# Glaciohound/Chimera-ST

Measured on AMD Instinct MI355X. Metric: train utterances/sec, MuST-C EN-DE s2t_transformer_m, 1/2/4/8 MI355X, higher is better.
Workload: dtype bf16

## Files before the change

chimera-st_amd/csrc/elementwise.hip:

```cpp
#include "cst_common.h"

namespace {

inline int ew_blocks(int64_t items) {
  int64_t b = cst_ceil_div(items, 256);
  return (int)(b < 1 ? 1 : (b > 4096 ? 4096 : b));
}

template <typename T>
__global__ void glu_fwd_kernel(const T* z, T* y, int64_t rows, int64_t C) {
  const int64_t cv = C / 8, total = rows * cv;
  for (int64_t i = (int64_t)blockIdx.x * blockDim.x + threadIdx.x; i < total; i += (int64_t)gridDim.x * blockDim.x) {
    const int64_t r = i / cv, c = (i % cv) * 8;
    float a[8], g[8], o[8];
    load8(z + r * 2 * C + c, a);
    load8(z + r * 2 * C + C + c, g);
#pragma unroll
    for (int e = 0; e < 8; ++e) o[e] = a[e] / (1.0f + __expf(-g[e]));
    store8(y + r * C + c, o);
  }
}

template <typename T>
__global__ void glu_bwd_kernel(const T* dy, const T* z, T* dz, int64_t rows, int64_t C) {
  const int64_t cv = C / 8, total = rows * cv;
  for (int64_t i = (int64_t)blockIdx.x * blockDim.x + threadIdx.x; i < total; i += (int64_t)gridDim.x * blockDim.x) {
    const int64_t r = i / cv, c = (i % cv) * 8;
    float a[8], g[8], d[8], da[8], dg[8];
    load8(z + r * 2 * C + c, a);
    load8(z + r * 2 * C + C + c, g);
    load8(dy + r * C + c, d);
#pragma unroll
    for (int e = 0; e < 8; ++e) {
      const float sg = 1.0f / (1.0f + __expf(-g[e]));
      da[e] = d[e] * sg;
      dg[e] = d[e] * a[e] * sg * (1.0f - sg);
    }
    store8(dz + r * 2 * C + c, da);
    store8(dz + r * 2 * C + C + c, dg);
  }
}

template <typename T>
__global__ void act_bwd_kernel(const T* dy, const T* z, T* dx, int64_t n8, int act) {
  for (int64_t i = (int64_t)blockIdx.x * blockDim.x + threadIdx.x; i < n8; i += (int64_t)gridDim.x * blockDim.x) {
    float d[8], zz[8];
    load8(dy + i * 8, d);
    load8(z + i * 8, zz);
#pragma unroll
    for (int e = 0; e < 8; ++e) d[e] *= dact_t<T>(zz[e], act);
    store8(dx + i * 8, d);
  }
}

template <typename T>
__global__ void act_fwd_kernel(const T* x, T* y, int64_t n8, int act) {
  for (int64_t i = (int64_t)blockIdx.x * blockDim.x + threadIdx.x; i < n8; i += (int64_t)gridDim.x * blockDim.x) {
    float v[8];
    load8(x + i * 8, v);
#pragma unroll
    for (int e = 0; e < 8; ++e) v[e] = act_t<T>(v[e], act);
    store8(y + i * 8, v);
  }
}

template <typename T, bool PART = false, bool DROP = false>
__global__ __launch_bounds__(256) void colsum_kernel(const T* x, int64_t ldx, float* out, int64_t rows, int64_t cols, int64_t rows_per,
                                                     const uint32_t* row_live = nullptr, uint32_t epoch = 0, T* xd = nullptr,
                                                     uint32_t dkey = 0, uint32_t dthr = 0, float dscale = 1.0f) {
  __shared__ float red[16][16 * 8 + 1];
  auto masked = [&](float (&v)[8], int64_t r, int64_t c0) {
    cst_drop8(v, dkey, (uint64_t)(r * cols + c0), dthr, dscale);
    store8(xd + r * ldx + c0, v);
    if (sizeof(T) == 2) {
#pragma unroll
      for (int e = 0; e < 8; ++e) v[e] = bf16_bits_to_f32(f32_to_bf16_bits(v[e]));
    } else {
#pragma unroll
      for (int e = 0; e < 8; ++e) asm volatile("" : "+v"(v[e]));
    }
  };
  const int cl = threadIdx.x & 15, g = threadIdx.x >> 4;
  const int64_t cv = (int64_t)blockIdx.x * 16 + cl;
  const bool ok = cv * 8 < cols;
  const int64_t r0 = (int64_t)blockIdx.y * rows_per;
  const int64_t r1 = r0 + rows_per < rows ? r0 + rows_per : rows;
  float acc[8] = {0, 0, 0, 0, 0, 0, 0, 0};
  if (ok) {
    int64_t r = r0 + g;
    for (; r + 48 < r1; r += 64) {
      if (row_live && row_live[(r - g) >> 6] != epoch) {
        if (DROP) {
          float z[8] = {0, 0, 0, 0, 0, 0, 0, 0};
          store8(xd + r * ldx + cv * 8, z); store8(xd + (r + 16) * ldx + cv * 8, z);
          store8(xd + (r + 32) * ldx + cv * 8, z); store8(xd + (r + 48) * ldx + cv * 8, z);
        }
        continue;
      }
      float v0[8], v1[8], v2[8], v3[8];
      load8(x + r * ldx + cv * 8, v0);
      load8(x + (r + 16) * ldx + cv * 8, v1);
      load8(x + (r + 32) * ldx + cv * 8, v2);
      load8(x + (r + 48) * ldx + cv * 8, v3);
      if (DROP) { masked(v0, r, cv * 8); masked(v1, r + 16, cv * 8); masked(v2, r + 32, cv * 8); masked(v3, r + 48, cv * 8); }
#pragma unroll
      for (int e = 0; e < 8; ++e) acc[e] += (v0[e] + v1[e]) + (v2[e] + v3[e]);
    }
    for (; r < r1; r += 16) {
      float v[8];
      load8(x + r * ldx + cv * 8, v);
      if (DROP) masked(v, r, cv * 8);
#pragma unroll
      for (int e = 0; e < 8; ++e) acc[e] += v[e];
    }
  }
#pragma unroll
  for (int e = 0; e < 8; ++e) red[g][cl * 8 + e] = acc[e];
  __syncthreads();
  if (threadIdx.x < 128) {
    const int c = threadIdx.x;
    float a = 0.0f;
#pragma unroll
    for (int k = 0; k < 16; ++k) a += red[k][c];
    const int64_t col = (int64_t)blockIdx.x * 128 + c;
    if (col < cols) {
      if (PART) out[(int64_t)blockIdx.y * cols + col] = a;
      else atomicAdd(out + col, a);
    }
  }
}

template <typename TO>
__global__ __launch_bounds__(1024) void colsum_reduce_kernel(const float* part, TO* out, int chunks, int64_t cols) {
  __shared__ float red[64][17];
  const int cl = threadIdx.x & 15, g = threadIdx.x >> 4;
  const int64_t c = (int64_t)blockIdx.x * 16 + cl;
  float a = 0.0f;
  if (c < cols)
    for (int i = g; i < chunks; i += 64) a += part[(int64_t)i * cols + c];
  red[g][cl] = a;
  __syncthreads();
  if (g == 0 && c < cols) {
#pragma unroll 8
    for (int k = 1; k < 64; ++k) a += red[k][cl];
    DT<TO>::st(out + c, a);
  }
}

template <typename T>
__global__ void col2im1d_kernel(const T* dcol, const T* z, T* dx, int64_t B, int64_t Lin, int64_t Lout, int64_t C, int k,
                                int stride, int pad, int dact) {
  const int64_t cv = C / 8, total = B * Lin * cv;
  for (int64_t i = (int64_t)blockIdx.x * blockDim.x + threadIdx.x; i < total; i += (int64_t)gridDim.x * blockDim.x) {
    const int64_t c = (i % cv) * 8, l = (i / cv) % Lin, b = i / (cv * Lin);
    float acc[8] = {0, 0, 0, 0, 0, 0, 0, 0};
    for (int j = 0; j < k; ++j) {
      const int64_t num = l + pad - j;
      if (num < 0 || num % stride) continue;
      const int64_t t = num / stride;
      if (t >= Lout) continue;
      float v[8];
      load8(dcol + ((b * Lout + t) * k + j) * C + c, v);
#pragma unroll
      for (int e = 0; e < 8; ++e) acc[e] += v[e];
    }
    if (dact) {
      float zz[8];
      load8(z + (b * Lin + l) * C + c, zz);
#pragma unroll
      for (int e = 0; e < 8; ++e) acc[e] *= dact_t<T>(zz[e], dact);
    }
    store8(dx + (b * Lin + l) * C + c, acc);
  }
// ... 133 lines not shown
  CST_REQUIRE(dtype == CST_F32 || dtype == CST_BF16, "cst_act_fwd: bad dtype");
  hipStream_t s = (hipStream_t)stream;
  CstProfScope prof(CST_K_ELEMENTWISE, s, 0.0, 2.0 * n * cst_dtype_size(dtype));
  if (dtype == CST_BF16) hipLaunchKernelGGL(act_fwd_kernel<bf16_t>, dim3(ew_blocks(n / 8)), dim3(256), 0, s, (const bf16_t*)x, (bf16_t*)y, n / 8, act);
  else hipLaunchKernelGGL(act_fwd_kernel<float>, dim3(ew_blocks(n / 8)), dim3(256), 0, s, (const float*)x, (float*)y, n / 8, act);
  return cst_check_launch("cst_act_fwd");
}

extern "C" int cst_colsum(const void* x, int64_t ldx, float* out, int64_t rows, int64_t cols, int dtype, cst_stream stream) {
  CST_REQUIRE(x && out && rows > 0 && cols > 0 && cols % 8 == 0 && ldx % 8 == 0, "cst_colsum: cols/ldx must be multiples of 8");
  CST_REQUIRE(dtype == CST_F32 || dtype == CST_BF16, "cst_colsum: bad dtype");
  hipStream_t s = (hipStream_t)stream;
  CstProfScope prof(CST_K_ELEMENTWISE, s, 0.0, (double)rows * cols * cst_dtype_size(dtype));
  if (hipMemsetAsync(out, 0, sizeof(float) * cols, s) != hipSuccess) { cst_set_error("cst_colsum: memset failed"); return CST_ERR_LAUNCH; }
  const int64_t cblocks = cst_ceil_div(cols / 8, 16);
  int64_t chunks = cst_ceil_div(1536, cblocks);
  if (chunks > cst_ceil_div(rows, 64)) chunks = cst_ceil_div(rows, 64);
  if (chunks < 1) chunks = 1;
  const int64_t rows_per = cst_ceil_div(rows, chunks);
  dim3 grid((unsigned)cblocks, (unsigned)cst_ceil_div(rows, rows_per));
  if (dtype == CST_BF16) hipLaunchKernelGGL(colsum_kernel<bf16_t>, grid, dim3(256), 0, s, (const bf16_t*)x, ldx, out, rows, cols, rows_per);
  else hipLaunchKernelGGL(colsum_kernel<float>, grid, dim3(256), 0, s, (const float*)x, ldx, out, rows, cols, rows_per);
  return cst_check_launch("cst_colsum");
}

static void colsum_grid(int64_t rows, int64_t cols, int64_t& cblocks, int64_t& nchunks, int64_t& rows_per) {
  cblocks = cst_ceil_div(cols / 8, 16);
  int64_t chunks = cst_ceil_div(1536, cblocks);
  if (chunks > cst_ceil_div(rows, 64)) chunks = cst_ceil_div(rows, 64);
  if (chunks < 1) chunks = 1;
  rows_per = cst_ceil_div(cst_ceil_div(rows, chunks), 64) * 64;
  nchunks = cst_ceil_div(rows, rows_per);
}

extern "C" int64_t cst_colsum_workspace(int64_t rows, int64_t cols) {
  if (rows <= 0 || cols <= 0) return 0;
  int64_t cb, nc, rp;
  colsum_grid(rows, cols, cb, nc, rp);
  return nc * cols * (int64_t)sizeof(float);
}

static int colsum_typed_impl(const void* x, int64_t ldx, void* out, void* workspace, int64_t rows, int64_t cols, int dtype,
                             int out_dtype, const uint32_t* row_live, uint32_t epoch, cst_stream stream) {
  CST_REQUIRE(x && workspace && rows > 0 && cols > 0 && cols % 8 == 0 && ldx % 8 == 0, "cst_colsum_typed: cols/ldx must be multiples of 8");
  CST_REQUIRE((dtype == CST_F32 || dtype == CST_BF16) && (out_dtype == CST_F32 || out_dtype == CST_BF16), "cst_colsum_typed: bad dtype");
  hipStream_t s = (hipStream_t)stream;
  CstProfScope prof(CST_K_ELEMENTWISE, s, 0.0, (double)rows * cols * cst_dtype_size(dtype));
  int64_t cblocks, nchunks, rows_per;
  colsum_grid(rows, cols, cblocks, nchunks, rows_per);
  dim3 grid((unsigned)cblocks, (unsigned)nchunks);
  float* part = (float*)workspace;
  if (dtype == CST_BF16) hipLaunchKernelGGL((colsum_kernel<bf16_t, true>), grid, dim3(256), 0, s, (const bf16_t*)x, ldx, part, rows, cols, rows_per, row_live, epoch);
  else hipLaunchKernelGGL((colsum_kernel<float, true>), grid, dim3(256), 0, s, (const float*)x, ldx, part, rows, cols, rows_per, row_live, epoch);
  if (!out) return cst_check_launch("cst_colsum_typed");
  const dim3 rgrid((unsigned)cst_ceil_div(cols, 16));
  if (out_dtype == CST_BF16) hipLaunchKernelGGL(colsum_reduce_kernel<bf16_t>, rgrid, dim3(1024), 0, s, (const float*)part, (bf16_t*)out, (int)nchunks, cols);
  else hipLaunchKernelGGL(colsum_reduce_kernel<float>, rgrid, dim3(1024), 0, s, (const float*)part, (float*)out, (int)nchunks, cols);
  return cst_check_launch("cst_colsum_typed");
}

extern "C" int cst_dropout_colsum(const void* x, void* xd, void* out, void* workspace, int64_t rows, int64_t cols, int dtype, int out_dtype,
                                  float p, uint32_t key, const uint32_t* row_live, uint32_t epoch, cst_stream stream) {
  CST_REQUIRE(x && xd && workspace && rows > 0 && cols > 0 && cols % 8 == 0, "cst_dropout_colsum: cols must be a multiple of 8");
  CST_REQUIRE((dtype == CST_F32 || dtype == CST_BF16) && (out_dtype == CST_F32 || out_dtype == CST_BF16), "cst_dropout_colsum: bad dtype");
  CST_REQUIRE(p > 0.0f && p < 1.0f, "cst_dropout_colsum: p must be in (0, 1)");
  CST_REQUIRE(!row_live || epoch != 0, "cst_dropout_colsum: stamps need a non-zero epoch");
  hipStream_t s = (hipStream_t)stream;
  CstProfScope prof(CST_K_ELEMENTWISE, s, 0.0, 2.0 * (double)rows * cols * cst_dtype_size(dtype));
  int64_t cblocks, nchunks, rows_per;
  colsum_grid(rows, cols, cblocks, nchunks, rows_per);
  dim3 grid((unsigned)cblocks, (unsigned)nchunks);
  float* part = (float*)workspace;
  const uint32_t thr = cst_drop_thr16(p);
  const float scale = 1.0f / (1.0f - p);
  if (dtype == CST_BF16) hipLaunchKernelGGL((colsum_kernel<bf16_t, true, true>), grid, dim3(256), 0, s, (const bf16_t*)x, cols, part, rows, cols, rows_per, row_live, epoch, (bf16_t*)xd, key, thr, scale);
  else hipLaunchKernelGGL((colsum_kernel<float, true, true>), grid, dim3(256), 0, s, (const float*)x, cols, part, rows, cols, rows_per, row_live, epoch, (float*)xd, key, thr, scale);
  if (!out) return cst_check_launch("cst_dropout_colsum");
  const dim3 rgrid((unsigned)cst_ceil_div(cols, 16));
  if (out_dtype == CST_BF16) hipLaunchKernelGGL(colsum_reduce_kernel<bf16_t>, rgrid, dim3(1024), 0, s, (const float*)part, (bf16_t*)out, (int)nchunks, cols);
  else hipLaunchKernelGGL(colsum_reduce_kernel<float>, rgrid, dim3(1024), 0, s, (const float*)part, (float*)out, (int)nchunks, cols);
  return cst_check_launch("cst_dropout_colsum");
}

extern "C" int cst_colsum_typed(const void* x, int64_t ldx, void* out, void* workspace, int64_t rows, int64_t cols, int dtype,
                                int out_dtype, cst_stream stream) {
  return colsum_typed_impl(x, ldx, out, workspace, rows, cols, dtype, out_dtype, nullptr, 0, stream);
}

extern "C" int cst_colsum_typed_live(const void* x, int64_t ldx, void* out, void* workspace, int64_t rows, int64_t cols, int dtype,
                                     int out_dtype, const uint32_t* row_live, uint32_t epoch, cst_stream stream) {
  CST_REQUIRE(row_live && epoch != 0, "cst_colsum_typed_live: stamps / non-zero epoch required");
  return colsum_typed_impl(x, ldx, out, workspace, rows, cols, dtype, out_dtype, row_live, epoch, stream);
}

extern "C" int cst_col2im1d(const void* dcol, const void* z, void* dx, int64_t B, int64_t Lin, int64_t Lout, int64_t C, int k,
                            int stride, int pad, int dact, int dtype, cst_stream stream) {
  CST_REQUIRE(dcol && dx && B > 0 && Lin > 0 && Lout > 0 && C > 0 && C % 8 == 0 && k >= 1 && stride >= 1 && pad >= 0, "cst_col2im1d: bad args");
  CST_REQUIRE(!dact || z, "cst_col2im1d: dact needs z");
  CST_REQUIRE(dtype == CST_F32 || dtype == CST_BF16, "cst_col2im1d: bad dtype");
  hipStream_t s = (hipStream_t)stream;
  CstProfScope prof(CST_K_ELEMENTWISE, s, 0.0, ((double)B * Lout * k * C + (double)B * Lin * C * (dact ? 2.0 : 1.0)) * cst_dtype_size(dtype));
  const int blocks = ew_blocks(B * Lin * C / 8);
  if (dtype == CST_BF16) hipLaunchKernelGGL(col2im1d_kernel<bf16_t>, dim3(blocks), dim3(256), 0, s, (const bf16_t*)dcol, (const bf16_t*)z, (bf16_t*)dx, B, Lin, Lout, C, k, stride, pad, dact);
  else hipLaunchKernelGGL(col2im1d_kernel<float>, dim3(blocks), dim3(256), 0, s, (const float*)dcol, (const float*)z, (float*)dx, B, Lin, Lout, C, k, stride, pad, dact);
  return cst_check_launch("cst_col2im1d");
}

extern "C" int cst_mask_rows(const void* x, const uint8_t* mask, void* y, int64_t rows, int64_t cols, int dtype, cst_stream stream) {
  CST_REQUIRE(x && mask && y && rows > 0 && cols > 0 && cols % 8 == 0, "cst_mask_rows: bad args");
  CST_REQUIRE(dtype == CST_F32 || dtype == CST_BF16, "cst_mask_rows: bad dtype");
  hipStream_t s = (hipStream_t)stream;
  CstProfScope prof(CST_K_ELEMENTWISE, s, 0.0, 2.0 * rows * cols * cst_dtype_size(dtype));
  const int blocks = ew_blocks(rows * cols / 8);
  if (dtype == CST_BF16) hipLaunchKernelGGL(mask_rows_kernel<bf16_t>, dim3(blocks), dim3(256), 0, s, (const bf16_t*)x, mask, (bf16_t*)y, rows, cols);
  else hipLaunchKernelGGL(mask_rows_kernel<float>, dim3(blocks), dim3(256), 0, s, (const float*)x, mask, (float*)y, rows, cols);
  return cst_check_launch("cst_mask_rows");
}

extern "C" int cst_dropout(const void* x, void* y, int64_t n, float p, uint32_t key, int dtype, cst_stream stream) {
  CST_REQUIRE(x && y && n > 0 && p >= 0.0f && p < 1.0f, "cst_dropout: bad args");
  CST_REQUIRE(dtype == CST_F32 || dtype == CST_BF16, "cst_dropout: bad dtype");
  CST_REQUIRE(((uintptr_t)x % 16 == 0) && ((uintptr_t)y % 16 == 0), "cst_dropout: x/y must be 16-byte aligned");
  hipStream_t s = (hipStream_t)stream;
  CstProfScope prof(CST_K_ELEMENTWISE, s, 0.0, 2.0 * n * cst_dtype_size(dtype));
  const int blocks = ew_blocks(cst_ceil_div(n, 8));
  const uint32_t thr = cst_drop_thr16(p);
  const float scale = 1.0f / (1.0f - p);
  if (dtype == CST_BF16) hipLaunchKernelGGL(dropout_kernel<bf16_t>, dim3(blocks), dim3(256), 0, s, (const bf16_t*)x, (bf16_t*)y, n, key, thr, scale);
  else hipLaunchKernelGGL(dropout_kernel<float>, dim3(blocks), dim3(256), 0, s, (const float*)x, (float*)y, n, key, thr, scale);
  return cst_check_launch("cst_dropout");
}


extern "C" int cst_rows_pack(const void* src, const int32_t* seq_off, void* dst, int64_t B, int64_t T, int64_t C, int tail_sum, int dtype,
                             cst_stream stream) {
  CST_REQUIRE(src && seq_off && dst && B > 0 && T > 0 && C > 0, "cst_rows_pack: bad args");
  CST_REQUIRE(dtype == CST_F32 || dtype == CST_BF16, "cst_rows_pack: bad dtype %d", dtype);
  CST_REQUIRE(C % 8 == 0 && B < 65536, "cst_rows_pack: C=%lld must be a multiple of 8", (long long)C);
  hipStream_t s = (hipStream_t)stream;
  CstProfScope prof(CST_K_ELEMENTWISE, s, 0.0, 2.0 * B * T * C * cst_dtype_size(dtype));
  const dim3 grid((unsigned)cst_ceil_div(T, 4), (unsigned)B);
  if (dtype == CST_BF16) hipLaunchKernelGGL(rows_pack_kernel<bf16_t>, grid, dim3(256), 0, s, (const bf16_t*)src, seq_off, (bf16_t*)dst, (int)T, (int)C, tail_sum);
  else hipLaunchKernelGGL(rows_pack_kernel<float>, grid, dim3(256), 0, s, (const float*)src, seq_off, (float*)dst, (int)T, (int)C, tail_sum);
  return cst_check_launch("cst_rows_pack");
}

extern "C" int cst_rows_unpack(const void* src, const int32_t* seq_off, void* dst, int64_t B, int64_t T, int64_t C, int tail_broadcast, int dtype,
                               cst_stream stream) {
  CST_REQUIRE(src && seq_off && dst && B > 0 && T > 0 && C > 0, "cst_rows_unpack: bad args");
  CST_REQUIRE(dtype == CST_F32 || dtype == CST_BF16, "cst_rows_unpack: bad dtype %d", dtype);
  CST_REQUIRE(C % 8 == 0 && B < 65536, "cst_rows_unpack: C=%lld must be a multiple of 8", (long long)C);
  hipStream_t s = (hipStream_t)stream;
  CstProfScope prof(CST_K_ELEMENTWISE, s, 0.0, 2.0 * B * T * C * cst_dtype_size(dtype));
  const dim3 grid((unsigned)cst_ceil_div(T, 4), (unsigned)B);
  if (dtype == CST_BF16) hipLaunchKernelGGL(rows_unpack_kernel<bf16_t>, grid, dim3(256), 0, s, (const bf16_t*)src, seq_off, (bf16_t*)dst, (int)T, (int)C, tail_broadcast);
  else hipLaunchKernelGGL(rows_unpack_kernel<float>, grid, dim3(256), 0, s, (const float*)src, seq_off, (float*)dst, (int)T, (int)C, tail_broadcast);
  return cst_check_launch("cst_rows_unpack");
}

namespace {
constexpr int WN_ROWS = 256;

template <typename T, bool DOT>
__global__ __launch_bounds__(256) void wn_partial_kernel(const T* v, const T* dw, float* part, int64_t R, int C) {
  const int gpr = C / 8, rl = threadIdx.x / gpr, cg = threadIdx.x % gpr, rpp = 256 / gpr;
  __shared__ float red[256 * 8];
// ... 274 lines not shown
```

chimera-st_amd/csrc/gemm.hip:

```cpp
#include "gemm_common.h"
#include <vector>
#include <stdlib.h>
#include <string.h>
#include <type_traits>

namespace {
using namespace cstg;

template <int BM_, int BN_, int WM_, int WN_, int KV_ = 8>
struct Cfg {
  static constexpr int BM = BM_, BN = BN_, WM = WM_, WN = WN_, NT = 64 * WM_ * WN_, TM = BM_ / WM_ / 32, TN = BN_ / WN_ / 32;
  static constexpr int KV = KV_;
  static_assert(BM_ <= GEMM_MAX_BM && GEMM_MAX_BM % BM_ == 0, "conv0.hip (cst_conv_row_limits) sizes live frames from GEMM_MAX_BM");
};
using CfgSmall = Cfg<128, 128, 2, 2>;
using CfgSkinny = Cfg<64, 64, 2, 2>;
using CfgNarrowN = Cfg<128, 64, 2, 2>;
using CfgNarrowM = Cfg<64, 128, 2, 2>;
using CfgLarge = Cfg<256, 256, 4, 4>;

template <typename T, bool A_KMAJOR, bool B_KMAJOR, bool SEG, typename C, bool CS = false>
__global__ __launch_bounds__(C::NT) void gemm_kernel(GemmParams p) {
  constexpr int BM = C::BM, BN = C::BN, NTHREADS = C::NT, TM = C::TM, TN = C::TN;
  constexpr int VEC = DT<T>::VEC;
  constexpr int KV = C::KV, BK = KV * VEC;
  constexpr int LDK = BK + VEC;
  constexpr int LDMA = sizeof(T) == 2 ? BM + 32 : BM + VEC;
  constexpr int LDMB = sizeof(T) == 2 ? BN + 32 : BN + VEC;
  constexpr int A_ELEMS = A_KMAJOR ? BM * LDK : BK * LDMA;
  constexpr int B_ELEMS = B_KMAJOR ? BN * LDK : BK * LDMB;
  constexpr int MVA = BM / VEC, MVB = BN / VEC;
  constexpr int NVA = BM * KV / NTHREADS, NVB = BN * KV / NTHREADS;
  extern __shared__ __attribute__((aligned(16))) char smem_raw[];
  T* smem = reinterpret_cast<T*>(smem_raw);
  constexpr int STAGE = A_ELEMS + B_ELEMS;

  const int tid = threadIdx.x, lane = tid & 63, wave = tid >> 6;
  const int wm = wave / C::WN, wn = wave % C::WN;

  const int ntiles = p.tiles_m * p.tiles_n;
  int tm, tn, z;
  if (p.split_order) {
    const int total = ntiles * p.splits, L = (int)blockIdx.x + (int)gridDim.x * (int)blockIdx.z;
    const int q = total / 8, r = total % 8, xcd = L % 8, loc = L / 8;
    const int item = (xcd < r ? xcd * (q + 1) : r * (q + 1) + (xcd - r) * q) + loc;
    z = item / ntiles;
    const int t = item % ntiles;
    tm = t / p.tiles_n;
    tn = t % p.tiles_n;
  } else {
    int id = blockIdx.x;
    {
      const int q = ntiles / 8, r = ntiles % 8, xcd = id % 8, loc = id / 8;
      id = (xcd < r ? xcd * (q + 1) : r * (q + 1) + (xcd - r) * q) + loc;
    }
    constexpr int GROUP_M = 8;
    const int per_group = GROUP_M * p.tiles_n;
    const int grp = id / per_group, rem = id % per_group;
    const int gm0 = grp * GROUP_M;
    const int gsz = (p.tiles_m - gm0 < GROUP_M) ? (p.tiles_m - gm0) : GROUP_M;
    tm = gm0 + rem % gsz;
    tn = rem / gsz;
    z = blockIdx.z;
  }
  const int64_t m0 = (int64_t)tm * BM, n0 = (int64_t)tn * BN;

  const int split = z % p.splits;
  const int64_t bidx = z / p.splits;
  const int64_t b0 = bidx / p.batch1, b1 = bidx % p.batch1;
  const T* A = (const T*)p.A + b0 * p.sa0 + b1 * p.sa1;
  const T* B = (const T*)p.B + b0 * p.sb0 + b1 * p.sb1;
  const int64_t cofs = b0 * p.sc0 + b1 * p.sc1;
  const int64_t bofs = b0 * p.sbias0 + b1 * p.sbias1;

  int ktiles = (int)((p.K + BK - 1) / BK);
  const int kfull = (int)(p.K / BK);
  if (p.k_len) {
    typedef const __attribute__((address_space(4))) int32_t* cptr_t;
    const int kl = ((cptr_t)p.k_len)[b0];
    const int live = kl <= 0 ? 0 : (kl + BK - 1) / BK;
    ktiles = live < ktiles ? live : ktiles;
  }
  const int per = (ktiles + p.splits - 1) / p.splits;
// ... 671 lines not shown
  p.tiles_m = (int)cst_ceil_div(M, C::BM);
  p.tiles_n = (int)cst_ceil_div(N, C::BN);
  p.split_order = (p.splits > 1 && nbatch == 1) ? 1 : 0;
  dim3 grid(p.tiles_m * p.tiles_n, 1, (unsigned)(nbatch * p.splits));
  if constexpr (!AK && !BK_ && !SEG && C::NT <= 256) {
    if (p.colsum) {
      static bool attr_cs = false;
      if (!attr_cs) {
        (void)hipFuncSetAttribute(reinterpret_cast<const void*>(&gemm_kernel<T, AK, BK_, SEG, C, true>), hipFuncAttributeMaxDynamicSharedMemorySize, 160 * 1024 - 4096);
        attr_cs = true;
      }
      hipLaunchKernelGGL((gemm_kernel<T, AK, BK_, SEG, C, true>), grid, dim3(C::NT), lds, s, p);
      return cst_check_launch("cst_gemm");
    }
  }
  if (p.colsum) { cst_set_error("cst_gemm: internal: column sums requested from a configuration that does not build them"); return CST_ERR_UNSUPPORTED; }
  hipLaunchKernelGGL((gemm_kernel<T, AK, BK_, SEG, C>), grid, dim3(C::NT), lds, s, p);
  return cst_check_launch("cst_gemm");
}

template <typename T, bool AK, bool BK_, typename C, int NS>
int launch_glds(GemmParams p, int64_t M, int64_t N, int64_t nbatch, hipStream_t s) {
  constexpr int ES = sizeof(T), BKc = 128 / ES;
  constexpr int A_BYTES = AK ? C::BM * 128 : BKc * C::BM * ES, B_BYTES = BK_ ? C::BN * 128 : BKc * C::BN * ES;
  size_t lds = (size_t)NS * (A_BYTES + B_BYTES);
  const size_t stage_bytes = (size_t)64 * (C::BN + 4) * sizeof(float);
  if (lds < stage_bytes) lds = stage_bytes;
  static bool attr_set = false;
  if (!attr_set) {
    (void)hipFuncSetAttribute(reinterpret_cast<const void*>(&gemm_glds_kernel<T, AK, BK_, C, NS>), hipFuncAttributeMaxDynamicSharedMemorySize, 160 * 1024);
    attr_set = true;
  }
  p.tiles_m = (int)cst_ceil_div(M, C::BM);
  p.tiles_n = (int)cst_ceil_div(N, C::BN);
  dim3 grid(p.tiles_m * p.tiles_n, 1, (unsigned)(nbatch * p.splits));
  hipLaunchKernelGGL((gemm_glds_kernel<T, AK, BK_, C, NS>), grid, dim3(C::NT), lds, s, p);
  return cst_check_launch("cst_gemm");
}


struct GemmSwitches {
  bool no_klive;
  int group_m;
  bool no_narrow;
  bool no_4w;
  bool experiment;
  const char* force_cfg;
};

GemmSwitches gemm_switches() {
  static const GemmSwitches once = [] {
    GemmSwitches w;
    w.no_klive = getenv("CST_GEMM_NO_KLIVE") != nullptr;
    const char* gm = getenv("CST_GEMM8P_GROUP_M");
    w.group_m = gm && atoi(gm) > 0 ? atoi(gm) : 4;
    w.no_narrow = getenv("CST_GEMM_NO_NARROW") != nullptr;
    w.no_4w = getenv("CST_GEMM_NO_4W") != nullptr;
    w.experiment = getenv("CST_GEMM_EXPERIMENT") != nullptr;
    w.force_cfg = nullptr;
    return w;
  }();
  GemmSwitches w = once;
  if (w.experiment) {
    const char* f = getenv("CST_GEMM_FORCE_CFG");
    w.force_cfg = f && *f ? f : nullptr;
  }
  return w;
}

enum class Family { Reg, Dma, Persistent8, FourWave };
enum class Tile { Small, Large, Skinny, NarrowN, NarrowM, Big4, Big4N, Unknown };
enum class Colsum { None, Fused, Separate };
using CfgBig4 = Cfg<256, 256, 2, 2>;
using CfgBig4N = Cfg<256, 192, 2, 2>;

struct GemmRoute {
  Family family;
  Tile tile;
  bool bf16, ak, bk;
  bool seg;
  int stages;
  int splits;
  Colsum colsum;
};

struct TileDims { int bm, bn, nt; };
template <typename C> constexpr TileDims dims_of() { return {C::BM, C::BN, C::NT}; }
constexpr TileDims kTileDims[] = {dims_of<CfgSmall>(),   dims_of<CfgLarge>(), dims_of<CfgSkinny>(), dims_of<CfgNarrowN>(),
                                  dims_of<CfgNarrowM>(), dims_of<CfgBig4>(),  dims_of<CfgBig4N>(),  {0, 0, 0}};

bool use_large(const cst_gemm_desc* d, bool seg, int splits) {
  if (seg) return false;
  const int64_t tiles = cst_ceil_div(d->M, 256) * cst_ceil_div(d->N, 256) * d->batch0 * d->batch1 * splits;
  return d->M >= 256 && d->N >= 256 && tiles >= 200;
}

int choose_splits(const cst_gemm_desc* d) {
  if (d->split_k > 1) return d->split_k;
  if (d->split_k == 0 || d->split_k == 1) return 1;
  const int bk = d->dtype == CST_BF16 ? 64 : 32;
  const int64_t ktiles = cst_ceil_div(d->K, bk);
  const int64_t nb = d->batch0 * d->batch1;
  if (d->M >= 256 && d->N >= 256) {
    const int64_t tl = cst_ceil_div(d->M, 256) * cst_ceil_div(d->N, 256) * nb;
    if (tl >= 200) return 1;
    int64_t s = 256 / tl;
    if (s > ktiles / 16) s = ktiles / 16;
    if (s > 32) s = 32;
    if (s >= 1 && tl * s >= 200) return (int)s;
  }
  const int64_t tiles = cst_ceil_div(d->M, 128) * cst_ceil_div(d->N, 128) * nb;
  if (tiles >= 256 || ktiles < 16) return 1;
  const int64_t cap = ktiles / 8 < 32 ? ktiles / 8 : 32;
  int64_t s1 = 256 / tiles, s2 = 512 / tiles;
  if (s1 > cap) s1 = cap;
  if (s2 > cap) s2 = cap;
  if (s1 < 1) s1 = 1;
  if (s2 < 1) s2 = 1;
  const int64_t s = (2.0 / (double)s2 < 0.9 / (double)s1) ? s2 : s1;
  return (int)s;
}

struct Forced { const char* name; bool kk; Family family; Tile tile; int stages; };
const Forced kForced[] = {
    {"small", false, Family::Reg, Tile::Small, 0},     {"narrowm", false, Family::Reg, Tile::NarrowM, 0},
    {"narrown", false, Family::Reg, Tile::NarrowN, 0}, {"skinny", false, Family::Reg, Tile::Skinny, 0},
    {"large", false, Family::Reg, Tile::Large, 0},     {"big4r", false, Family::Reg, Tile::Big4, 0},
    {"skinny4", true, Family::Dma, Tile::Skinny, 4},   {"skinny2", true, Family::Dma, Tile::Skinny, 2},
    {"small2", true, Family::Dma, Tile::Small, 2},     {"small3", true, Family::Dma, Tile::Small, 3},
    {"big4", true, Family::Dma, Tile::Big4, 2},        {"big4n", true, Family::Dma, Tile::Big4N, 2},
    {"big4r", true, Family::Reg, Tile::Big4, 0},       {"large", true, Family::Reg, Tile::Large, 0},
    {"8p", true, Family::Persistent8, Tile::Large, 0}, {"4w", true, Family::FourWave, Tile::Big4N, 0},
};

GemmRoute gemm_route(const cst_gemm_desc* d, const GemmParams& p, const GemmSwitches& sw) {
  GemmRoute r;
  r.bf16 = d->dtype == CST_BF16;
  r.ak = d->a_kmajor != 0;
  r.bk = d->b_kmajor != 0;
  r.seg = (r.ak && d->a_seg) || (r.bk && d->b_seg);
  r.stages = 2;
  r.splits = choose_splits(d);
  const bool kk = r.ak && r.bk, mm = !r.ak && !r.bk;
  const bool large = use_large(d, r.seg, r.splits);
  const int64_t nbatch = d->batch0 * d->batch1;
  r.colsum = !d->colsum ? Colsum::None : (mm && !d->a_seg && !d->b_seg && !large) ? Colsum::Fused : Colsum::Separate;
  auto take = [&r](Family f, Tile t, int stages = 2) { r.family = f; r.tile = t; r.stages = stages; return r; };

  if (!sw.no_narrow && !r.seg && !large && kk && d->N <= 64 && d->M > 256) return take(Family::Dma, Tile::NarrowN);
  if (!sw.no_narrow && !r.seg && !large && mm && d->M <= 64 && d->N > 256) return take(Family::Reg, Tile::NarrowM);

  GemmParams q = p;
  q.splits = r.splits;
  const bool unsplit1 = !r.seg && nbatch == 1 && r.splits == 1;
  if (sw.force_cfg && r.bf16 && !r.seg && nbatch == 1 && (mm || (kk && r.splits == 1))) {
    for (const Forced& f : kForced) {
      if (f.kk != kk || strcmp(f.name, sw.force_cfg) != 0) continue;
      if (f.family == Family::Persistent8 && !cst_gemm8p_supported(q, r.ak, r.bk, nbatch)) break;
      if (f.family == Family::FourWave && !cst_gemm4w_supported(q, r.ak, r.bk, nbatch)) break;
      return take(f.family, f.tile, f.stages);
    }
    return take(Family::Reg, Tile::Unknown);
  }

  const bool mid8p = kk && unsplit1 && d->M >= 256 && d->N >= 256 && cst_ceil_div(d->M, 256) * cst_ceil_div(d->N, 256) >= 150;
  if (kk && unsplit1 && (d->M <= 256 || (!large && !mid8p && cst_ceil_div(d->M, 128) * cst_ceil_div(d->N, 128) < 256))) {
    const bool two_stage = d->M > 256 && cst_ceil_div(d->M, 64) * cst_ceil_div(d->N, 64) > 512;
    return take(Family::Dma, Tile::Skinny, two_stage ? 2 : 4);
  }
  if (r.bf16 && !r.seg && !d->colsum) {
    if (!sw.no_4w && cst_gemm4w_supported(q, r.ak, r.bk, nbatch)) return take(Family::FourWave, Tile::Big4N);
    if (r.ak && (!d->dact || (!d->resid && !d->aux_out)) && (large || mid8p) && cst_gemm8p_supported(q, r.ak, r.bk, nbatch))
      return take(Family::Persistent8, Tile::Large);
  }
  const Tile t = large ? Tile::Large : Tile::Small;
  if (r.seg) return take(Family::Reg, Tile::Small);
  return take(kk && !d->colsum ? Family::Dma : Family::Reg, t);
}

void route_text(const GemmRoute& r, char* out, int64_t n) {
  const TileDims t = kTileDims[(int)r.tile];
  const char* dt = r.bf16 ? "bf16" : "f32";
  const char a = r.ak ? 'k' : 'm', b = r.bk ? 'k' : 'm';
  switch (r.family) {
    case Family::Reg:
      snprintf(out, (size_t)n, "reg %s %c%c%s %dx%d nt%d%s split%d", dt, a, b, r.seg ? " seg" : "", t.bm, t.bn, t.nt,
               r.colsum == Colsum::Fused ? " colsum" : "", r.splits);
      break;
    case Family::Dma: snprintf(out, (size_t)n, "glds %s %c%c %dx%d nt%d ns%d split%d", dt, a, b, t.bm, t.bn, t.nt, r.stages, r.splits); break;
    case Family::Persistent8: snprintf(out, (size_t)n, "8p %c%c", a, b); break;
    case Family::FourWave: snprintf(out, (size_t)n, "4w"); break;
  }
}

}

extern "C" int64_t cst_colsum_workspace(int64_t rows, int64_t cols);
extern "C" int cst_colsum_typed(const void* x, int64_t ldx, void* out, void* workspace, int64_t rows, int64_t cols, int dtype, int out_dtype, cst_stream stream);
extern "C" int cst_colsum_typed_live(const void* x, int64_t ldx, void* out, void* workspace, int64_t rows, int64_t cols, int dtype, int out_dtype,
                                     const uint32_t* row_live, uint32_t epoch, cst_stream stream);

namespace {

int validate(const cst_gemm_desc* d) {
  CST_REQUIRE(d && d->A && d->B && d->C, "cst_gemm: null operand");
  CST_REQUIRE(d->dtype == CST_F32 || d->dtype == CST_BF16, "cst_gemm: bad dtype %d", d->dtype);
  CST_REQUIRE(d->c_dtype == d->dtype || d->c_dtype == CST_F32, "cst_gemm: c_dtype must be dtype or f32");
  CST_REQUIRE(d->M > 0 && d->N > 0 && d->K > 0, "cst_gemm: empty problem M=%lld N=%lld K=%lld", (long long)d->M,
              (long long)d->N, (long long)d->K);
  const int vec = d->dtype == CST_BF16 ? 8 : 4;
  if (d->a_kmajor) CST_REQUIRE(d->K % vec == 0 && d->lda % vec == 0, "cst_gemm: k-major A needs K,lda %% %d == 0 (K=%lld lda=%lld)", vec, (long long)d->K, (long long)d->lda);
  else CST_REQUIRE(d->M % vec == 0 && d->lda % vec == 0, "cst_gemm: mn-major A needs M,lda %% %d == 0 (M=%lld lda=%lld)", vec, (long long)d->M, (long long)d->lda);
  if (d->b_kmajor) CST_REQUIRE(d->K % vec == 0 && d->ldb % vec == 0, "cst_gemm: k-major B needs K,ldb %% %d == 0 (K=%lld ldb=%lld)", vec, (long long)d->K, (long long)d->ldb);
  else CST_REQUIRE(d->N % vec == 0 && d->ldb % vec == 0, "cst_gemm: mn-major B needs N,ldb %% %d == 0 (N=%lld ldb=%lld)", vec, (long long)d->N, (long long)d->ldb);
  CST_REQUIRE(d->a_seg % vec == 0 && d->b_seg % vec == 0 && d->a_seg_stride % vec == 0 && d->b_seg_stride % vec == 0,
              "cst_gemm: segment sizes must be multiples of %d", vec);
  CST_REQUIRE(((uintptr_t)d->A % 16 == 0) && ((uintptr_t)d->B % 16 == 0), "cst_gemm: A/B must be 16-byte aligned");
  CST_REQUIRE(d->sa0 % vec == 0 && d->sa1 % vec == 0 && d->sb0 % vec == 0 && d->sb1 % vec == 0, "cst_gemm: batch strides of A/B must be multiples of %d", vec);
  CST_REQUIRE(d->batch0 >= 1 && d->batch1 >= 1, "cst_gemm: batch counts must be >= 1");
  CST_REQUIRE(!d->dact || d->aux_in, "cst_gemm: dact needs aux_in");
  CST_REQUIRE(d->drop_p >= 0.0f && d->drop_p < 1.0f, "cst_gemm: drop_p must be in [0, 1)");
  CST_REQUIRE(d->drop_p == 0.0f || d->batch0 * d->batch1 == 1, "cst_gemm: fused dropout needs an unbatched problem");
  CST_REQUIRE(!d->colsum || (!d->a_kmajor && !d->a_seg), "cst_gemm: colsum needs an mn-major, unsegmented A");
  return CST_OK;
}

GemmParams fill_params(const cst_gemm_desc* d, const GemmSwitches& sw) {
  GemmParams p;
  p.M = d->M; p.N = d->N; p.K = d->K;
  p.A = d->A; p.lda = d->lda; p.a_seg = d->a_seg; p.a_seg_stride = d->a_seg_stride;
  p.B = d->B; p.ldb = d->ldb; p.b_seg = d->b_seg; p.b_seg_stride = d->b_seg_stride;
  p.C = d->C; p.ldc = d->ldc;
  p.bias = d->bias; p.bias_mode = d->bias ? d->bias_mode : CST_BIAS_NONE; p.sbias0 = d->sbias0; p.sbias1 = d->sbias1;
  p.act = d->act;
  p.aux_out = d->aux_out; p.ld_aux_out = d->ld_aux_out;
  p.dact = d->dact; p.aux_in = d->aux_in; p.ld_aux_in = d->ld_aux_in;
  p.resid = d->resid; p.ld_resid = d->ld_resid;
  p.alpha = d->alpha;
  p.drop_thr = d->drop_p > 0.0f ? cst_drop_thr16(d->drop_p) : 0u;
  p.drop_key = d->drop_key;
  p.drop_scale = d->drop_p > 0.0f ? 1.0f / (1.0f - d->drop_p) : 1.0f;
  p.drop_row0 = 0;
  p.batch1 = d->batch1;
  p.sa0 = d->sa0; p.sa1 = d->sa1; p.sb0 = d->sb0; p.sb1 = d->sb1; p.sc0 = d->sc0; p.sc1 = d->sc1;
  p.c_f32 = (d->c_dtype == CST_F32 && d->dtype != CST_F32) ? 1 : 0;
  {
    auto al16 = [](const void* q) { return q == nullptr || ((uintptr_t)q % 16) == 0; };
    bool ok = d->ldc % 8 == 0 && d->sc0 % 8 == 0 && d->sc1 % 8 == 0 && al16(d->C) && al16(d->bias) && al16(d->aux_out) && al16(d->aux_in) && al16(d->resid);
    if (d->bias && d->bias_mode == CST_BIAS_COL) ok = ok && d->sbias0 % 8 == 0 && d->sbias1 % 8 == 0;
    if (d->aux_out) ok = ok && d->ld_aux_out % 8 == 0;
    if (d->aux_in) ok = ok && d->ld_aux_in % 8 == 0;
    if (d->resid) ok = ok && d->ld_resid % 8 == 0;
    if (d->drop_p > 0.0f) ok = ok && (d->N % 2 == 0);
    p.vec_epi = ok ? 1 : 0;
  }
  p.tiles_m = p.tiles_n = 0;
  p.split_order = 0;
  p.sched = nullptr;
  p.gperm_full = 0;
  p.mrot = 0;
  p.k_live = sw.no_klive ? nullptr : d->k_live;
  p.k_epoch = d->k_epoch;
  p.m_live = sw.no_klive ? nullptr : d->m_live;
  p.m_epoch = d->m_epoch;
  p.k_len = sw.no_klive ? nullptr : d->k_len;
  p.m_len = sw.no_klive ? nullptr : d->m_len;
  p.group_m = sw.group_m;
  p.splits = 1;
  p.ws = nullptr;
  p.colsum = nullptr;
  p.colsum_ws = nullptr;
  return p;
}

int64_t route_workspace(const cst_gemm_desc* d, const GemmRoute& r) {
  const int64_t s = r.splits, nb = d->batch0 * d->batch1;
  int64_t bytes = s > 1 ? s * d->M * d->N * nb * (int64_t)sizeof(float) : 0;
  if (r.colsum == Colsum::Fused) bytes += s > 1 ? s * d->M * nb * (int64_t)sizeof(float) : 0;
  else if (r.colsum == Colsum::Separate) bytes += cst_colsum_workspace(d->K, d->M);
  return bytes;
}

int take_route(const cst_gemm_desc* d, const GemmSwitches& sw, GemmParams& p, GemmRoute& r) {
  r = gemm_route(d, p, sw);
  const int64_t nbatch = d->batch0 * d->batch1;
  CST_REQUIRE(r.colsum != Colsum::Separate || (nbatch == 1 && d->M % 8 == 0 && d->lda % 8 == 0),
              "cst_gemm: colsum of this configuration runs as a separate column sum: unbatched, M and lda multiples of 8");
  CST_REQUIRE(cst_ceil_div(d->M, 128) * cst_ceil_div(d->N, 128) < (1ll << 31) && nbatch * r.splits < 65536, "cst_gemm: grid too large");
  p.splits = r.splits;
  p.colsum = r.colsum == Colsum::Fused ? d->colsum : nullptr;
#ifdef CST_TRACE
  if (p.splits == 1 && d->workspace) p.ws = (float*)d->workspace;
#endif
  const int64_t need = route_workspace(d, r);
  if (need > 0 && (!d->workspace || d->workspace_bytes < need)) {
    if (r.splits > 1) cst_set_error("cst_gemm: split_k=%d needs %lld workspace bytes, got %lld", r.splits, (long long)need, (long long)d->workspace_bytes);
    else cst_set_error("cst_gemm: colsum needs %lld workspace bytes, got %lld", (long long)need, (long long)d->workspace_bytes);
    return CST_ERR_WORKSPACE;
  }
  if (r.splits > 1) {
    p.ws = (float*)d->workspace;
    p.colsum_ws = p.ws + (int64_t)r.splits * d->M * d->N * nbatch;
  }
  return CST_OK;
}

template <typename W>
bool read_back(hipStream_t s, const W* dev, int64_t n, std::vector<W>& host) {
  host.resize((size_t)n);
  return hipStreamSynchronize(s) == hipSuccess && hipMemcpy(host.data(), dev, sizeof(W) * n, hipMemcpyDeviceToHost) == hipSuccess;
}

struct Work { double flops, bytes; };
Work credited_work(const cst_gemm_desc* d, const GemmParams& p, hipStream_t s) {
  double frac = 1.0;
  if (cst_prof_is_on()) {
    std::vector<uint32_t> st;
    std::vector<int32_t> len;
    const int64_t mtiles = cst_ceil_div(d->M, 256);
    if (p.k_live && read_back(s, p.k_live, cst_ceil_div(d->K, 64), st)) {
      int64_t live = 0;
      for (uint32_t v : st) live += v == p.k_epoch;
      frac *= (double)live / (double)st.size();
    }
    if (p.k_len && read_back(s, p.k_len, d->batch0, len)) {
      double sum = 0.0;
      for (int32_t v : len) sum += (double)(v < 0 ? 0 : (v < d->K ? v : d->K));
      frac *= sum / ((double)d->batch0 * (double)d->K);
    }
    if (p.m_len && read_back(s, p.m_len, d->batch0, len)) {
      double live = 0.0;
      for (int32_t v : len) {
        const int64_t t = v <= 0 ? 0 : cst_ceil_div((int64_t)v, 256);
        live += (double)(t < mtiles ? t : mtiles);
      }
      frac *= live / ((double)d->batch0 * (double)mtiles);
    }
    if (p.m_live && read_back(s, p.m_live, cst_ceil_div(d->M, 64), st)) {
      const int64_t nt = (int64_t)st.size();
      int64_t live = 0;
      for (int64_t t = 0; t < mtiles; ++t) {
        bool l = false;
        for (int64_t i = 4 * t; i < 4 * t + 4 && i < nt; ++i) l |= st[i] == p.m_epoch;
        live += l;
      }
      frac *= (double)live / (double)mtiles;
    }
  }
  const double nbatch = (double)(d->batch0 * d->batch1), esz = (double)cst_dtype_size(d->dtype);
  return {2.0 * (double)d->M * (double)d->N * (double)d->K * nbatch * frac,
          ((double)d->M * d->K + (double)d->N * d->K) * esz * nbatch * frac + (double)d->M * d->N * cst_dtype_size(d->c_dtype) * nbatch};
}

int unlaunchable(const GemmRoute& r, const GemmSwitches& sw) {
  if (r.tile == Tile::Unknown) {
    cst_set_error("cst_gemm: unknown CST_GEMM_FORCE_CFG %s", sw.force_cfg ? sw.force_cfg : "");
    return CST_ERR_BAD_ARG;
  }
  if (r.family == Family::Reg && r.colsum == Colsum::Fused && kTileDims[(int)r.tile].nt > 256) {
    cst_set_error("cst_gemm: internal: column sums requested from a configuration that does not build them");
    return CST_ERR_UNSUPPORTED;
  }
  return CST_OK;
}

template <typename T, bool SEG, typename C>
int launch_reg(const GemmRoute& r, const GemmParams& p, int64_t nbatch, hipStream_t s) {
  return r.ak ? (r.bk ? launch<T, true, true, SEG, C>(p, p.M, p.N, nbatch, s) : launch<T, true, false, SEG, C>(p, p.M, p.N, nbatch, s))
              : (r.bk ? launch<T, false, true, SEG, C>(p, p.M, p.N, nbatch, s) : launch<T, false, false, SEG, C>(p, p.M, p.N, nbatch, s));
}

constexpr int arm(Family f, Tile t, int stages = 0) { return ((int)f << 8) | ((int)t << 4) | stages; }

// ... 5 lines not shown
    case arm(Family::Persistent8, Tile::Large): return cst_gemm8p_launch(p, r.ak, r.bk, nbatch, s);
    case arm(Family::FourWave, Tile::Big4N): return cst_gemm4w_launch(p, s);
    case arm(Family::Reg, Tile::Small): return r.seg ? launch_reg<T, true, CfgSmall>(r, p, nbatch, s) : launch_reg<T, false, CfgSmall>(r, p, nbatch, s);
    case arm(Family::Reg, Tile::Large): return launch_reg<T, false, CfgLarge>(r, p, nbatch, s);
    case arm(Family::Reg, Tile::NarrowM): return launch<T, false, false, false, CfgNarrowM>(p, M, N, nbatch, s);
    case arm(Family::Dma, Tile::Small, 2): return launch_glds<T, true, true, CfgSmall, 2>(p, M, N, nbatch, s);
    case arm(Family::Dma, Tile::Large, 2): return launch_glds<T, true, true, CfgLarge, 2>(p, M, N, nbatch, s);
    case arm(Family::Dma, Tile::NarrowN, 2): return launch_glds<T, true, true, CfgNarrowN, 2>(p, M, N, nbatch, s);
    case arm(Family::Dma, Tile::Skinny, 2): return launch_glds<T, true, true, CfgSkinny, 2>(p, M, N, nbatch, s);
    case arm(Family::Dma, Tile::Skinny, 4): return launch_glds<T, true, true, CfgSkinny, 4>(p, M, N, nbatch, s);
    case arm(Family::Reg, Tile::NarrowN): if constexpr (HOOK) return launch<T, false, false, false, CfgNarrowN>(p, M, N, nbatch, s); break;
    case arm(Family::Reg, Tile::Skinny): if constexpr (HOOK) return launch<T, false, false, false, CfgSkinny>(p, M, N, nbatch, s); break;
    case arm(Family::Reg, Tile::Big4):
      if constexpr (HOOK) return r.ak ? launch<T, true, true, false, CfgBig4>(p, M, N, nbatch, s) : launch<T, false, false, false, CfgBig4>(p, M, N, nbatch, s);
      break;
    case arm(Family::Dma, Tile::Small, 3): if constexpr (HOOK) return launch_glds<T, true, true, CfgSmall, 3>(p, M, N, nbatch, s); break;
    case arm(Family::Dma, Tile::Big4, 2): if constexpr (HOOK) return launch_glds<T, true, true, CfgBig4, 2>(p, M, N, nbatch, s); break;
    case arm(Family::Dma, Tile::Big4N, 2): if constexpr (HOOK) return launch_glds<T, true, true, CfgBig4N, 2>(p, M, N, nbatch, s); break;
    default: break;
  }
  const int rc = unlaunchable(r, sw);
  if (rc == CST_OK) cst_set_error("cst_gemm: internal: a route without a launch arm");
  return rc == CST_OK ? CST_ERR_UNSUPPORTED : rc;
}

int finish(const cst_gemm_desc* d, const GemmRoute& r, const GemmParams& p, cst_stream stream) {
  const int64_t nbatch = d->batch0 * d->batch1;
  if (p.splits > 1 && d->defer_reduce) {
    CST_REQUIRE((nbatch == 1 || !d->colsum) && d->alpha == 1.0f && !d->bias && !d->act && !d->dact && !d->aux_out && !d->resid && d->drop_p == 0.0f && d->ldc == d->N &&
                    d->N % 8 == 0 && r.colsum != Colsum::Separate,
                "cst_gemm: defer_reduce needs a plain epilogue and a dense C (batched: no colsum; the slabs are [batch][split][M][N])");
    return CST_OK;
  }
  int rc = CST_OK;
  if (p.splits > 1) {
    const int64_t total = d->M * d->N;
    const int64_t work = (p.vec_epi && d->N % 8 == 0) ? total / 8 : total;
    int blocks = (int)(cst_ceil_div(work, 256) < 2048 ? cst_ceil_div(work, 256) : 2048);
    dim3 grid(blocks, (unsigned)nbatch);
    if (d->dtype == CST_BF16) hipLaunchKernelGGL(splitk_reduce_kernel<bf16_t>, grid, dim3(256), 0, (hipStream_t)stream, p);
    else hipLaunchKernelGGL(splitk_reduce_kernel<float>, grid, dim3(256), 0, (hipStream_t)stream, p);
    rc = cst_check_launch("cst_gemm split-k reduce");
  }
  if (rc == CST_OK && r.colsum == Colsum::Separate) {
    void* cws = (char*)d->workspace + (p.splits > 1 ? (int64_t)p.splits * d->M * d->N * (int64_t)sizeof(float) : 0);
    rc = p.k_live ? cst_colsum_typed_live(d->A, d->lda, d->colsum, cws, d->K, d->M, d->dtype, d->dtype, p.k_live, p.k_epoch, stream)
                  : cst_colsum_typed(d->A, d->lda, d->colsum, cws, d->K, d->M, d->dtype, d->dtype, stream);
  }
  return rc;
}

int gemm_one(const cst_gemm_desc* d, cst_stream stream) {
  int rc = validate(d);
  if (rc != CST_OK) return rc;
  const GemmSwitches sw = gemm_switches();
  GemmParams p = fill_params(d, sw);
  GemmRoute r;
  if ((rc = take_route(d, sw, p, r)) != CST_OK) return rc;
  hipStream_t s = (hipStream_t)stream;
  const int64_t nbatch = d->batch0 * d->batch1;
  const Work w = credited_work(d, p, s);
  CstProfScope prof(CST_K_GEMM, s, w.flops, w.bytes);
  rc = r.bf16 ? launch_route<bf16_t>(r, p, nbatch, s, sw) : launch_route<float>(r, p, nbatch, s, sw);
  if (cst_prof_is_on())
    prof.tag("M=%lld N=%lld K=%lld b=%lld a%c b%c split=%d%s%s%s%s%s%s%s", (long long)d->M, (long long)d->N, (long long)d->K, (long long)nbatch, r.ak ? 'k' : 'm',
             r.bk ? 'k' : 'm', p.splits, d->bias ? " bias" : "", d->act ? " act" : "", d->aux_out ? " aux_out" : "", d->dact ? " dact" : "",
             d->resid ? " resid" : "", d->drop_p > 0 ? " drop" : "", (d->k_live || d->m_live || d->k_len || d->m_len) ? " live" : "");
  return rc != CST_OK ? rc : finish(d, r, p, stream);
}

GemmRoute query_route(const cst_gemm_desc* d) {
  const GemmSwitches sw = gemm_switches();
  return gemm_route(d, fill_params(d, sw), sw);
}

}

extern "C" int cst_gemm_splits(const cst_gemm_desc* d) { return d ? query_route(d).splits : 0; }

extern "C" int cst_gemm_colsum_is_fused(const cst_gemm_desc* d) { return d && query_route(d).colsum == Colsum::Fused ? 1 : 0; }

extern "C" int64_t cst_gemm_workspace(const cst_gemm_desc* d) { return route_workspace(d, query_route(d)); }

extern "C" int cst_gemm_route(const cst_gemm_desc* d, char* out, int64_t out_bytes) {
  if (out && out_bytes > 0) out[0] = 0;
  int rc = validate(d);
  if (rc != CST_OK) return rc;
  CST_REQUIRE(out && out_bytes > 0, "cst_gemm_route: no room for the text");
  const GemmSwitches sw = gemm_switches();
  GemmParams p = fill_params(d, sw);
  GemmRoute r;
  if ((rc = take_route(d, sw, p, r)) != CST_OK) return rc;
  if ((rc = unlaunchable(r, sw)) != CST_OK) return rc;
  route_text(r, out, out_bytes);
  return CST_OK;
}

extern "C" int cst_gemm(const cst_gemm_desc* d, cst_stream stream) { return gemm_one(d, stream); }
```

chimera-st_amd/csrc/gemm8p.hip:

```cpp
#include "gemm_common.h"
#include <atomic>
#include <cstdlib>
#include <mutex>
#include <type_traits>

namespace {
using namespace cstg;
using T = bf16_t;

constexpr int BM = 256, BN = 256, BK = 64, NTHREADS = 512;
static_assert(BM <= cstg::GEMM_MAX_BM && cstg::GEMM_MAX_BM % BM == 0, "conv0.hip (cst_conv_row_limits) sizes live frames from GEMM_MAX_BM");
constexpr int QB = 17408;
constexpr int GSTRIDE = 1088;
constexpr int KSTRIDE = 1024;
constexpr int BUFB = 4 * QB;
constexpr int LDS_BYTES = 2 * BUFB;
constexpr unsigned OOB = 0x80000000u;

template <int N>
__device__ __forceinline__ void wait_vm() { asm volatile("s_waitcnt vmcnt(%0)" ::"n"(N) : "memory"); }
template <int N>
__device__ __forceinline__ void wait_lgkm() { asm volatile("s_waitcnt lgkmcnt(%0)" ::"n"(N) : "memory"); }

__device__ __forceinline__ unsigned lds_off(const void* p) {
  return (unsigned)(uintptr_t)(const __attribute__((address_space(3))) char*)p;
}
__device__ __forceinline__ void lds_write_b64(unsigned addr, uint2 v) {
  asm volatile("ds_write_b64 %0, %1" ::"v"(addr), "v"(v) : "memory");
}
__device__ __forceinline__ void lds_write_b128(unsigned addr, f32x4 v) {
  asm volatile("ds_write_b128 %0, %1" ::"v"(addr), "v"(v) : "memory");
}
__device__ __forceinline__ u32x4 lds_read_b128(unsigned addr) {
  u32x4 v;
  asm volatile("ds_read_b128 %0, %1" : "=v"(v) : "v"(addr) : "memory");
  return v;
}

template <int OFF>
__device__ __forceinline__ u32x4 lds_read_b128_off(unsigned addr) {
  u32x4 v;
  asm volatile("ds_read_b128 %0, %1 offset:%2" : "=v"(v) : "v"(addr), "n"(OFF) : "memory");
  return v;
}

__device__ __forceinline__ void dma16(__amdgpu_buffer_rsrc_t rsrc, char* lds_wave_base, unsigned voff) {
  __builtin_amdgcn_raw_ptr_buffer_load_lds(rsrc, (__attribute__((address_space(3))) void*)lds_wave_base, 16, (int)voff, 0, 0, 0);
}

template <bool AK, bool BKM, int MODE>
__global__ __launch_bounds__(NTHREADS) void gemm8p_kernel(GemmParams p) {
  extern __shared__ __attribute__((aligned(16))) char smem[];
  const int tid = threadIdx.x, lane = tid & 63;
  const int wave = __builtin_amdgcn_readfirstlane(tid >> 6);
  const int wm = wave >> 2, wn = wave & 3;
  const int lrow = lane & 31, hi = lane >> 5;
  const int ntiles = p.tiles_m * p.tiles_n;
  const int total = p.nitems;
  const int ktiles = (int)((p.K + BK - 1) / BK);
  const int per = (ktiles + p.splits - 1) / p.splits;
  typedef const __attribute__((address_space(4))) GemmParams* kparg_t;
  kparg_t kp = (kparg_t)__builtin_amdgcn_kernarg_segment_ptr();

  const int ck = (lane & 7) ^ (((4 * wave) + (lane >> 4)) & 7);
  const int klm = 16 * (wave >> 2) + 4 * (lane >> 4) + (wave & 3);
  const int kla = AK ? ck * 8 : klm, klb = BKM ? ck * 8 : klm;
  const int pa = AK ? 8 * wave + (lane >> 3) : (lane & 15) * 8;
  const int pb = BKM ? 8 * wave + (lane >> 3) : (lane & 15) * 8;
  const unsigned step_a = AK ? (unsigned)(BK * 2) : (unsigned)(BK * p.lda * 2);
  const unsigned step_b = BKM ? (unsigned)(BK * 2) : (unsigned)(BK * p.ldb * 2);
  constexpr bool EXF = MODE == 2;
  const bool fast_epi = MODE != 0 || (!p.c_f32 && p.splits == 1 && p.vec_epi && (p.N % 8) == 0 && p.bias_mode != CST_BIAS_ROW &&
                                (p.bias_mode == CST_BIAS_NONE || p.alpha == 1.0f));
  const bool bias_in_acc = fast_epi && p.bias_mode == CST_BIAS_COL;
  char* const bias_lds = smem + 2 * BUFB;

  __amdgpu_buffer_rsrc_t ra, rb;
  unsigned va0 = 0, vb0 = 0;
  int nt = 0, krem0 = 0, mrem = 0, nrem = 0;
  int hf = 0;
  unsigned lda2 = 0, ldb2 = 0;
  int64_t m0 = 0, n0 = 0, cofs = 0, bofs = 0;
  int zcur = 0;

  auto setup = [&](int v) {
    asm volatile("" : "+s"(kp));
    struct { int64_t M, N, K, lda, ldb, batch1, sa0, sa1, sb0, sb1, sc0, sc1, sbias0, sbias1; const void *A, *B, *bias; int splits, tiles_m, tiles_n; } p;
    p.M = kp->M; p.N = kp->N; p.K = kp->K; p.lda = kp->lda; p.ldb = kp->ldb; p.batch1 = kp->batch1;
    p.sa0 = kp->sa0; p.sa1 = kp->sa1; p.sb0 = kp->sb0; p.sb1 = kp->sb1; p.sc0 = kp->sc0; p.sc1 = kp->sc1;
    p.sbias0 = kp->sbias0; p.sbias1 = kp->sbias1; p.A = kp->A; p.B = kp->B; p.bias = kp->bias;
    p.splits = kp->splits; p.tiles_m = kp->tiles_m; p.tiles_n = kp->tiles_n;
    auto fdiv = [](int n, unsigned long long magic) { return (int)(((unsigned long long)(unsigned)n * magic) >> 40); };
    int half = -1, vt = v;
    if (v >= kp->half_from) {
      const int o = v - kp->half_from;
      half = o & 1;
      vt = kp->half_from + (o >> 1);
    }
    hf = half >= 0 ? 1 : 0;
    const int z = kp->nz > 1 ? fdiv(vt, kp->magic_ntiles) : 0;
    int id = vt - z * ntiles;
    {
      const int q = ntiles >> 3, r = ntiles & 7, xcd = id & 7, loc = id >> 3;
      id = (xcd < r ? xcd * (q + 1) : r * (q + 1) + (xcd - r) * q) + loc;
    }
    if (kp->mrot > 0) {
      int zr = z * kp->mrot;
      zr -= fdiv(zr, kp->magic_ntiles) * ntiles;
      id += zr;
      if (id >= ntiles) id -= ntiles;
    }
    const int GROUP_M = kp->group_m, per_group = kp->per_group, gshift = kp->group_shift;
    int grp = fdiv(id, kp->magic_per_group);
    const int rem = id - grp * per_group;
    if (kp->gperm_full > 0 && grp < kp->gperm_full) {
      const int q = kp->gperm_q, r = kp->gperm_r, big = (q + 1) * r;
      int col, row;
      if (grp < big) { col = fdiv(grp, kp->magic_gq1); row = grp - col * (q + 1); }
      else { const int t = grp - big, c = fdiv(t, kp->magic_gq); col = r + c; row = t - c * q; }
      grp = row * 8 + col;
    }
    const int gm0 = grp * GROUP_M;
    const int gsz = (p.tiles_m - gm0 < GROUP_M) ? (p.tiles_m - gm0) : GROUP_M;
    int tm, tn;
    if (gsz == GROUP_M && gshift >= 0) { tm = gm0 + (rem & (GROUP_M - 1)); tn = rem >> gshift; }
    else { tm = gm0 + rem % gsz; tn = rem / gsz; }
    m0 = (int64_t)tm * BM + (half == 1 ? 128 : 0);
    n0 = (int64_t)tn * BN;
    zcur = z;
    const int split = p.splits > 1 ? z % p.splits : 0;
    const int64_t bidx = p.splits > 1 ? z / p.splits : z;
    const int64_t b0 = p.batch1 > 1 ? bidx / p.batch1 : bidx, b1 = p.batch1 > 1 ? bidx % p.batch1 : 0;
    const T* A = (const T*)p.A + b0 * p.sa0 + b1 * p.sa1;
// ... 69 lines not shown
    const v4s_t x = __builtin_amdgcn_ds_read_tr16_b64_v4i16((v4s_t __attribute__((address_space(3)))*)(q));
    const v4s_t y = __builtin_amdgcn_ds_read_tr16_b64_v4i16((v4s_t __attribute__((address_space(3)))*)(q + 256));
    u16x8 t;
    t[0] = (unsigned short)x[0]; t[1] = (unsigned short)x[1]; t[2] = (unsigned short)x[2]; t[3] = (unsigned short)x[3];
    t[4] = (unsigned short)y[0]; t[5] = (unsigned short)y[1]; t[6] = (unsigned short)y[2]; t[7] = (unsigned short)y[3];
    f.v = __builtin_bit_cast(bf16x8, t);
  };
  auto read_a = [&](Frag<T>& f, const char* img, int i, int kk) {
    if (AK) f.v = *reinterpret_cast<const bf16x8*>(img + arow + i * 4096 + (((2 * kk + hi) ^ swr) << 4));
    else read_tr(f, img + trl + wm * 128 + i * 64 + kk * 4 * GSTRIDE);
  };
  auto read_b = [&](Frag<T>& f, const char* img, int kk) {
    if (BKM) f.v = *reinterpret_cast<const bf16x8*>(img + brow + (((2 * kk + hi) ^ swr) << 4));
    else read_tr(f, img + trl + wn * 64 + kk * 4 * GSTRIDE);
  };

  f32x16 acc[4][2];
  Frag<T> fa[2][4], fb0[4], fb1[4];

  auto mfma_quadrant = [&](auto hmc, auto hnc) {
    constexpr int HM = decltype(hmc)::value, HN = decltype(hnc)::value;
    __builtin_amdgcn_s_setprio(1);
#pragma unroll
    for (int kk = 0; kk < 4; ++kk)
#pragma unroll
      for (int i = 0; i < 2; ++i) mma16(acc[HM * 2 + i][HN], HN ? fb1[kk] : fb0[kk], fa[i][kk]);
    __builtin_amdgcn_s_setprio(0);
  };

  auto tile_body = [&](auto bufc, int t, int S, const bool half) {
    constexpr int BUF = decltype(bufc)::value;
    using BC = std::integral_constant<int, BUF>;
    using BN_ = std::integral_constant<int, BUF ^ 1>;
    const char* img = smem + BUF * BUFB;
    const int s0 = 7 + 4 * t;
#pragma unroll
    for (int kk = 0; kk < 4; ++kk) read_b(fb0[kk], img + 0 * QB, kk);
    __builtin_amdgcn_sched_barrier(0);
#pragma unroll
    for (int kk = 0; kk < 4; ++kk)
#pragma unroll
      for (int i = 0; i < 2; ++i) read_a(fa[i][kk], img + 1 * QB, i, kk);
    __builtin_amdgcn_sched_barrier(0);
    if (s0 < S) stage(I3{}, BN_{}, t + 1);
    wait_lgkm<AK ? 8 : 15>();
    __builtin_amdgcn_s_barrier();
    wait_lgkm<0>();
    __builtin_amdgcn_sched_barrier(0);
    mfma_quadrant(I0{}, I0{});
    __builtin_amdgcn_s_barrier();
#pragma unroll
    for (int kk = 0; kk < 4; ++kk) read_b(fb1[kk], img + 2 * QB, kk);
    __builtin_amdgcn_sched_barrier(0);
    if (s0 + 1 < S) stage(I0{}, BC{}, t + 2);
    __builtin_amdgcn_s_barrier();
    wait_lgkm<0>();
    __builtin_amdgcn_sched_barrier(0);
    mfma_quadrant(I0{}, I1{});
    __builtin_amdgcn_s_barrier();
    if (!half) {
#pragma unroll
      for (int kk = 0; kk < 4; ++kk)
#pragma unroll
        for (int i = 0; i < 2; ++i) read_a(fa[i][kk], img + 3 * QB, i, kk);
    }
    __builtin_amdgcn_sched_barrier(0);
    if (s0 + 2 < S) stage(I1{}, BC{}, t + 2);
    __builtin_amdgcn_s_barrier();
    wait_lgkm<0>();
    __builtin_amdgcn_sched_barrier(0);
    if (!half) mfma_quadrant(I1{}, I1{});
    __builtin_amdgcn_s_barrier();
    if (s0 + 3 < S) stage(I2{}, BC{}, t + 2);
    if (s0 + 4 <= S) wait_vm<6>();
    else wait_vm<0>();
    __builtin_amdgcn_s_barrier();
    __builtin_amdgcn_sched_barrier(0);
    if (!half) mfma_quadrant(I1{}, I0{});
    __builtin_amdgcn_s_barrier();
  };

  char* const ebase = smem + BUFB;
  const unsigned ebase_off = lds_off(ebase);

  int v = blockIdx.x;
  if (v >= total) return;
  const unsigned slot_off = lds_off(smem + 2 * BUFB + 1024);
  int par = 0;
  int claim = 0;
  auto claim_issue = [&]() {
    int* const sched = p.sched;
    if (sched && tid == 0) claim = __hip_atomic_fetch_add(sched + (blockIdx.x & 7), 1, __ATOMIC_RELAXED, __HIP_MEMORY_SCOPE_AGENT);
  };
  auto claim_land = [&]() {
    if (p.sched && tid == 0) {
      const int item = (int)gridDim.x + (int)(blockIdx.x & 7) + 8 * claim;
      asm volatile("ds_write_b32 %0, %1" ::"v"(slot_off + 4u * (unsigned)(par ^ 1)), "v"(item) : "memory");
    }
    par ^= 1;
  };
  setup(v);
  {
    const int S = 4 * nt;
    if (0 < S) stage(I0{}, I0{}, 0);
    if (1 < S) stage(I1{}, I0{}, 0);
    if (2 < S) stage(I2{}, I0{}, 0);
    if (3 < S) stage(I3{}, I0{}, 0);
  }
  claim_issue();
  claim_land();
#ifdef CST_TRACE
  long long* trace = (p.splits == 1 && p.ws) ? reinterpret_cast<long long*>(p.ws) + (int64_t)blockIdx.x * 64 : nullptr;
  int titem = 0;
#define CST_STAMP(k) do { if (trace && tid == 0 && titem < 8) trace[titem * 8 + (k)] = (long long)__builtin_readcyclecounter(); } while (0)
#else
#define CST_STAMP(k) do { } while (0)
#endif
  while (true) {
    CST_STAMP(0);
    const int64_t e_m0 = m0, e_n0 = n0, e_cofs = cofs, e_bofs = bofs;
    const int e_z = zcur, e_nt = nt;
    const bool e_hf = hf != 0;
    const int S = 4 * e_nt;
    if (4 < S) stage(I0{}, I1{}, 1);
    if (5 < S) stage(I1{}, I1{}, 1);
    if (6 < S) stage(I2{}, I1{}, 1);
    if (7 <= S) wait_vm<6>();
    else wait_vm<0>();
    __builtin_amdgcn_s_barrier();
    if (bias_in_acc) {
#pragma unroll
      for (int hn = 0; hn < 2; ++hn)
#pragma unroll
        for (int g = 0; g < 4; ++g) {
          const uint2 raw = *reinterpret_cast<const uint2*>(bias_lds + (hn * 128 + wn * 32 + 8 * g + 4 * hi) * 2);
          const float b0 = __uint_as_float(raw.x << 16), b1 = __uint_as_float(raw.x & 0xffff0000u);
          const float b2 = __uint_as_float(raw.y << 16), b3 = __uint_as_float(raw.y & 0xffff0000u);
#pragma unroll
          for (int i = 0; i < 4; ++i) {
            acc[i][hn][4 * g] = b0; acc[i][hn][4 * g + 1] = b1; acc[i][hn][4 * g + 2] = b2; acc[i][hn][4 * g + 3] = b3;
          }
        }
      wait_lgkm<0>();
    } else {
#pragma unroll
      for (int i = 0; i < 4; ++i)
#pragma unroll
        for (int j = 0; j < 2; ++j)
#pragma unroll
          for (int r = 0; r < 16; ++r) acc[i][j][r] = 0.0f;
    }
    if (wm == 1) __builtin_amdgcn_s_barrier();
    CST_STAMP(1);
    for (int t = 0; t < e_nt; t += 2) {
      tile_body(I0{}, t, S, e_hf);
      if (t + 1 < e_nt) tile_body(I1{}, t + 1, S, e_hf);
    }
    if (wm == 0) __builtin_amdgcn_s_barrier();
    CST_STAMP(2);

    {
      int item;
      asm volatile("ds_read_b32 %0, %1\n\ts_waitcnt lgkmcnt(0)" : "=v"(item) : "v"(slot_off + 4u * (unsigned)par) : "memory");
      v = __builtin_amdgcn_readfirstlane(p.sched ? item : v + (int)gridDim.x);
    }
    const bool has_next = v < total;
    if (has_next) {
      claim_issue();
      setup(v);
      CST_STAMP(5);
      const int Sn = 4 * nt;
      if (0 < Sn) stage(I0{}, I0{}, 0);
      if (1 < Sn) stage(I1{}, I0{}, 0);
      if (2 < Sn) stage(I2{}, I0{}, 0);
      if (3 < Sn) stage(I3{}, I0{}, 0);
      CST_STAMP(6);
    }

    CST_STAMP(3);
    asm volatile("" : "+s"(kp));
    GemmParams q;
    q.M = kp->M; q.N = kp->N; q.C = kp->C; q.ldc = kp->ldc; q.bias = kp->bias; q.bias_mode = kp->bias_mode; q.act = kp->act;
    q.aux_out = kp->aux_out; q.ld_aux_out = kp->ld_aux_out; q.dact = kp->dact; q.aux_in = kp->aux_in; q.ld_aux_in = kp->ld_aux_in;
    q.resid = kp->resid; q.ld_resid = kp->ld_resid; q.alpha = kp->alpha; q.splits = kp->splits; q.ws = kp->ws;
    q.c_f32 = kp->c_f32; q.vec_epi = kp->vec_epi; q.drop_thr = kp->drop_thr; q.drop_key = kp->drop_key; q.drop_scale = kp->drop_scale; q.drop_row0 = kp->drop_row0;
    if (fast_epi && e_nt == 0 && q.bias_mode == CST_BIAS_NONE && !q.resid) {
      if (has_next) claim_land();
      const u32x4 z4 = {0u, 0u, 0u, 0u};
      const int64_t col = e_n0 + (tid & 31) * 8;
      if (col < q.N) {
        T* const cb = (T*)q.C + e_cofs + col;
        T* const xb = q.aux_out ? (T*)q.aux_out + e_cofs + col : nullptr;
#pragma unroll 4
        for (int it = 0; it < (e_hf ? 8 : 16); ++it) {
          const int64_t row = e_m0 + (tid >> 5) + 16 * it;
          if (row < q.M) {
            __builtin_nontemporal_store(z4, reinterpret_cast<u32x4*>(cb + row * q.ldc));
            if (xb) __builtin_nontemporal_store(z4, reinterpret_cast<u32x4*>(xb + row * q.ld_aux_out));
          }
        }
      }
    } else if (fast_epi) {
      constexpr int ERS = 528;
      const T* exsrc = MODE == 1 ? nullptr : (q.dact ? (const T*)q.aux_in : (const T*)q.resid);
      const int64_t exld = q.dact ? q.ld_aux_in : q.ld_resid;
      const bool both = q.dact && q.resid;
      constexpr bool ex_fast = EXF;
      u32x4 exq[8];
      const T* ex_b = nullptr;
      if (ex_fast) {
        int64_t colc = e_n0 + (tid & 31) * 8;
        colc = colc < q.N ? colc : q.N - 8;
        ex_b = exsrc + e_cofs + colc;
#pragma unroll
        for (int it = 0; it < 8; ++it) {
          int64_t row = e_m0 + (tid >> 5) + 16 * it;
          row = row < q.M ? row : q.M - 1;
          exq[it] = __builtin_nontemporal_load(reinterpret_cast<const u32x4*>(ex_b + row * exld));
        }
      }
#pragma unroll
      for (int hm = 0; hm < 2; ++hm) {
        if (hm && e_hf) break;
        if (hm) __builtin_amdgcn_s_barrier();
#pragma unroll
        for (int i = 0; i < 2; ++i)
#pragma unroll
          for (int hn = 0; hn < 2; ++hn)
#pragma unroll
            for (int g = 0; g < 4; ++g) {
              typedef __bf16 bf16x4_t __attribute__((ext_vector_type(4)));
              bf16x4_t pk;
#pragma unroll
              for (int e = 0; e < 4; ++e) pk[e] = static_cast<__bf16>(acc[hm * 2 + i][hn][4 * g + e] * q.alpha);
              lds_write_b64(ebase_off + (wm * 64 + i * 32 + lrow) * ERS + (hn * 128 + wn * 32 + 8 * g + 4 * hi) * 2, __builtin_bit_cast(uint2, pk));
            }
        wait_lgkm<0>();
        __builtin_amdgcn_s_barrier();
        if (hm == 0 && has_next) claim_land();
        if (exsrc && !ex_fast) {
#pragma unroll 2
          for (int it = 0; it < 8; ++it) {
            const int vi = tid + NTHREADS * it;
            const int rl = vi >> 5, cl = (vi & 31) * 8;
            const int64_t row = e_m0 + hm * 128 + rl, col = e_n0 + cl;
            if (row >= q.M || col >= q.N) continue;
            const u32x4 exv = *reinterpret_cast<const u32x4*>(exsrc + e_cofs + row * exld + col);
            const u32x4 zraw = lds_read_b128(ebase_off + rl * ERS + cl * 2);
            wait_lgkm<0>();
            __builtin_amdgcn_sched_barrier(0);
            if (q.aux_out) *reinterpret_cast<u32x4*>((T*)q.aux_out + e_cofs + row * q.ld_aux_out + col) = zraw;
            float x[8];
#pragma unroll
            for (int e = 0; e < 4; ++e) {
              x[2 * e] = __uint_as_float(zraw[e] << 16);
              x[2 * e + 1] = __uint_as_float(zraw[e] & 0xffff0000u);
            }
            if (q.act == CST_ACT_RELU) {
#pragma unroll
              for (int e = 0; e < 8; ++e) x[e] = fmaxf(x[e], 0.0f);
            } else if (q.act == CST_ACT_GELU) {
#pragma unroll
              for (int e = 0; e < 8; ++e) x[e] = gelu_t<T>(x[e]);
            }
            if (q.drop_thr) cst_drop8(x, q.drop_key, (uint64_t)((row + q.drop_row0) * q.N + col), q.drop_thr, q.drop_scale);
            if (q.dact) {
#pragma unroll
              for (int e = 0; e < 4; ++e) {
                x[2 * e] *= dact_t<T>(__uint_as_float(exv[e] << 16), q.dact);
                x[2 * e + 1] *= dact_t<T>(__uint_as_float(exv[e] & 0xffff0000u), q.dact);
              }
              if (both) {
                float rr[8];
                load8((const T*)q.resid + e_cofs + row * q.ld_resid + col, rr);
#pragma unroll
                for (int e = 0; e < 8; ++e) x[e] += rr[e];
              }
            } else {
#pragma unroll
              for (int e = 0; e < 4; ++e) {
                x[2 * e] += __uint_as_float(exv[e] << 16);
                x[2 * e + 1] += __uint_as_float(exv[e] & 0xffff0000u);
              }
            }
            bf16x8 ob;
#pragma unroll
            for (int e = 0; e < 8; ++e) ob[e] = static_cast<__bf16>(x[e]);
            lds_write_b128(ebase_off + rl * ERS + cl * 2, __builtin_bit_cast(f32x4, ob));
          }
          wait_lgkm<0>();
        }
        const bool post = !exsrc && (q.act != CST_ACT_NONE || q.drop_thr);
        {
          constexpr int RSTEP = 16 * ERS;
          const int rl0 = tid >> 5, cl = (tid & 31) * 8;
          const unsigned a0 = ebase_off + rl0 * ERS + cl * 2;
          const int64_t col = e_n0 + cl, row0 = e_m0 + hm * 128 + rl0;
          const bool col_ok = col < q.N;
          u32x4 zr[8];
          zr[0] = lds_read_b128_off<0 * RSTEP>(a0); zr[1] = lds_read_b128_off<1 * RSTEP>(a0);
          zr[2] = lds_read_b128_off<2 * RSTEP>(a0); zr[3] = lds_read_b128_off<3 * RSTEP>(a0);
          zr[4] = lds_read_b128_off<4 * RSTEP>(a0); zr[5] = lds_read_b128_off<5 * RSTEP>(a0);
          zr[6] = lds_read_b128_off<6 * RSTEP>(a0); zr[7] = lds_read_b128_off<7 * RSTEP>(a0);
          T* const cbase = (T*)q.C + e_cofs + row0 * q.ldc + col;
          T* const xbase = (T*)q.aux_out + e_cofs + row0 * q.ld_aux_out + col;
          const bool want_aux = !exsrc && q.aux_out;
          if (ex_fast) {
            wait_lgkm<0>();
            __builtin_amdgcn_sched_barrier(0);
#pragma unroll
            for (int it = 0; it < 8; ++it) {
              const u32x4 zraw = zr[it], exv = exq[it];
              float x[8];
#pragma unroll
              for (int e = 0; e < 4; ++e) {
                x[2 * e] = __uint_as_float(zraw[e] << 16);
                x[2 * e + 1] = __uint_as_float(zraw[e] & 0xffff0000u);
              }
              if (q.act == CST_ACT_RELU) {
#pragma unroll
                for (int e = 0; e < 8; ++e) x[e] = fmaxf(x[e], 0.0f);
              } else if (q.act == CST_ACT_GELU) {
#pragma unroll
                for (int e = 0; e < 8; ++e) x[e] = gelu_t<T>(x[e]);
              }
              if (q.drop_thr) cst_drop8(x, q.drop_key, (uint64_t)((row0 + 16 * it + q.drop_row0) * q.N + col), q.drop_thr, q.drop_scale);
              if (q.dact) {
#pragma unroll
                for (int e = 0; e < 4; ++e) {
                  x[2 * e] *= dact_t<T>(__uint_as_float(exv[e] << 16), q.dact);
                  x[2 * e + 1] *= dact_t<T>(__uint_as_float(exv[e] & 0xffff0000u), q.dact);
                }
              } else {
#pragma unroll
                for (int e = 0; e < 4; ++e) {
                  x[2 * e] += __uint_as_float(exv[e] << 16);
                  x[2 * e + 1] += __uint_as_float(exv[e] & 0xffff0000u);
                }
              }
              bf16x8 ob;
#pragma unroll
              for (int e = 0; e < 8; ++e) ob[e] = static_cast<__bf16>(x[e]);
              zr[it] = __builtin_bit_cast(u32x4, ob);
            }
            if (hm == 0 && !e_hf) {
#pragma unroll
              for (int it = 0; it < 8; ++it) {
                int64_t row = e_m0 + 128 + (tid >> 5) + 16 * it;
                row = row < q.M ? row : q.M - 1;
                exq[it] = __builtin_nontemporal_load(reinterpret_cast<const u32x4*>(ex_b + row * exld));
              }
            }
#pragma unroll
            for (int it = 0; it < 8; ++it)
              if (col_ok && row0 + 16 * it < q.M)
                __builtin_nontemporal_store(zr[it], reinterpret_cast<u32x4*>(cbase + (int64_t)(16 * it) * q.ldc));
            continue;
          }
#pragma unroll
          for (int it = 0; it < 8; ++it) {
            if (it == 0) wait_lgkm<7>(); else if (it == 1) wait_lgkm<6>(); else if (it == 2) wait_lgkm<5>(); else if (it == 3) wait_lgkm<4>();
            else if (it == 4) wait_lgkm<3>(); else if (it == 5) wait_lgkm<2>(); else if (it == 6) wait_lgkm<1>(); else wait_lgkm<0>();
            __builtin_amdgcn_sched_barrier(0);
            const u32x4 zraw = zr[it];
            if (!(col_ok && row0 + 16 * it < q.M)) continue;
            T* cdst = cbase + (int64_t)(16 * it) * q.ldc;
            if (want_aux) __builtin_nontemporal_store(zraw, reinterpret_cast<u32x4*>(xbase + (int64_t)(16 * it) * q.ld_aux_out));
            if (!post) {
              __builtin_nontemporal_store(zraw, reinterpret_cast<u32x4*>(cdst));
              continue;
            }
            float x[8];
#pragma unroll
            for (int e = 0; e < 4; ++e) {
              x[2 * e] = __uint_as_float(zraw[e] << 16);
              x[2 * e + 1] = __uint_as_float(zraw[e] & 0xffff0000u);
            }
            if (q.act == CST_ACT_RELU) {
#pragma unroll
              for (int e = 0; e < 8; ++e) x[e] = fmaxf(x[e], 0.0f);
            } else if (q.act == CST_ACT_GELU) {
#pragma unroll
              for (int e = 0; e < 8; ++e) x[e] = gelu_t<T>(x[e]);
            }
            if (q.drop_thr) cst_drop8(x, q.drop_key, (uint64_t)((row0 + 16 * it + q.drop_row0) * q.N + col), q.drop_thr, q.drop_scale);
            {
              bf16x8 ob;
#pragma unroll
              for (int e = 0; e < 8; ++e) ob[e] = static_cast<__bf16>(x[e]);
              __builtin_nontemporal_store(__builtin_bit_cast(u32x4, ob), reinterpret_cast<u32x4*>(cdst));
            }
          }
        }
      }
    } else {
      constexpr int LDC = BN + 4;
      constexpr int VPR = BN / 8;
      constexpr int ITERS = 64 * VPR / NTHREADS;
      float* wsp = q.splits > 1 ? q.ws + ((int64_t)e_z) * q.M * q.N : nullptr;
      const bool ws_vec = (q.N % 4) == 0;
#pragma unroll
      for (int ps = 0; ps < 4; ++ps) {
        if (ps == 2 && e_hf) break;
        if (ps) __builtin_amdgcn_s_barrier();
        if (wm == (ps & 1)) {
#pragma unroll
          for (int i = 0; i < 2; ++i)
#pragma unroll
            for (int hn = 0; hn < 2; ++hn)
#pragma unroll
              for (int g = 0; g < 4; ++g) {
                f32x4 q;
#pragma unroll
                for (int e = 0; e < 4; ++e) q[e] = acc[(ps >> 1) * 2 + i][hn][4 * g + e];
                lds_write_b128(ebase_off + ((i * 32 + lrow) * LDC + hn * 128 + wn * 32 + 8 * g + 4 * hi) * 4, q);
              }
        }
        wait_lgkm<0>();
        __builtin_amdgcn_s_barrier();
        if (ps == 0 && has_next) claim_land();
#pragma unroll 2
        for (int itv = 0; itv < ITERS; ++itv) {
          const int vi = tid + NTHREADS * itv;
          const int rl = vi / VPR, cl = (vi % VPR) * 8;
          const int64_t row = e_m0 + 64 * ps + rl, col = e_n0 + cl;
          if (row >= q.M || col >= q.N) continue;
          float x[8];
          {
            const u32x4 ua = lds_read_b128(ebase_off + (rl * LDC + cl) * 4), ub = lds_read_b128(ebase_off + (rl * LDC + cl + 4) * 4);
            wait_lgkm<0>();
            __builtin_amdgcn_sched_barrier(0);
            const f32x4 a = __builtin_bit_cast(f32x4, ua), b = __builtin_bit_cast(f32x4, ub);
            x[0] = a[0]; x[1] = a[1]; x[2] = a[2]; x[3] = a[3]; x[4] = b[0]; x[5] = b[1]; x[6] = b[2]; x[7] = b[3];
          }
          const bool full = col + 8 <= q.N;
          if (wsp) {
            if (full && ws_vec) store8(wsp + row * q.N + col, x);
            else
              for (int e = 0; e < 8 && col + e < q.N; ++e) wsp[row * q.N + col + e] = x[e];
          } else if (full && q.vec_epi) {
            epilogue_store8<T>(q, e_cofs, e_bofs, row, col, x);
          } else {
            for (int e = 0; e < 8 && col + e < q.N; ++e) epilogue_store<T>(q, e_cofs, e_bofs, row, col + e, x[e]);
          }
        }
      }
    }
    CST_STAMP(4);
#ifdef CST_TRACE
    ++titem;
#endif
    if (!has_next) break;
    __builtin_amdgcn_s_barrier();
  }
  int* const sched_exit = p.sched;
  if (int* const sched = sched_exit; sched && tid == 0) {
    if (atomicAdd(sched + 8, 1) == (int)gridDim.x - 1) {
#pragma unroll
      for (int i = 0; i < 9; ++i) __hip_atomic_store(sched + i, 0, __ATOMIC_RELAXED, __HIP_MEMORY_SCOPE_AGENT);
    }
  }
}

int* sched_slot() {
  constexpr int SLOTS = 1024, MAXDEV = 64;
  static int* ring[MAXDEV] = {};
  static std::atomic<unsigned> next[MAXDEV];
  static std::mutex mu;
  int dev = 0;
  if (hipGetDevice(&dev) != hipSuccess || dev < 0 || dev >= MAXDEV) return nullptr;
  int* r = __atomic_load_n(&ring[dev], __ATOMIC_ACQUIRE);
  if (!r) {
    std::lock_guard<std::mutex> g(mu);
    r = ring[dev];
    if (!r) {
      void* q = nullptr;
      if (hipMalloc(&q, SLOTS * 64) != hipSuccess) return nullptr;
      if (hipMemset(q, 0, SLOTS * 64) != hipSuccess || hipDeviceSynchronize() != hipSuccess) return nullptr;
      r = (int*)q;
      __atomic_store_n(&ring[dev], r, __ATOMIC_RELEASE);
    }
  }
  return r + 16 * (next[dev].fetch_add(1, std::memory_order_relaxed) % SLOTS);
}

std::atomic<int> g_reserved_cus{[] { const char* e = getenv("CST_GEMM_RESERVE_CUS"); return e ? atoi(e) : 0; }()};

template <bool AK, bool BKM, int MODE>
int launch8p(GemmParams p, int64_t nbatch, hipStream_t s) {
  static bool attr_set = false;
  if (!attr_set) {
    (void)hipFuncSetAttribute(reinterpret_cast<const void*>(&gemm8p_kernel<AK, BKM, MODE>), hipFuncAttributeMaxDynamicSharedMemorySize, 160 * 1024);
    attr_set = true;
  }
  p.tiles_m = (int)cst_ceil_div(p.M, BM);
  p.tiles_n = (int)cst_ceil_div(p.N, BN);
  p.nz = (int)(nbatch * p.splits);
  const int64_t total = (int64_t)p.tiles_m * p.tiles_n * p.nz;
  {
    const int64_t ntl = (int64_t)p.tiles_m * p.tiles_n;
    p.per_group = p.group_m * p.tiles_n;
    if (total * ntl >= (1ll << 40) || total * (int64_t)p.per_group >= (1ll << 40)) { cst_set_error("cst_gemm (8-phase): too many work items"); return CST_ERR_BAD_ARG; }
    p.magic_ntiles = ((1ull << 40) / (unsigned long long)ntl) + 1ull;
    p.magic_per_group = ((1ull << 40) / (unsigned long long)p.per_group) + 1ull;
    p.group_shift = -1;
    for (int sft = 0; sft < 16; ++sft)
      if ((1 << sft) == p.group_m) p.group_shift = sft;
    const int gfull = p.tiles_m / p.group_m;
    p.gperm_full = (p.m_len && gfull >= 16) ? gfull : 0;
    p.mrot = (p.m_len && p.gperm_full == 0 && ntl >= 2) ? (int)(ntl / 8 > 0 ? ntl / 8 : 1) : 0;
    p.gperm_q = gfull / 8;
    p.gperm_r = gfull % 8;
    p.magic_gq = p.gperm_q > 0 ? ((1ull << 40) / (unsigned long long)p.gperm_q) + 1ull : 0ull;
    p.magic_gq1 = ((1ull << 40) / (unsigned long long)(p.gperm_q + 1)) + 1ull;
  }
  static const int ncu = [] {
    int dev = 0, n = 256;
    (void)hipGetDevice(&dev);
    (void)hipDeviceGetAttribute(&n, hipDeviceAttributeMultiprocessorCount, dev);
    return n > 0 ? n : 256;
  }();
  const int avail = ncu - g_reserved_cus.load(std::memory_order_relaxed) > 8 ? ncu - g_reserved_cus.load(std::memory_order_relaxed) : 8;
  const bool no_halves = getenv("CST_GEMM8P_NO_HALVES") != nullptr;
  int64_t nitems = total;
  p.half_from = 0x7fffffff;
  if (!no_halves && p.nz == 1 && total > avail) {
    const int64_t r = total % avail;
    if (r > 0 && 2 * r <= avail) {
      p.half_from = (int)(total - r);
      nitems = total + r;
    }
  }
  p.nitems = (int)nitems;
  dim3 grid((unsigned)(nitems < avail ? nitems : avail), 1, 1);
  static const bool static_walk = getenv("CST_GEMM8P_STATIC") != nullptr;
  hipStreamCaptureStatus cap = hipStreamCaptureStatusNone;
  const bool capturing = hipStreamIsCapturing(s, &cap) != hipSuccess || cap != hipStreamCaptureStatusNone;
  p.sched = (!static_walk && !capturing && nitems > avail && grid.x % 8 == 0) ? sched_slot() : nullptr;
  hipLaunchKernelGGL((gemm8p_kernel<AK, BKM, MODE>), grid, dim3(NTHREADS), LDS_BYTES + 1024 + 64, s, p);
  return cst_check_launch("cst_gemm (8-phase)");
}

}

extern "C" int cst_gemm_reserve_cus(int n) {
  const int old = g_reserved_cus.load();
  if (n >= 0) g_reserved_cus.store(n > 248 ? 248 : n);
  return old;
}

bool cst_gemm8p_supported(const cstg::GemmParams& p, bool ak, bool bk, int64_t nbatch) {
  (void)nbatch;
  if (p.a_seg || p.b_seg) return false;
  const int64_t lim = (int64_t)1 << 31;
  const int64_t ea = ak ? (256 * p.lda + p.K) * 2 : (p.K + 64) * p.lda * 2;
  const int64_t eb = bk ? (256 * p.ldb + p.K) * 2 : (p.K + 64) * p.ldb * 2;
  return ea < lim && eb < lim && p.lda > 0 && p.ldb > 0;
}

int cst_gemm8p_launch(cstg::GemmParams p, bool ak, bool bk, int64_t nbatch, hipStream_t s) {
  const bool fast = !p.c_f32 && p.splits == 1 && p.vec_epi && (p.N % 8) == 0 && p.bias_mode != CST_BIAS_ROW &&
                    (p.bias_mode == CST_BIAS_NONE || p.alpha == 1.0f);
  const bool exf = fast && !p.aux_out && ((p.dact != 0) != (p.resid != nullptr)) && (!p.dact || p.aux_in);
  const bool plainf = fast && !p.dact && !p.resid;
#define CST_8P_MODE(MODE)                                                                                          \
  (ak ? (bk ? launch8p<true, true, MODE>(p, nbatch, s) : launch8p<true, false, MODE>(p, nbatch, s))              \
      : (bk ? launch8p<false, true, MODE>(p, nbatch, s) : launch8p<false, false, MODE>(p, nbatch, s)))
  if (exf) return CST_8P_MODE(2);
  if (plainf) return CST_8P_MODE(1);
  return CST_8P_MODE(0);
#undef CST_8P_MODE
}
```

chimera-st_amd/csrc/gemm_common.h:

```cpp
#pragma once
#include "cst_common.h"

namespace cstg {

constexpr int GEMM_MAX_BM = 256;

struct GemmParams {
  int64_t M, N, K;
  const void* A; int64_t lda, a_seg, a_seg_stride;
  const void* B; int64_t ldb, b_seg, b_seg_stride;
  void* C; int64_t ldc;
  const void* bias; int bias_mode; int64_t sbias0, sbias1;
  int act;
  void* aux_out; int64_t ld_aux_out;
  int dact;
  const void* aux_in; int64_t ld_aux_in;
  const void* resid; int64_t ld_resid;
  float alpha;
  uint32_t drop_thr, drop_key; float drop_scale;
  int64_t drop_row0;
  int64_t batch1;
  int64_t sa0, sa1, sb0, sb1, sc0, sc1;
  int splits;
  float* ws;
  int c_f32;
  int vec_epi;
  int tiles_m, tiles_n;
  int nz;
  int half_from, nitems;
  int group_m;
  unsigned long long magic_ntiles, magic_per_group;
  int per_group, group_shift;
  int gperm_full, gperm_q, gperm_r;
  int mrot;
  unsigned long long magic_gq, magic_gq1;
  int split_order;
  int* sched;
  const uint32_t* m_live; uint32_t m_epoch;
  const int32_t* k_len;
  const int32_t* m_len;
  const uint32_t* k_live; uint32_t k_epoch;
  void* colsum;
  float* colsum_ws;
};

__device__ __forceinline__ int64_t segaddr(int64_t c, int64_t seg, int64_t seg_stride) {
  return seg ? (c / seg) * seg_stride + (c % seg) : c;
}

template <typename T>
__device__ __forceinline__ void epilogue_store(const GemmParams& p, int64_t cofs, int64_t bofs, int64_t row, int64_t col, float v) {
  v *= p.alpha;
  if (p.bias_mode == CST_BIAS_COL) v += DT<T>::ld((const T*)p.bias + bofs + col);
  else if (p.bias_mode == CST_BIAS_ROW) v += DT<T>::ld((const T*)p.bias + bofs + row);
  if (p.aux_out) DT<T>::st((T*)p.aux_out + cofs + row * p.ld_aux_out + col, v);
  v = act_t<T>(v, p.act);
  if (p.drop_thr) v *= cst_drop1(p.drop_key, (uint64_t)((row + p.drop_row0) * p.N + col), p.drop_thr, p.drop_scale);
  if (p.dact) v *= dact_t<T>(DT<T>::ld((const T*)p.aux_in + cofs + row * p.ld_aux_in + col), p.dact);
  if (p.resid) v += DT<T>::ld((const T*)p.resid + cofs + row * p.ld_resid + col);
  if (p.c_f32) ((float*)p.C)[cofs + row * p.ldc + col] = v;
  else DT<T>::st((T*)p.C + cofs + row * p.ldc + col, v);
}

template <typename T>
__device__ __forceinline__ void epilogue_store8(const GemmParams& p, int64_t cofs, int64_t bofs, int64_t row, int64_t col, float (&v)[8]) {
#pragma unroll
  for (int e = 0; e < 8; ++e) v[e] *= p.alpha;
  if (p.bias_mode == CST_BIAS_COL) {
    float b[8];
    load8((const T*)p.bias + bofs + col, b);
#pragma unroll
    for (int e = 0; e < 8; ++e) v[e] += b[e];
  } else if (p.bias_mode == CST_BIAS_ROW) {
    const float b = DT<T>::ld((const T*)p.bias + bofs + row);
#pragma unroll
    for (int e = 0; e < 8; ++e) v[e] += b;
  }
  if (p.aux_out) store8((T*)p.aux_out + cofs + row * p.ld_aux_out + col, v);
  if (p.act == CST_ACT_RELU) {
#pragma unroll
    for (int e = 0; e < 8; ++e) v[e] = fmaxf(v[e], 0.0f);
  } else if (p.act == CST_ACT_GELU) {
#pragma unroll
    for (int e = 0; e < 8; ++e) v[e] = gelu_t<T>(v[e]);
  }
  if (p.drop_thr) cst_drop8(v, p.drop_key, (uint64_t)((row + p.drop_row0) * p.N + col), p.drop_thr, p.drop_scale);
  if (p.dact) {
    float z[8];
    load8((const T*)p.aux_in + cofs + row * p.ld_aux_in + col, z);
#pragma unroll
    for (int e = 0; e < 8; ++e) v[e] *= dact_t<T>(z[e], p.dact);
  }
  if (p.resid) {
    float r[8];
    load8((const T*)p.resid + cofs + row * p.ld_resid + col, r);
#pragma unroll
    for (int e = 0; e < 8; ++e) v[e] += r[e];
  }
  if (p.c_f32) store8((float*)p.C + cofs + row * p.ldc + col, v);
  else store8((T*)p.C + cofs + row * p.ldc + col, v);
}

}

int cst_gemm8p_launch(cstg::GemmParams p, bool a_kmajor, bool b_kmajor, int64_t nbatch, hipStream_t s);
bool cst_gemm8p_supported(const cstg::GemmParams& p, bool a_kmajor, bool b_kmajor, int64_t nbatch);
int cst_gemm4w_launch(cstg::GemmParams p, hipStream_t s);
bool cst_gemm4w_supported(const cstg::GemmParams& p, bool a_kmajor, bool b_kmajor, int64_t nbatch);
```

chimera-st_amd/functional.py:

```python
import os as _os
import weakref as _weakref

import torch

from . import kernels as K
from . import lib as L

_ACT = {None: L.ACT_NONE, "none": L.ACT_NONE, "relu": L.ACT_RELU, "gelu": L.ACT_GELU}


def _flat2d(x):
    return x.reshape(-1, x.shape[-1]).contiguous()


def _vec(dtype):
    return 8 if dtype == torch.bfloat16 else 4


def _with_tiles(t, tiles):
    if t.is_contiguous():
        t._cst_live_tiles = (tiles[0], tiles[1], t.data_ptr(), t.numel(), t.shape[-1], t._version)
        if t._base is not None:
            t._base._cst_live_tiles = t._cst_live_tiles
    return t
# ... 21 lines not shown
    parts = getattr(w, "_cst_parts", None)
    return w._version if parts is None else sum(p._version for p in parts)


class _WeightTransposes:

    def __init__(self):
        self.entries = {}
        self.tables = {}
        self.refreshes = 0
        self.persistent = {}

    def register_storage(self, owner, flat):
        sp = flat.untyped_storage().data_ptr()
        self.persistent[sp] = _weakref.ref(owner)
        _weakref.finalize(owner, self._drop_storage, sp)

    def _drop_storage(self, sp):
        self.persistent.pop(sp, None)
        for k in [k for k, e in self.entries.items() if e[4] == sp]:
            del self.entries[k]
        self.tables.clear()

    def invalidate(self):
        self.entries.clear()
        self.tables.clear()

    @staticmethod
    def _src(e):
        return e[0]() if isinstance(e[0], _weakref.ref) else e[0]

    def get(self, w):
        from .optim import PARAM_EPOCH
        epoch = PARAM_EPOCH[0]
        key = (w.data_ptr(), tuple(w.shape), w.dtype)
        e = self.entries.get(key)
        if e is not None and self._src(e) is None:
            del self.entries[key]
            self.tables.pop((w.device, w.dtype), None)
            e = None
        if e is None:
            sp = w.untyped_storage().data_ptr()
            owner = self.persistent.get(sp)
            if owner is not None and owner() is not None:
                src = w.detach()
                parts = getattr(w, "_cst_parts", None)
                if parts is not None:
                    src._cst_parts = parts
            elif isinstance(w, torch.nn.Parameter):
                src, sp = _weakref.ref(w), None
            else:
                return K.transpose2d(w)
            e = self.entries[key] = [src, K.transpose2d(w), _wversion(w), epoch, sp]
            self.tables.pop((w.device, w.dtype), None)
            return e[1]
        if e[2] != _wversion(w):
            K.transpose2d(w, e[1])
            e[2], e[3] = _wversion(w), epoch
            return e[1]
        if e[3] != epoch:
            kind = (w.device, w.dtype)
            stale = []
            for k, v in list(self.entries.items()):
                t = self._src(v)
                if t is None or t.data_ptr() != k[0]:
                    del self.entries[k]
                    self.tables.pop(kind, None)
                elif t.device == w.device and k[2] == w.dtype and v[3] != epoch:
                    stale.append(v)
            ids = [id(v) for v in stale]
            t = self.tables.get(kind)
            if t is None or t[5] != ids:
                t = self.tables[kind] = K.transpose_table([(self._src(v), v[1]) for v in stale]) + (ids,)
            K.transpose2d_multi(t)
            self.refreshes += 1
            for v in stale:
                v[2], v[3] = _wversion(self._src(v)), epoch
        return e[1]


WEIGHT_TRANSPOSES = _WeightTransposes()


def _may_defer(*params):
    if not K.DEFER.on:
        return False
    for w in params:
        if w is None:
            continue
        for p in (getattr(w, "_cst_parts_params", None) or (w,)):
            if not isinstance(p, torch.nn.Parameter) or p.grad is not None or getattr(p, "_cst_shared", False):
                return False
    return True


def _grad_out(w):
    if _os.environ.get("CST_NO_GRAD_SLOT"):
        return None
    from .optim import grad_slot
    return grad_slot(w)


class _LinearFn(torch.autograd.Function):
    @staticmethod
    def forward(ctx, x, weight, bias, resid, act, drop_p, drop_key):
        x2 = _flat2d(x)
        M, Kd = x2.shape
        N = weight.shape[0]
        w = weight.contiguous()
        ctx.bias_obj = bias
        Np = (N + _vec(x.dtype) - 1) // _vec(x.dtype) * _vec(x.dtype)
        if Np != N:
            wp = torch.zeros(Np, Kd, dtype=w.dtype, device=w.device)
            wp[:N] = w
            w = wp
            if bias is not None:
                bp = torch.zeros(Np, dtype=bias.dtype, device=bias.device)
                bp[:N] = bias
                bias = bp
            assert resid is None and drop_p == 0.0
        y = torch.empty(M, Np, dtype=x.dtype, device=x.device)
        z = torch.empty_like(y) if act != L.ACT_NONE else None
        r2 = _flat2d(resid) if resid is not None else None
        K.gemm(x2, w, y, M, Np, Kd, a_kmajor=1, b_kmajor=1, lda=Kd, ldb=Kd, ldc=Np, bias=bias, act=act, aux_out=z, ld_aux_out=Np,
               resid=r2, ld_resid=Np, split_k=1, drop_p=drop_p, drop_key=drop_key)
        ctx.save_for_backward(x2, w, z)
        ctx.act, ctx.has_bias, ctx.has_resid = act, bias is not None, resid is not None
        ctx.drop = (drop_p, drop_key)
        ctx.xshape, ctx.N = x.shape, N
        if Np != N:
            y = y[:, :N].contiguous()
        return y.view(*x.shape[:-1], N)

    @staticmethod
    def backward(ctx, dy):
        return _linear_backward(ctx, dy, None)


def _dx_gemm(dz, w, M, *, use_wt, like, resid=None, dact=L.ACT_NONE, aux_in=None, drop=(0.0, 0), m_live=None):
    n_out, n_in = w.shape
    dx = torch.empty(M, n_in, dtype=like.dtype, device=like.device)
    b, b_kmajor, ldb = (WEIGHT_TRANSPOSES.get(w), 1, n_out) if use_wt else (w, 0, n_in)
    K.gemm(dz, b, dx, M, n_in, n_out, a_kmajor=1, b_kmajor=b_kmajor, lda=n_out, ldb=ldb, ldc=n_in, dact=dact, aux_in=aux_in, ld_aux_in=n_in,
           resid=resid, ld_resid=n_in, split_k=1, drop_p=drop[0], drop_key=drop[1], m_live=m_live)
    return dx


def _dw_gemm(dz, x2, w, bias_obj, M, *, db_in_dw, live, dz_travels_on, allow_slot=True, allow_defer=True):
    n_out, n_in = w.shape
    dw = _grad_out(w) if allow_slot else None
    if dw is None:
        dw = torch.empty(n_out, n_in, dtype=w.dtype, device=w.device)
    db = torch.empty(n_out, dtype=w.dtype, device=w.device) if db_in_dw else None
    may = allow_defer and _may_defer(w, bias_obj if db_in_dw else None)
    big = not may or not K.dw_colsum_is_fused(n_out, n_in, M, w.dtype) or dz_travels_on
    K.side_gemm(big, (dz, x2, live[0] if live is not None else None), dz, x2, dw, n_out, n_in, M, a_kmajor=0, b_kmajor=0, lda=n_out, ldb=n_in,
                ldc=n_in, split_k=-1, k_live=live, colsum=db, defer=may)
    return dw, db


def _drop_grad(dy2, drop, out_dtype, live, *, with_colsum, defer):
    if with_colsum and not _os.environ.get("CST_NO_DROP_COLSUM"):
        return K.dropout_colsum(dy2.contiguous(), drop[0], drop[1], out_dtype, live, defer=defer)
    return K.dropout(dy2.contiguous(), *drop), None


def _linear_backward(ctx, dy, dxp):
    x2, w, z = ctx.saved_tensors
    M, Kd = x2.shape
    Np, N = w.shape[0], ctx.N
    if dy is None:
        return dxp, None, None, None, None, None, None
    dy2 = _flat2d(dy)
    live = _tiles_of(dy, M)
    if Np != N:
        dyp = torch.zeros(M, Np, dtype=dy2.dtype, device=dy2.device)
        dyp[:, :N] = dy2
        dy2 = dyp
    db_fused = None
    want_db = ctx.has_bias and ctx.needs_input_grad[2]
    db_in_dw = want_db and ctx.needs_input_grad[1] and Np % 8 == 0 and not _os.environ.get("CST_NO_GEMM_COLSUM") and K.dw_colsum_is_fused(Np, Kd, M, w.dtype)
    may_b = want_db and Np == N and _may_defer(w, ctx.bias_obj)
    if ctx.drop[0] > 0.0:
        dy2, db_fused = _drop_grad(dy2, ctx.drop, w.dtype, live, defer=may_b,
                                   with_colsum=not db_in_dw and ctx.act == L.ACT_NONE and want_db and Np == N and N % 8 == 0)
    dz = K.act_bwd(dy2, z, ctx.act) if ctx.act != L.ACT_NONE else dy2
    dx = dw = db = dres = None
    if ctx.needs_input_grad[0]:
        dx = _dx_gemm(dz, w, M, use_wt=_want_wt(M, w), like=x2, resid=_flat2d(dxp) if dxp is not None else None,
                      m_live=live).view(ctx.xshape)
        if live is not None and dxp is None:
            dx = _with_tiles(dx, live)
    if ctx.needs_input_grad[1]:
        dw, db = _dw_gemm(dz, x2, w, ctx.bias_obj, M, db_in_dw=db_in_dw, live=live, dz_travels_on=dz.data_ptr() == dy.data_ptr() and ctx.has_resid,
                          allow_slot=Np == N, allow_defer=Np == N)
        dw = dw[:N]
        if db is not None:
            db = db[:N]
    if want_db and db is None:
        db = db_fused if db_fused is not None else K.colsum(dz, w.dtype, live, defer=may_b)[:N]
    if ctx.has_resid and ctx.needs_input_grad[3]:
        dres = dy
    return dx, dw, db, dres, None, None, None


class _LinearPassFn(torch.autograd.Function):

    @staticmethod
    def forward(ctx, x, weight, bias, act, drop_p, drop_key):
        y = _LinearFn.forward(ctx, x, weight, bias, None, act, drop_p, drop_key)
        ctx.set_materialize_grads(False)
        return y, x.view_as(x)

    @staticmethod
    def backward(ctx, dy, dxp):
        g = _linear_backward(ctx, dy, dxp)
        return g[0], g[1], g[2], None, None, None


def linear_pass(x, weight, bias=None, act=None, dropout_p=0.0):
    return _LinearPassFn.apply(x, weight, bias, _ACT[act], *_drop_args(dropout_p))


def linear(x, weight, bias=None, act=None, resid=None, dropout_p=0.0):
    return _LinearFn.apply(x, weight, bias, resid, _ACT[act], *_drop_args(dropout_p))


class _FFNFn(torch.autograd.Function):

    @staticmethod
    def forward(ctx, x, w1, b1, w2, b2, resid, act, p_act, key_act, p_out, key_out):
        x2 = _flat2d(x)
        M, d = x2.shape
        F_ = w1.shape[0]
        dout = w2.shape[0]
        z1 = torch.empty(M, F_, dtype=x.dtype, device=x.device)
        h = torch.empty_like(z1)
        K.gemm(x2, w1, h, M, F_, d, a_kmajor=1, b_kmajor=1, lda=d, ldb=d, ldc=F_, bias=b1, act=act, aux_out=z1, ld_aux_out=F_, split_k=1,
               drop_p=p_act, drop_key=key_act)
        y = torch.empty(M, dout, dtype=x.dtype, device=x.device)
        r2 = _flat2d(resid) if resid is not None else None
        K.gemm(h, w2, y, M, dout, F_, a_kmajor=1, b_kmajor=1, lda=F_, ldb=F_, ldc=dout, bias=b2, resid=r2, ld_resid=dout, split_k=1,
               drop_p=p_out, drop_key=key_out)
        ctx.save_for_backward(x2, w1, w2, z1, h)
        ctx.cfg = (act, b1 is not None, b2 is not None, resid is not None, x.shape)
        ctx.res_is_x = (resid is not None and resid.data_ptr() == x.data_ptr() and resid.shape == x.shape
                        and resid.stride() == x.stride() and dout == d)
        ctx.drop = (p_act, key_act, p_out, key_out)
        ctx.bias_objs = (b1, b2)
        return y.view(*x.shape[:-1], dout)

    @staticmethod
    def backward(ctx, dy):
        x2, w1, w2, z1, h = ctx.saved_tensors
        act, has_b1, has_b2, has_res, xshape = ctx.cfg
        M, d = x2.shape
        F_, dout = w1.shape[0], w2.shape[0]
        dy2 = _flat2d(dy)
        live = _tiles_of(dy, M)
        p_act, key_act, p_out, key_out = ctx.drop
        b1, b2 = ctx.bias_objs
        db2_fused = None
        gcs = not _os.environ.get("CST_NO_GEMM_COLSUM")
        db2_in_dw = gcs and has_b2 and ctx.needs_input_grad[4] and ctx.needs_input_grad[3] and dout % 8 == 0 and K.dw_colsum_is_fused(dout, F_, M, w2.dtype)
        db1_in_dw = gcs and has_b1 and ctx.needs_input_grad[2] and ctx.needs_input_grad[1] and F_ % 8 == 0 and K.dw_colsum_is_fused(F_, d, M, w1.dtype)
        if p_out > 0.0:
            dy2, db2_fused = _drop_grad(dy2, (p_out, key_out), w2.dtype, live, defer=_may_defer(w2, b2),
                                        with_colsum=not db2_in_dw and has_b2 and ctx.needs_input_grad[4] and dout % 8 == 0)
        use_wt = _want_wt(M, w2) and _want_wt(M, w1)
        dz1 = _dx_gemm(dy2, w2, M, use_wt=use_wt, like=dy2, dact=act, aux_in=z1, drop=(p_act, key_act), m_live=live)
        dx = dw1 = db1 = dw2 = db2 = None
        if ctx.needs_input_grad[3]:
            dw2, db2 = _dw_gemm(dy2, h, w2, b2, M, db_in_dw=db2_in_dw, live=live, dz_travels_on=dy2.data_ptr() == dy.data_ptr() and has_res)
        if has_b2 and ctx.needs_input_grad[4] and db2 is None:
            db2 = db2_fused if db2_fused is not None else K.colsum(dy2, w2.dtype, live, defer=_may_defer(w2, b2))
        if ctx.needs_input_grad[0]:
            dx = _dx_gemm(dz1, w1, M, use_wt=use_wt, like=x2, resid=_flat2d(dy) if ctx.res_is_x else None, m_live=live).view(xshape)
        if ctx.needs_input_grad[1]:
            dw1, db1 = _dw_gemm(dz1, x2, w1, b1, M, db_in_dw=db1_in_dw, live=live, dz_travels_on=False)
        if has_b1 and ctx.needs_input_grad[2] and db1 is None:
            db1 = K.colsum(dz1, w1.dtype, live, defer=_may_defer(w1, b1))
        dres = dy if has_res and ctx.needs_input_grad[5] and not (ctx.res_is_x and ctx.needs_input_grad[0]) else None
        return dx, dw1, db1, dw2, db2, dres, None, None, None, None, None


def ffn(x, w1, b1, w2, b2, act, resid=None, activation_dropout_p=0.0, dropout_p=0.0):
    assert _ACT[act] != L.ACT_NONE
    return _FFNFn.apply(x, w1.contiguous(), b1, w2.contiguous(), b2, resid, _ACT[act], *_drop_args(activation_dropout_p), *_drop_args(dropout_p))


class _LayerNormFn(torch.autograd.Function):
    @staticmethod
    def forward(ctx, x, res, gamma, beta, eps):
        x2 = _flat2d(x)
        r2 = _flat2d(res) if res is not None else None
        y, s, mean, rstd = K.layernorm_fwd(x2, r2, gamma, beta, eps, want_sum=True)
        src = s if res is not None else x2
        ctx.save_for_backward(src, gamma, mean, rstd)
        ctx.has_res = res is not None
        ctx.shape = x.shape
        ctx.set_materialize_grads(False)
        if res is not None:
            return y.view(x.shape), s.view(x.shape)
        return y.view(x.shape), None

    @staticmethod
    def backward(ctx, dy, ds):
        src, gamma, mean, rstd = ctx.saved_tensors
        if dy is None:
            return ds, (ds if ctx.has_res else None), None, None, None
        dy2 = _flat2d(dy)
        dres = _flat2d(ds) if ds is not None else None
        dx, dg, db, tiles = K.layernorm_bwd(dy2, src, gamma, mean, rstd, dres, grad_dtype=gamma.dtype, want_tiles=True, defer=_may_defer(gamma))
        dx = _with_tiles(dx.view(ctx.shape), tiles)
        return dx, (dx if ctx.has_res else None), dg, db, None


def layer_norm(x, gamma, beta, eps=1e-5):
    return _LayerNormFn.apply(x, None, gamma, beta, eps)[0]


def add_layer_norm(x, res, gamma, beta, eps=1e-5):
    return _LayerNormFn.apply(x, res, gamma, beta, eps)


class _LayerNormPassFn(torch.autograd.Function):

    @staticmethod
    def forward(ctx, x, gamma, beta, eps):
        x2 = _flat2d(x)
        y, _, mean, rstd = K.layernorm_fwd(x2, None, gamma, beta, eps)
        ctx.save_for_backward(x2, gamma, mean, rstd)
        ctx.shape = x.shape
        ctx.set_materialize_grads(False)
        return y.view(x.shape), x.view_as(x)

    @staticmethod
    def backward(ctx, dy, dxp):
        x2, gamma, mean, rstd = ctx.saved_tensors
        dres = _flat2d(dxp) if dxp is not None else None
        if dy is None:
            return (dxp, None, None, None)
        dx, dg, db = K.layernorm_bwd(_flat2d(dy), x2, gamma, mean, rstd, dres, grad_dtype=gamma.dtype, defer=_may_defer(gamma))
        return dx.view(ctx.shape), dg, db, None


def layer_norm_residual(x, gamma, beta, eps=1e-5):
    return _LayerNormPassFn.apply(x, gamma, beta, eps)


_MASK_CACHE = []


_PAD_TILES = []


def _pad_tiles(u8):
    for src, pt in _PAD_TILES:
        if src is u8:
            return pt
    flat = u8.reshape(-1)
    pad = (-flat.numel()) % 64
    if pad:
        flat = torch.cat([flat, torch.ones(pad, dtype=flat.dtype, device=flat.device)])
# ... 826 lines not shown
```

chimera-st_amd/kernels.py:

```python
import ctypes
import os

import torch

from . import lib as L

_ws = {}
STATS = {}


def workspace(nbytes: int, device) -> torch.Tensor:
    key = (device.index, L.stream_ptr().value)
    t = _ws.get(key)
    if t is None or t.numel() < nbytes:
        t = torch.empty(max(nbytes, 1 << 20), dtype=torch.uint8, device=device)
        _ws[key] = t
    return t


class _Deferred:

    MAX_BYTES = 32 << 20

    def __init__(self):
# ... 15 lines not shown
        if self.side_used:
            torch.cuda.current_stream().wait_stream(self.side)
            self.side_used = False

    def flush(self):
        self.join()
        if self.items:
            reduce_multi(self.items)
            self.flushes += 1
            self.items, self.keep = [], []


DEFER = _Deferred()


def reduce_multi(items):
    lib = L.load()
    for at in range(0, len(items), 64):
        chunk = items[at:at + 64]
        arr = (L.ReduceItem * len(chunk))()
        for a, (src, dst, stride, Lr, P, dt, order) in zip(arr, chunk):
            a.src, a.dst, a.stride, a.L, a.P, a.dst_dtype, a.order = src, dst, stride, Lr, P, dt, order
        L.check(lib.cst_reduce_multi(arr, len(chunk), L.stream_ptr()), "cst_reduce_multi")


class deferred_reductions:

    def __init__(self, enabled=True):
        self.enabled = bool(enabled) and not os.environ.get("CST_NO_DEFER")

    def __enter__(self):
        if self.enabled:
            DEFER.on += 1
            DEFER.main = torch.cuda.current_stream()
            DEFER.poison = bool(os.environ.get("CST_DEFER_POISON"))
        return self

    def __exit__(self, *exc):
        if self.enabled:
            DEFER.on -= 1
            if DEFER.on == 0:
                DEFER.flush()
        return False


def side_gemm(big, reads, *args, **kw):
    if big or not DEFER.on or DEFER.main is None or not os.environ.get("CST_SIDE_STREAM") or torch.cuda.current_stream() != DEFER.main:
        return gemm(*args, **kw)
    if DEFER.side is None:
        DEFER.side = torch.cuda.Stream()
    side = DEFER.side
    side.wait_stream(DEFER.main)
    DEFER.side_used = True
    with torch.cuda.stream(side):
        out = gemm(*args, **kw)
    for t in reads:
        if t is not None:
            t.record_stream(side)
    STATS["side_gemm"] = STATS.get("side_gemm", 0) + 1
    return out


def _2d(t):
    assert t.dim() == 2 and t.stride(1) == 1, "expected a row-major 2-D tensor, got %s / %s" % (tuple(t.shape), t.stride())
    return t


def _stamps(live, extent, stat):
    if live is None:
        return None, 0
    assert live[0].numel() * 64 >= extent and live[0].dtype == torch.int32
    STATS[stat] = STATS.get(stat, 0) + 1
    return live[0].data_ptr(), live[1]


def _per_batch(v, batch0, stat):
    if v is None:
        return None
    assert v.dtype == torch.int32 and v.numel() == batch0 and v.is_contiguous()
    STATS[stat] = STATS.get(stat, 0) + 1
    return v.data_ptr()


def gemm(A, B, C, M, N, K, *, a_kmajor, b_kmajor, lda, ldb, ldc, bias=None, bias_mode=L.BIAS_COL, act=L.ACT_NONE,
         aux_out=None, ld_aux_out=0, dact=L.ACT_NONE, aux_in=None, ld_aux_in=0, resid=None, ld_resid=0, alpha=1.0,
         batch0=1, batch1=1, sa=(0, 0), sb=(0, 0), sc=(0, 0), sbias=(0, 0), a_seg=0, a_seg_stride=0, b_seg=0,
         b_seg_stride=0, split_k=-1, a_off=0, b_off=0, c_off=0, drop_p=0.0, drop_key=0, k_live=None, m_live=None, k_len=None, m_len=None,
         ws=None, colsum=None, defer=False, reduce_to=None):
    lib = L.load()
    d = L.GemmDesc()
    d.dtype = L.dtype_code(A.dtype)
    assert B.dtype == A.dtype, "A/B dtype mismatch"
    d.c_dtype = L.dtype_code(C.dtype)
    d.a_kmajor, d.b_kmajor = int(a_kmajor), int(b_kmajor)
    d.M, d.N, d.K = M, N, K
    es = A.element_size()
    d.A = A.data_ptr() + a_off * es
    d.lda, d.a_seg, d.a_seg_stride = lda, a_seg, a_seg_stride
    d.B = B.data_ptr() + b_off * es
    d.ldb, d.b_seg, d.b_seg_stride = ldb, b_seg, b_seg_stride
    d.C = C.data_ptr() + c_off * C.element_size()
    d.ldc = ldc
    if bias is not None:
        assert bias.dtype == A.dtype
        d.bias, d.bias_mode = bias.data_ptr(), bias_mode
    else:
        d.bias, d.bias_mode = None, L.BIAS_NONE
    d.sbias0, d.sbias1 = sbias
    d.act = act
    d.aux_out = None if aux_out is None else aux_out.data_ptr() + c_off * es
    d.ld_aux_out = ld_aux_out
    d.dact = dact
    d.aux_in = None if aux_in is None else aux_in.data_ptr() + c_off * es
    d.ld_aux_in = ld_aux_in
    d.resid = None if resid is None else resid.data_ptr() + c_off * es
    d.ld_resid = ld_resid
    d.alpha = alpha
    d.drop_p, d.drop_key = float(drop_p), int(drop_key) & 0xFFFFFFFF
    d.batch0, d.batch1 = batch0, batch1
    d.sa0, d.sa1 = sa
    d.sb0, d.sb1 = sb
    d.sc0, d.sc1 = sc
    d.split_k = split_k
    d.k_live, d.k_epoch = _stamps(k_live, K, "gemm_k_live")
    d.m_live, d.m_epoch = _stamps(m_live, M, "gemm_m_live")
    d.k_len = _per_batch(k_len, batch0, "gemm_k_len")
    d.m_len = _per_batch(m_len, batch0, "gemm_m_len")
    if colsum is not None:
        assert not a_kmajor and colsum.dtype == A.dtype and colsum.is_contiguous() and colsum.numel() == M * batch0 * batch1
        d.colsum = colsum.data_ptr()
    else:
        d.colsum = None
    d.defer_reduce = 0
    splits = 1
    need = lib.cst_gemm_workspace(ctypes.byref(d))
    nb = batch0 * batch1
    deferred = False
    if need > 0 and (reduce_to is not None or (defer and DEFER.on and nb == 1 and need <= DEFER.MAX_BYTES and ldc == N and N % 8 == 0)):
        splits = lib.cst_gemm_splits(ctypes.byref(d))
        if splits > 1:
            assert ws is None and bias is None and act == L.ACT_NONE and dact == L.ACT_NONE and resid is None and aux_out is None and alpha == 1.0
            ws = torch.empty(need, dtype=torch.uint8, device=A.device)
            d.defer_reduce = 1
            deferred = True
    if need > 0:
        if ws is None:
            ws = workspace(need, A.device)
        assert ws.dtype == torch.uint8 and ws.numel() >= need, "split-K scratch too small: %d < %d" % (ws.numel(), need)
        d.workspace, d.workspace_bytes = ws.data_ptr(), ws.numel()
    else:
        d.workspace, d.workspace_bytes = None, 0
    L.check(lib.cst_gemm(ctypes.byref(d), L.stream_ptr()), "cst_gemm")
    if reduce_to is not None:
        assert C.dtype == torch.float32 and sc == (M * N, 0) and ldc == N and reduce_to.numel() == M * N and reduce_to.is_contiguous() and colsum is None
        item = ((ws.data_ptr(), reduce_to, M * N, M * N, nb * splits, ws) if deferred else (C.data_ptr(), reduce_to, M * N, M * N, nb, C))
        if defer and DEFER.on:
            DEFER.push(*item)
        else:
            reduce_multi([(item[0], item[1].data_ptr(), item[2], item[3], item[4], L.dtype_code(reduce_to.dtype), 0)])
    elif deferred:
        DEFER.push(ws.data_ptr(), C, M * N, M * N, splits, ws)
        if colsum is not None:
            DEFER.push(ws.data_ptr() + 4 * splits * M * N, colsum, M, M, splits, ws)
    return C


_DW_FUSED = {}


def dw_colsum_is_fused(n_out, k_in, tokens, dtype):
    key = (n_out, k_in, tokens, dtype)
    r = _DW_FUSED.get(key)
    if r is None:
        d = L.GemmDesc()
        d.dtype = d.c_dtype = L.dtype_code(dtype)
        d.a_kmajor = d.b_kmajor = 0
        d.M, d.N, d.K = n_out, k_in, tokens
        d.batch0 = d.batch1 = 1
        d.split_k = -1
        d.colsum = 1
        r = _DW_FUSED[key] = bool(L.load().cst_gemm_colsum_is_fused(ctypes.byref(d)))
        if len(_DW_FUSED) > 4096:
            _DW_FUSED.clear()
    return r


def layernorm_fwd(x, res, gamma, beta, eps, want_sum=False):
    x = _2d(x)
    rows, cols = x.shape
    y = torch.empty_like(x)
    s = torch.empty_like(x) if (want_sum and res is not None) else None
    mean = torch.empty(rows, dtype=torch.float32, device=x.device)
    rstd = torch.empty(rows, dtype=torch.float32, device=x.device)
    L.check(L.load().cst_layernorm_fwd(L.ptr(x), L.ptr(res), L.ptr(gamma), L.ptr(beta), L.ptr(y), L.ptr(s), L.ptr(mean),
                                       L.ptr(rstd), rows, cols, eps, L.dtype_code(x.dtype), L.stream_ptr()), "cst_layernorm_fwd")
    return y, s, mean, rstd


_EPOCH = [0x3C6EF372]


def next_epoch():
    _EPOCH[0] = (_EPOCH[0] % 0xFFFFFFFE) + 1
    return _EPOCH[0]


def _two_stage(wbytes, outs, defer, launch):
    deferred = bool(defer) and DEFER.on > 0
    dev = outs[0].device
    ws = torch.empty(wbytes, dtype=torch.uint8, device=dev) if deferred else workspace(wbytes, dev)
    launch(ws, *[None if deferred else L.ptr(o) for o in outs])
    if deferred:
        n, cols = len(outs), outs[0].numel()
        for i, o in enumerate(outs):
            DEFER.push(ws.data_ptr() + 4 * cols * i, o, n * cols, cols, wbytes // (4 * n * cols), ws, order=1)


def layernorm_bwd(dy, s, gamma, mean, rstd, dres=None, grad_dtype=torch.float32, want_tiles=False, defer=False):
    dy, s = _2d(dy), _2d(s)
    rows, cols = s.shape
    lib = L.load()
    dx = torch.empty_like(s)
    dg = torch.empty(cols, dtype=grad_dtype, device=s.device)
    db = torch.empty(cols, dtype=grad_dtype, device=s.device)
    stamps, epoch = (torch.empty((rows + 63) // 64, dtype=torch.int32, device=s.device), next_epoch()) if want_tiles else (None, 0)

    def launch(ws, pg, pb):
        if want_tiles:
            L.check(lib.cst_layernorm_bwd_tiles(L.ptr(dy), L.ptr(s), L.ptr(gamma), L.ptr(mean), L.ptr(rstd), L.ptr(dres), L.ptr(dx), pg,
                                                pb, L.ptr(ws), rows, cols, L.dtype_code(s.dtype), L.dtype_code(grad_dtype),
                                                L.ptr(stamps), epoch, L.stream_ptr()), "cst_layernorm_bwd_tiles")
        else:
            L.check(lib.cst_layernorm_bwd(L.ptr(dy), L.ptr(s), L.ptr(gamma), L.ptr(mean), L.ptr(rstd), L.ptr(dres), L.ptr(dx), pg,
                                          pb, L.ptr(ws), rows, cols, L.dtype_code(s.dtype), L.dtype_code(grad_dtype), L.stream_ptr()),
                    "cst_layernorm_bwd")

    _two_stage(lib.cst_layernorm_bwd_workspace(rows, cols), (dg, db), defer, launch)
    return (dx, dg, db, (stamps, epoch)) if want_tiles else (dx, dg, db)


def _bhtd_strides(t, layout):
    assert t.stride(-1) == 1
    if layout == "bt":
        return t.stride(0), None, t.stride(1)
    return t.stride(1), None, t.stride(0)


def attn_desc(q, k, v, o, lse, H, D, kpm, causal, scale, layout_q="bt", layout_kv="bt", drop_p=0.0, drop_key=0, kv_len=None, seq=None):
    d = L.AttnDesc()
# ... 224 lines not shown

def glu_fwd(z):
    z = _2d(z)
    rows, C2 = z.shape
    y = torch.empty(rows, C2 // 2, dtype=z.dtype, device=z.device)
    L.check(L.load().cst_glu_fwd(L.ptr(z), L.ptr(y), rows, C2 // 2, L.dtype_code(z.dtype), L.stream_ptr()), "cst_glu_fwd")
    return y


def glu_bwd(dy, z):
    dy, z = _2d(dy), _2d(z)
    rows, C2 = z.shape
    dz = torch.empty_like(z)
    L.check(L.load().cst_glu_bwd(L.ptr(dy), L.ptr(z), L.ptr(dz), rows, C2 // 2, L.dtype_code(z.dtype), L.stream_ptr()), "cst_glu_bwd")
    return dz


def act_bwd(dy, z, act):
    assert dy.is_contiguous() and z.is_contiguous()
    dx = torch.empty_like(z)
    L.check(L.load().cst_act_bwd(L.ptr(dy), L.ptr(z), L.ptr(dx), z.numel(), act, L.dtype_code(z.dtype), L.stream_ptr()), "cst_act_bwd")
    return dx


def posconv_fwd(x, wg, bias, groups, m_len=None):
    B, T, C = x.shape
    k = wg.shape[2]
    assert x.is_contiguous() and wg.is_contiguous() and x.dtype == torch.bfloat16 and wg.dtype == x.dtype
    y = torch.empty_like(x)
    z = torch.empty_like(x)
    L.check(L.load().cst_posconv_fwd(L.ptr(x), L.ptr(wg), L.ptr(bias) if bias is not None else None, L.ptr(y), L.ptr(z),
                                     _per_batch(m_len, B, "gemm_m_len"), B, T, C, groups, k, L.stream_ptr()), "cst_posconv_fwd")
    return y, z


def posconv_dx(dz, wflip, dy, groups, m_len=None):
    B, T, C = dz.shape
    k = wflip.shape[2]
    assert dz.is_contiguous() and dy.is_contiguous() and wflip.is_contiguous() and dz.dtype == torch.bfloat16
    dx = torch.empty_like(dz)
    L.check(L.load().cst_posconv_dx(L.ptr(dz), L.ptr(wflip), L.ptr(dy), L.ptr(dx), _per_batch(m_len, B, "gemm_m_len"),
                                    B, T, C, groups, k, L.stream_ptr()), "cst_posconv_dx")
    return dx


def posconv_dw(dz, x, groups, k, db=None, k_live=None):
    B, T, C = dz.shape
    assert dz.is_contiguous() and x.is_contiguous() and dz.dtype == torch.bfloat16 and x.dtype == dz.dtype
    assert db is None or (db.dtype == dz.dtype and db.numel() == C and db.is_contiguous())
    dw = torch.empty(C, C // groups, k, dtype=dz.dtype, device=dz.device)
    Tp = T + k - 1 + (1 if k % 2 == 0 else 0)
    stamps, epoch = _stamps(k_live, B * Tp - (k - 1), "gemm_k_live")
    L.check(L.load().cst_posconv_dw(L.ptr(dz), L.ptr(x), L.ptr(dw), L.ptr(db) if db is not None else None,
                                    stamps, epoch, B, T, C, groups, k, L.stream_ptr()), "cst_posconv_dw")
    return dw


def act_fwd(x, act):
    assert x.is_contiguous()
    y = torch.empty_like(x)
    L.check(L.load().cst_act_fwd(L.ptr(x), L.ptr(y), x.numel(), act, L.dtype_code(x.dtype), L.stream_ptr()), "cst_act_fwd")
    return y


def colsum(x, out_dtype=torch.float32, live=None, defer=False):
    x = _2d(x)
    rows, cols = x.shape
    lib = L.load()
    out = torch.empty(cols, dtype=out_dtype, device=x.device)

    def launch(ws, po):
        if live is not None:
            assert live[0].numel() * 64 >= rows
            L.check(lib.cst_colsum_typed_live(L.ptr(x), x.stride(0), po, L.ptr(ws), rows, cols, L.dtype_code(x.dtype),
                                              L.dtype_code(out_dtype), L.ptr(live[0]), live[1], L.stream_ptr()), "cst_colsum_typed_live")
        else:
            L.check(lib.cst_colsum_typed(L.ptr(x), x.stride(0), po, L.ptr(ws), rows, cols, L.dtype_code(x.dtype), L.dtype_code(out_dtype),
                                         L.stream_ptr()), "cst_colsum_typed")

    _two_stage(lib.cst_colsum_workspace(rows, cols), (out,), defer, launch)
    return out


def dropout_colsum(x, p, key, out_dtype=torch.float32, live=None, defer=False):
    x = _2d(x)
    assert x.is_contiguous()
    rows, cols = x.shape
    lib = L.load()
    xd = torch.empty_like(x)
    out = torch.empty(cols, dtype=out_dtype, device=x.device)

    def launch(ws, po):
        L.check(lib.cst_dropout_colsum(L.ptr(x), L.ptr(xd), po, L.ptr(ws), rows, cols, L.dtype_code(x.dtype),
                                       L.dtype_code(out_dtype), float(p), int(key) & 0xFFFFFFFF, L.ptr(live[0]) if live is not None else None,
                                       live[1] if live is not None else 0, L.stream_ptr()), "cst_dropout_colsum")

    _two_stage(lib.cst_colsum_workspace(rows, cols), (out,), defer, launch)
    return xd, out


def colsum_atomic(x):
    x = _2d(x)
    rows, cols = x.shape
    out = torch.empty(cols, dtype=torch.float32, device=x.device)
    L.check(L.load().cst_colsum(L.ptr(x), x.stride(0), L.ptr(out), rows, cols, L.dtype_code(x.dtype), L.stream_ptr()), "cst_colsum")
    return out


def col2im1d(dcol, z, B, Lin, Lout, C, k, stride, pad, dact):
    dx = torch.empty(B, Lin, C, dtype=dcol.dtype, device=dcol.device)
    L.check(L.load().cst_col2im1d(L.ptr(dcol), L.ptr(z), L.ptr(dx), B, Lin, Lout, C, k, stride, pad, dact,
                                  L.dtype_code(dcol.dtype), L.stream_ptr()), "cst_col2im1d")
    return dx


def mask_rows(x, mask_u8):
    x = _2d(x)
    y = torch.empty_like(x)
    L.check(L.load().cst_mask_rows(L.ptr(x), L.ptr(mask_u8), L.ptr(y), x.shape[0], x.shape[1], L.dtype_code(x.dtype),
                                   L.stream_ptr()), "cst_mask_rows")
    return y


def rows_pack(x, seq_off, n_rows, tail_sum):
    assert x.dim() == 3 and x.is_contiguous() and seq_off.dtype == torch.int32 and seq_off.numel() == x.shape[0] + 1
    out = torch.empty(n_rows, x.shape[2], dtype=x.dtype, device=x.device)
    L.check(L.load().cst_rows_pack(L.ptr(x), L.ptr(seq_off), L.ptr(out), x.shape[0], x.shape[1], x.shape[2], int(bool(tail_sum)), L.dtype_code(x.dtype),
                                   L.stream_ptr()), "cst_rows_pack")
    return out


def rows_unpack(y, seq_off, B, T, tail_broadcast):
    assert y.dim() == 2 and y.is_contiguous() and seq_off.dtype == torch.int32 and seq_off.numel() == B + 1
    out = torch.empty(B, T, y.shape[1], dtype=y.dtype, device=y.device)
    L.check(L.load().cst_rows_unpack(L.ptr(y), L.ptr(seq_off), L.ptr(out), B, T, y.shape[1], int(bool(tail_broadcast)), L.dtype_code(y.dtype),
                                     L.stream_ptr()), "cst_rows_unpack")
    return out


def dropout(x, p, key):
    assert x.is_contiguous()
    y = torch.empty_like(x)
    L.check(L.load().cst_dropout(L.ptr(x), L.ptr(y), x.numel(), float(p), int(key) & 0xFFFFFFFF, L.dtype_code(x.dtype), L.stream_ptr()),
            "cst_dropout")
    return y


def conv_row_limits(nz_last, conv_spec, samples):
    Lc = len(conv_spec)
    ks = (ctypes.c_int32 * Lc)(*[int(c[1]) for c in conv_spec])
    st = (ctypes.c_int32 * Lc)(*[int(c[2]) for c in conv_spec])
    smax = max([int(c[2]) for c in conv_spec[1:]] or [1])
    B = nz_last.numel()
    assert nz_last.dtype == torch.int32 and nz_last.is_contiguous()
    out = torch.empty(Lc, 1 + smax, B, dtype=torch.int32, device=nz_last.device)
    L.check(L.load().cst_conv_row_limits(L.ptr(nz_last), ks, st, Lc, int(samples), L.ptr(out), B, smax, L.stream_ptr()), "cst_conv_row_limits")
    return out


def dropout_scale(x, alpha, p, key):
    assert x.is_contiguous()
    y = torch.empty_like(x)
    L.check(L.load().cst_dropout_scale(L.ptr(x), L.ptr(y), x.numel(), float(alpha), float(p), int(key) & 0xFFFFFFFF, L.dtype_code(x.dtype),
                                       L.stream_ptr()), "cst_dropout_scale")
    return y

# ... 390 lines not shown
```

chimera-st_amd/lib.py:

```python
import ctypes
import os

import torch

_HERE = os.path.dirname(os.path.abspath(__file__))
LIB_PATH = os.path.join(_HERE, "libcst_hip.so")
ABI_VERSION = 13

F32, BF16 = 0, 1
ACT_NONE, ACT_RELU, ACT_GELU = 0, 1, 2
BIAS_NONE, BIAS_COL, BIAS_ROW = 0, 1, 2
K_GEMM, K_ATTN_FWD, K_ATTN_BWD, K_LAYERNORM, K_CONV0, K_ELEMENTWISE, K_LOSS, K_OPTIM = range(8)
KERNEL_CLASSES = ["gemm", "attn_fwd", "attn_bwd", "layernorm", "conv0", "elementwise", "loss", "optim"]

c_i64, c_int, c_f, c_p = ctypes.c_int64, ctypes.c_int, ctypes.c_float, ctypes.c_void_p


class GemmDesc(ctypes.Structure):
    _fields_ = [
        ("dtype", c_int), ("c_dtype", c_int), ("a_kmajor", c_int), ("b_kmajor", c_int),
        ("M", c_i64), ("N", c_i64), ("K", c_i64),
        ("A", c_p), ("lda", c_i64), ("a_seg", c_i64), ("a_seg_stride", c_i64),
        ("B", c_p), ("ldb", c_i64), ("b_seg", c_i64), ("b_seg_stride", c_i64),
        ("C", c_p), ("ldc", c_i64),
        ("bias", c_p), ("bias_mode", c_int), ("sbias0", c_i64), ("sbias1", c_i64),
        ("act", c_int),
        ("aux_out", c_p), ("ld_aux_out", c_i64),
        ("dact", c_int),
        ("aux_in", c_p), ("ld_aux_in", c_i64),
        ("resid", c_p), ("ld_resid", c_i64),
        ("alpha", c_f),
        ("drop_p", c_f), ("drop_key", ctypes.c_uint32),
        ("batch0", c_i64), ("batch1", c_i64),
        ("sa0", c_i64), ("sa1", c_i64), ("sb0", c_i64), ("sb1", c_i64), ("sc0", c_i64), ("sc1", c_i64),
        ("split_k", c_int),
        ("workspace", c_p), ("workspace_bytes", c_i64),
        ("k_live", c_p), ("k_epoch", ctypes.c_uint32),
        ("m_live", c_p), ("m_epoch", ctypes.c_uint32),
        ("k_len", c_p),
        ("m_len", c_p),
        ("colsum", c_p),
        ("defer_reduce", c_int),
    ]


class ReduceItem(ctypes.Structure):
    _fields_ = [("src", c_p), ("dst", c_p), ("stride", c_i64), ("L", c_i64), ("P", ctypes.c_int32), ("dst_dtype", ctypes.c_int32),
                ("block0", ctypes.c_int32), ("order", ctypes.c_int32)]


class AttnDesc(ctypes.Structure):
    _fields_ = [
        ("dtype", c_int),
        ("B", c_i64), ("H", c_i64), ("Tq", c_i64), ("Tk", c_i64), ("D", c_i64),
        ("Q", c_p), ("q_sb", c_i64), ("q_sh", c_i64), ("q_st", c_i64),
        ("K", c_p), ("k_sb", c_i64), ("k_sh", c_i64), ("k_st", c_i64),
        ("V", c_p), ("v_sb", c_i64), ("v_sh", c_i64), ("v_st", c_i64),
        ("O", c_p), ("o_sb", c_i64), ("o_sh", c_i64), ("o_st", c_i64),
        ("lse", c_p),
        ("key_padding_mask", c_p), ("kpm_stride", c_i64),
        ("causal", c_int), ("scale", c_f),
        ("drop_p", c_f), ("drop_key", ctypes.c_uint32),
        ("dO", c_p), ("do_sb", c_i64), ("do_sh", c_i64), ("do_st", c_i64),
        ("dQ", c_p), ("dq_sb", c_i64), ("dq_sh", c_i64), ("dq_st", c_i64),
        ("dK", c_p), ("dk_sb", c_i64), ("dk_sh", c_i64), ("dk_st", c_i64),
        ("dV", c_p), ("dv_sb", c_i64), ("dv_sh", c_i64), ("dv_st", c_i64),
        ("delta", c_p),
        ("kv_len", c_p),
        ("q_flags", c_p),
        ("seq_offsets", c_p),
        ("kpm_bits", c_p),
        ("bwd_ws", c_p),
    ]


class BeamDesc(ctypes.Structure):
    _fields_ = [
        ("dtype", c_int),
        ("bsz", c_i64), ("beam", c_i64), ("vocab", c_i64), ("max_len", c_i64),
        ("pad", c_i64), ("unk", c_i64), ("eos", c_i64), ("min_len", c_i64),
        ("unk_penalty", c_f), ("len_penalty", c_f), ("temperature", c_f),
        ("normalize_scores", c_int),
        ("logits", c_p), ("ld_logits", c_i64),
        ("step", c_p),
        ("tokens", c_p), ("scores", c_p), ("anc", c_p),
        ("cands_to_ignore", c_p), ("finished", c_p), ("nfinal", c_p), ("num_remaining", c_p),
        ("fin_tokens", c_p), ("fin_pos", c_p), ("fin_score", c_p), ("fin_len", c_p),
        ("workspace", c_p),
        ("members", c_i64), ("logits_n", c_p * 7), ("lprobs_out", c_p),
        ("no_repeat_ngram", c_i64), ("prefix_tokens", c_p), ("prefix_len", c_i64),
        ("sampling", c_i64), ("sample_topk", c_i64), ("sample_topp", c_f), ("sample_key", c_p),
        ("diverse_groups", c_i64), ("diverse_strength", c_f), ("diverse_siblings", c_i64), ("sibling_rate", c_f),
        ("fin_anc", c_p),
    ]


class LmFusionDesc(ctypes.Structure):
    _fields_ = [("lm_logits", c_p), ("lm_weight", c_f), ("lprobs_out", c_p)]


class LexDesc(ctypes.Structure):
    _fields_ = [("representation", c_i64), ("constraints", c_p), ("width", c_i64), ("workspace", c_p)]


LEX_TBL_W, LEX_SW, LEX_NEXT_MAX, LEX_WIDTH_MAX = 136, 44, 16, 65


def lex_states(workspace, bsz, beam):
    words = workspace.view(torch.int32)
    return words[bsz * LEX_TBL_W:bsz * LEX_TBL_W + 2 * bsz * beam * LEX_SW].view(2, bsz * beam, LEX_SW)


class FbankDesc(ctypes.Structure):
    _fields_ = [
        ("B", c_i64), ("S", c_i64), ("T", c_i64),
        ("wave", c_p), ("n_samples", c_p), ("out", c_p), ("n_frames", c_p),
        ("utterance_cmvn", c_int), ("norm_means", c_int), ("norm_vars", c_int),
        ("global_mean", c_p), ("global_std", c_p),
        ("global_first", c_int),
        ("specaugment", c_int),
        ("n_fmask", c_int), ("n_tmask", c_int),
        ("fmask", c_p), ("tmask", c_p),
        ("mask_mean", c_int), ("mask_value", c_f),
        ("workspace", c_p), ("workspace_bytes", c_i64),
    ]


SYMBOLS = [
    ("cst_last_error", ctypes.c_char_p, []),
    ("cst_version", c_int, []),
    ("cst_device_arch_ok", c_int, []),
    ("cst_prof_enable", None, [c_int]),
    ("cst_prof_query", c_i64, [c_int, ctypes.POINTER(ctypes.c_double), ctypes.POINTER(ctypes.c_double), ctypes.POINTER(ctypes.c_double)]),
    ("cst_layernorm_fwd", c_int, [c_p, c_p, c_p, c_p, c_p, c_p, c_p, c_p, c_i64, c_i64, c_f, c_int, c_p]),
    ("cst_layernorm_bwd_workspace", c_i64, [c_i64, c_i64]),
    ("cst_layernorm_bwd", c_int, [c_p, c_p, c_p, c_p, c_p, c_p, c_p, c_p, c_p, c_p, c_i64, c_i64, c_int, c_int, c_p]),
    ("cst_layernorm_bwd_tiles", c_int, [c_p, c_p, c_p, c_p, c_p, c_p, c_p, c_p, c_p, c_p, c_i64, c_i64, c_int, c_int, c_p, ctypes.c_uint32, c_p]),
    ("cst_gemm_workspace", c_i64, [ctypes.POINTER(GemmDesc)]),
    ("cst_gemm_colsum_is_fused", c_int, [ctypes.POINTER(GemmDesc)]),
    ("cst_gemm_splits", c_int, [ctypes.POINTER(GemmDesc)]),
    ("cst_gemm_route", c_int, [ctypes.POINTER(GemmDesc), ctypes.c_char_p, c_i64]),
    ("cst_reduce_multi", c_int, [ctypes.POINTER(ReduceItem), c_int, c_p]),
    ("cst_gemm", c_int, [ctypes.POINTER(GemmDesc), c_p]),
    ("cst_posconv_fwd", c_int, [c_p, c_p, c_p, c_p, c_p, c_p, c_i64, c_i64, c_i64, c_i64, c_i64, c_p]),
    ("cst_posconv_dx", c_int, [c_p, c_p, c_p, c_p, c_p, c_i64, c_i64, c_i64, c_i64, c_i64, c_p]),
    ("cst_posconv_dw", c_int, [c_p, c_p, c_p, c_p, c_p, ctypes.c_uint32, c_i64, c_i64, c_i64, c_i64, c_i64, c_p]),
    ("cst_prof_dump", c_i64, [c_int, ctypes.c_char_p, c_i64]),
    ("cst_gemm_reserve_cus", c_int, [c_int]),
    ("cst_transpose2d", c_int, [c_p, c_p, c_i64, c_i64, c_int, c_p]),
    ("cst_transpose2d_multi", c_int, [c_p, c_int, c_i64, c_int, c_p]),
    ("cst_weight_norm_workspace", c_i64, [c_i64, c_i64]),
    ("cst_weight_norm_fwd", c_int, [c_p, c_p, c_p, c_p, c_p, c_i64, c_i64, c_int, c_p]),
    ("cst_weight_norm_bwd", c_int, [c_p, c_p, c_p, c_p, c_p, c_p, c_p, c_i64, c_i64, c_int, c_p]),
    ("cst_attn_bwd_workspace", c_i64, [ctypes.POINTER(AttnDesc)]),
    ("cst_attn_fwd", c_int, [ctypes.POINTER(AttnDesc), c_p]),
    ("cst_attn_bwd", c_int, [ctypes.POINTER(AttnDesc), c_p]),
    ("cst_conv0_fwd_workspace", c_i64, [c_i64, c_i64, c_int, c_int]),
    ("cst_conv0_gn_gelu_fwd", c_int, [c_p, c_p, c_p, c_p, c_p, c_p, c_p, c_p, c_p, c_p, c_i64, c_i64, c_i64, c_int, c_int, c_f, c_int, c_p]),
    ("cst_conv0_bwd_workspace", c_i64, [c_i64, c_i64, c_i64, c_int, c_int]),
    ("cst_conv0_gn_gelu_bwd", c_int, [c_p, c_p, c_p, c_p, c_p, c_p, c_p, c_p, c_p, c_p, c_p, c_p, c_p, c_i64, c_i64, c_i64, c_int, c_int, c_int, c_p]),
    ("cst_conv0_ln_gelu_fwd", c_int, [c_p, c_p, c_p, c_p, c_p, c_p, c_p, c_p, c_p, c_i64, c_i64, c_i64, c_int, c_int, c_f, c_int, c_p]),
    ("cst_conv0_ln_bwd_workspace", c_i64, [c_i64, c_i64, c_i64, c_int, c_int]),
    ("cst_conv0_ln_gelu_bwd", c_int, [c_p, c_p, c_p, c_p, c_p, c_p, c_p, c_p, c_p, c_p, c_p, c_p, c_p, c_p, c_i64, c_i64, c_i64, c_int, c_int, c_int, c_p]),
    ("cst_ln_gelu_fwd", c_int, [c_p, c_p, c_p, c_p, c_p, c_p, c_p, c_i64, c_i64, c_i64, c_f, c_int, c_p]),
    ("cst_ln_gelu_bwd_workspace", c_i64, [c_i64, c_i64]),
    ("cst_ln_gelu_bwd", c_int, [c_p, c_p, c_p, c_p, c_p, c_p, c_p, c_i64, c_p, c_p, c_p, c_p, c_p, c_i64, c_i64, c_i64, c_int, c_p]),
    ("cst_glu_fwd", c_int, [c_p, c_p, c_i64, c_i64, c_int, c_p]),
    ("cst_glu_bwd", c_int, [c_p, c_p, c_p, c_i64, c_i64, c_int, c_p]),
    ("cst_act_bwd", c_int, [c_p, c_p, c_p, c_i64, c_int, c_int, c_p]),
    ("cst_act_fwd", c_int, [c_p, c_p, c_i64, c_int, c_int, c_p]),
    ("cst_colsum", c_int, [c_p, c_i64, c_p, c_i64, c_i64, c_int, c_p]),
    ("cst_colsum_workspace", c_i64, [c_i64, c_i64]),
    ("cst_colsum_typed", c_int, [c_p, c_i64, c_p, c_p, c_i64, c_i64, c_int, c_int, c_p]),
    ("cst_colsum_typed_live", c_int, [c_p, c_i64, c_p, c_p, c_i64, c_i64, c_int, c_int, c_p, ctypes.c_uint32, c_p]),
    ("cst_col2im1d", c_int, [c_p, c_p, c_p, c_i64, c_i64, c_i64, c_i64, c_int, c_int, c_int, c_int, c_int, c_p]),
    ("cst_mask_rows", c_int, [c_p, c_p, c_p, c_i64, c_i64, c_int, c_p]),
    ("cst_dropout", c_int, [c_p, c_p, c_i64, c_f, ctypes.c_uint32, c_int, c_p]),
    ("cst_rows_pack", c_int, [c_p, c_p, c_p, c_i64, c_i64, c_i64, c_int, c_int, c_p]),
    ("cst_rows_unpack", c_int, [c_p, c_p, c_p, c_i64, c_i64, c_i64, c_int, c_int, c_p]),
    ("cst_dec_linear", c_int, [c_p, c_p, c_p, c_p, c_p, c_i64, c_i64, c_i64, c_i64, c_i64, c_i64, c_int, c_p, c_i64, c_int, c_p]),
    ("cst_dec_ln_linear", c_int, [c_p, c_p, c_p, c_p, c_f, c_p, c_p, c_i64, c_i64, c_i64, c_i64, c_i64, c_i64, c_int, c_p, c_i64, c_int, c_p]),
    ("cst_dropout_colsum", c_int, [c_p, c_p, c_p, c_p, c_i64, c_i64, c_int, c_int, c_f, ctypes.c_uint32, c_p, ctypes.c_uint32, c_p]),
    ("cst_conv_row_limits", c_int, [c_p, c_p, c_p, c_int, c_i64, c_p, c_i64, c_int, c_p]),
    ("cst_dropout_scale", c_int, [c_p, c_p, c_i64, c_f, c_f, ctypes.c_uint32, c_int, c_p]),
    ("cst_embed_pos_fwd", c_int, [c_p, c_p, c_p, c_p, c_p, c_f, c_i64, c_p, c_i64, c_i64, c_i64, c_i64, c_i64, c_f, ctypes.c_uint32, c_int, c_p]),
    ("cst_embed_bwd", c_int, [c_p, c_p, c_p, c_f, c_i64, c_i64, c_i64, c_i64, c_f, ctypes.c_uint32, c_int, c_int, c_p]),
    ("cst_ls_ce_fwd", c_int, [c_p, c_p, c_p, c_p, c_p, c_i64, c_i64, c_f, c_i64, c_int, c_p]),
    ("cst_ls_ce_bwd", c_int, [c_p, c_p, c_p, c_p, c_p, c_i64, c_i64, c_f, c_i64, c_int, c_p]),
    ("cst_score_tokens", c_int, [c_p, ctypes.POINTER(c_p), c_i64, c_i64, c_p, c_i64, c_p, c_p, c_p, c_i64, c_i64, c_i64, c_int, c_p]),
    ("cst_ctc_fwd", c_int, [c_p, c_i64, c_i64, c_p, c_i64, c_p, c_p, c_i64, c_int, c_p, c_p, c_p, c_p, c_p, c_p, c_i64, c_i64, c_i64, c_int, c_p]),
    ("cst_ctc_bwd", c_int, [c_p, c_i64, c_i64, c_p, c_i64, c_p, c_p, c_i64, c_int, c_p, c_p, c_p, c_p, c_p, c_p, c_i64, c_i64, c_i64, c_i64, c_i64,
                            c_int, c_p]),
    ("cst_ctc_greedy", c_int, [c_p, c_i64, c_i64, c_p, c_i64, c_p, c_p, c_p, c_i64, c_i64, c_i64, c_int, c_p]),
    ("cst_w2v_negatives", c_int, [ctypes.c_uint32, c_i64, c_i64, c_i64, c_i64, c_p, c_p]),
    ("cst_infonce_fwd", c_int, [c_p, c_p, c_p, c_f, c_p, c_p, c_p, c_p, c_p, c_p, c_p, c_p, c_i64, c_i64, c_i64, c_int, c_p]),
    ("cst_infonce_bwd_x", c_int, [c_p, c_p, c_p, c_f, c_p, c_p, c_p, c_p, c_p, c_p, c_i64, c_i64, c_i64, c_int, c_p]),
    ("cst_infonce_bwd_y", c_int, [c_p, c_p, c_p, c_p, c_p, c_p, c_p, c_p, c_i64, c_i64, c_i64, c_int, c_p]),
    ("cst_gumbel_vq_workspace", c_i64, [c_i64, c_i64, c_i64]),
    ("cst_gumbel_vq_fwd", c_int, [c_p, c_p, c_p, ctypes.c_uint32, c_int, c_p, c_p, c_p, c_p, c_p, c_p, c_p, c_i64, c_i64, c_i64, c_i64, c_int, c_p]),
    ("cst_gumbel_vq_bwd", c_int, [c_p, c_p, ctypes.c_uint32, c_f, c_p, c_p, c_p, c_p, c_p, c_i64, c_i64, c_i64, c_int, c_p]),
    ("cst_contrastive_fwd", c_int, [c_p, c_p, c_p, c_p, c_p, c_p, c_p, c_i64, c_i64, c_i64, c_f, c_int, c_p]),
    ("cst_contrastive_bwd", c_int, [c_p, c_p, c_p, c_p, c_p, c_p, c_p, c_p, c_i64, c_i64, c_i64, c_f, c_int, c_p]),
    ("cst_sumsq_workspace", c_i64, []),
    ("cst_sumsq", c_int, [c_p, c_i64, c_p, c_p, c_int, c_p]),
    ("cst_adam_step", c_int, [c_p, c_p, c_p, c_p, c_p, c_i64, c_f, c_f, c_f, c_f, c_f, c_i64, c_p, c_int, c_int, c_p]),
    ("cst_beam_workspace", c_i64, [c_i64, c_i64]),
    ("cst_beam_init", c_int, [ctypes.POINTER(BeamDesc), c_p]),
    ("cst_beam_step", c_int, [ctypes.POINTER(BeamDesc), c_p]),
    ("cst_beam_step_lm", c_int, [ctypes.POINTER(BeamDesc), ctypes.POINTER(LmFusionDesc), c_p]),
    ("cst_lex_workspace", c_i64, [c_i64, c_i64, c_i64]),
    ("cst_lex_init", c_int, [ctypes.POINTER(BeamDesc), ctypes.POINTER(LexDesc), c_p]),
    ("cst_beam_step_lex", c_int, [ctypes.POINTER(BeamDesc), ctypes.POINTER(LmFusionDesc), ctypes.POINTER(LexDesc), c_p]),
    ("cst_dec_embed", c_int, [c_p, c_p, c_p, c_p, c_f, c_i64, c_p, c_i64, c_i64, c_i64, c_i64, c_int, c_p]),
    ("cst_dec_self_attn", c_int, [c_p, c_p, c_p, c_p, c_p, c_p, c_i64, c_i64, c_i64, c_i64, c_f, c_int, c_p]),
    ("cst_batch_by_size", c_i64, [c_p, c_i64, c_i64, c_i64, ctypes.c_int32, c_p]),
    ("cst_wav_info", c_int, [ctypes.c_char_p, c_p, c_p, c_p, c_p]),
    ("cst_wav_read_f32", c_i64, [ctypes.c_char_p, c_i64, c_i64, c_p, c_i64]),
    ("cst_edit_distance", c_i64, [c_p, c_i64, c_p, c_i64]),
    ("cst_dec_cross_attn", c_int, [c_p, c_p, c_p, c_p, c_p, c_p, c_i64, c_i64, c_i64, c_i64, c_i64, c_i64, c_f, c_int, c_p]),
    ("cst_fbank_workspace_bytes", c_i64, [c_i64, c_i64]),
    ("cst_fbank", c_int, [ctypes.POINTER(FbankDesc), c_p]),
    ("cst_dec_ln_q_cross_attn", c_int, [c_p, c_i64, c_p, c_p, c_p, c_f, c_p, c_p, c_p, c_p, c_p, c_i64, c_i64, c_i64, c_i64, c_i64, c_i64, c_f, c_int, c_p]),
    ("cst_attn_avg_probs", c_int, [c_p, c_i64, c_p, c_i64, c_i64, c_i64, c_p, c_p, c_i64, c_p, c_i64, c_i64, c_i64, c_i64, c_i64, c_i64, c_f, c_f,
                                   c_int, c_int, c_p]),
    ("cst_collate_pairs", c_int, [c_p, c_p, c_int, c_p, c_p, c_i64, c_p, c_i64, c_i64, c_i64, c_i64, c_i64, c_int, c_int, c_p, c_p]),
    ("cst_token_block_slices", c_i64, [c_p, c_i64, c_int, c_i64, c_i64, c_p, c_i64]),
    ("cst_token_block_index", c_int, [c_p, c_i64, c_p, c_i64, c_p]),
    ("cst_collate_blocks", c_int, [c_p, c_int, c_p, c_i64, c_p, c_i64, c_i64, c_i64, c_i64, c_p, c_p]),
]

_lib = None


def load():
    global _lib
    if _lib is not None:
        return _lib
    if not os.path.exists(LIB_PATH):
        raise RuntimeError(
            "chimera-st_amd: %s is missing — the HIP extension is the product path and there is no fallback. "
            "Build it with `python -c 'import __graft_entry__ as g; g.build()'` or `make -C chimera-st_amd/csrc`." % LIB_PATH)
    lib = ctypes.CDLL(LIB_PATH)
    for name, res, args in SYMBOLS:
        fn = getattr(lib, name)
        fn.restype = res
        fn.argtypes = args
    built = lib.cst_version()
    if built != ABI_VERSION:
        raise RuntimeError("chimera-st_amd: %s was built for ABI version %d, this package binds version %d (include/cst.h "
                           "CST_ABI_VERSION) — rebuild it with `make -C chimera-st_amd/csrc`." % (LIB_PATH, built, ABI_VERSION))
    _lib = lib
    return lib


def check(rc, what=""):
    if rc != 0:
        msg = load().cst_last_error()
# ... 54 lines not shown
```

include/cst.h:

```cpp
#ifndef CST_H
#define CST_H

#include <stdint.h>

#ifdef __cplusplus
extern "C" {
#endif

#define CST_ABI_VERSION 13

typedef enum { CST_F32 = 0, CST_BF16 = 1 } cst_dtype;

typedef enum {
  CST_OK = 0,
  CST_ERR_BAD_ARG = -1,
  CST_ERR_LAUNCH = -2,
  CST_ERR_WORKSPACE = -3,
  CST_ERR_UNSUPPORTED = -4
} cst_status;

typedef void* cst_stream;

const char* cst_last_error(void);
int cst_version(void);
int cst_device_arch_ok(void);

typedef enum {
  CST_K_GEMM = 0, CST_K_ATTN_FWD, CST_K_ATTN_BWD, CST_K_LAYERNORM, CST_K_CONV0, CST_K_ELEMENTWISE,
  CST_K_LOSS, CST_K_OPTIM, CST_K_NUM
} cst_kernel_class;
void cst_prof_enable(int on);
int64_t cst_prof_query(int kernel_class, double* total_ms, double* flops, double* bytes);
int64_t cst_prof_dump(int kernel_class, char* buf, int64_t cap);

int cst_layernorm_fwd(const void* x, const void* res, const void* gamma, const void* beta,
                      void* y, void* sum_out, float* mean, float* rstd,
                      int64_t rows, int64_t cols, float eps, int dtype, cst_stream stream);
int64_t cst_layernorm_bwd_workspace(int64_t rows, int64_t cols);
int cst_layernorm_bwd(const void* dy, const void* s, const void* gamma, const float* mean,
                      const float* rstd, const void* dres, void* dx, void* dgamma, void* dbeta,
                      void* workspace, int64_t rows, int64_t cols, int dtype, int grad_dtype, cst_stream stream);
int cst_layernorm_bwd_tiles(const void* dy, const void* s, const void* gamma, const float* mean,
                            const float* rstd, const void* dres, void* dx, void* dgamma, void* dbeta,
                            void* workspace, int64_t rows, int64_t cols, int dtype, int grad_dtype,
                            uint32_t* tile_live, uint32_t epoch, cst_stream stream);

typedef enum { CST_ACT_NONE = 0, CST_ACT_RELU = 1, CST_ACT_GELU = 2 } cst_act;
typedef enum { CST_BIAS_NONE = 0, CST_BIAS_COL = 1, CST_BIAS_ROW = 2 } cst_bias_mode;

typedef struct {
  int dtype;
  int c_dtype;
  int a_kmajor, b_kmajor;
  int64_t M, N, K;
  const void* A; int64_t lda, a_seg, a_seg_stride;
  const void* B; int64_t ldb, b_seg, b_seg_stride;
  void* C; int64_t ldc;
  const void* bias; int bias_mode;
  int64_t sbias0, sbias1;
  int act;
  void* aux_out; int64_t ld_aux_out;
  int dact;
  const void* aux_in; int64_t ld_aux_in;
  const void* resid; int64_t ld_resid;
  float alpha;
  float drop_p; uint32_t drop_key;
  int64_t batch0, batch1;
  int64_t sa0, sa1, sb0, sb1, sc0, sc1;
  int split_k;
  void* workspace; int64_t workspace_bytes;
  const uint32_t* k_live; uint32_t k_epoch;
  const uint32_t* m_live; uint32_t m_epoch;
  const int32_t* k_len;
  const int32_t* m_len;
  void* colsum;
  int defer_reduce;
} cst_gemm_desc;

int64_t cst_gemm_workspace(const cst_gemm_desc* d);
int cst_gemm_colsum_is_fused(const cst_gemm_desc* d);
int cst_gemm_splits(const cst_gemm_desc* d);
int cst_gemm_route(const cst_gemm_desc* d, char* out, int64_t out_bytes);
int cst_gemm_reserve_cus(int n);
int cst_gemm(const cst_gemm_desc* d, cst_stream stream);

int cst_posconv_fwd(const void* x, const void* w, const void* bias, void* y, void* z, const int32_t* m_len, int64_t B, int64_t T,
                    int64_t C, int64_t groups, int64_t k, cst_stream stream);
int cst_posconv_dx(const void* dz, const void* wflip, const void* dy, void* dx, const int32_t* m_len, int64_t B, int64_t T,
                   int64_t C, int64_t groups, int64_t k, cst_stream stream);
int cst_posconv_dw(const void* dz, const void* x, void* dw, void* db, const uint32_t* k_live, uint32_t k_epoch, int64_t B,
                   int64_t T, int64_t C, int64_t groups, int64_t k, cst_stream stream);

typedef struct {
  int dtype;
  int64_t B, H, Tq, Tk, D;
  const void* Q; int64_t q_sb, q_sh, q_st;
  const void* K; int64_t k_sb, k_sh, k_st;
  const void* V; int64_t v_sb, v_sh, v_st;
  void* O; int64_t o_sb, o_sh, o_st;
  float* lse;
  const uint8_t* key_padding_mask; int64_t kpm_stride;
  int causal;
  float scale;
  float drop_p; uint32_t drop_key;
  const void* dO; int64_t do_sb, do_sh, do_st;
  void* dQ; int64_t dq_sb, dq_sh, dq_st;
  void* dK; int64_t dk_sb, dk_sh, dk_st;
  void* dV; int64_t dv_sb, dv_sh, dv_st;
  float* delta;
  const int32_t* kv_len;
  uint8_t* q_flags;
  const int32_t* seq_offsets;
  const uint64_t* kpm_bits;
  void* bwd_ws;
} cst_attn_desc;

int64_t cst_attn_bwd_workspace(const cst_attn_desc* d);
int cst_attn_fwd(const cst_attn_desc* d, cst_stream stream);
int cst_attn_bwd(const cst_attn_desc* d, cst_stream stream);

int cst_conv_row_limits(const int32_t* nz_last, const int32_t* k, const int32_t* stride, int L, int64_t S, int32_t* out, int64_t B,
                        int smax, cst_stream stream);
int64_t cst_conv0_fwd_workspace(int64_t B, int64_t S, int k, int stride);
int cst_conv0_gn_gelu_fwd(const float* wav, const void* w, const void* gamma, const void* beta,
                          void* y, float* mean, float* rstd, float* gram, float* workspace, const int32_t* frame_limit, int64_t B,
                          int64_t S, int64_t C, int k, int stride, float eps, int dtype, cst_stream stream);
int64_t cst_conv0_bwd_workspace(int64_t B, int64_t S, int64_t C, int k, int stride);
int cst_conv0_gn_gelu_bwd(const void* dy, const float* wav, const void* w, const void* gamma,
                          const void* beta, const float* mean, const float* rstd, const float* gram,
                          float* dw, float* dgamma, float* dbeta, float* workspace, const int32_t* frame_limit,
                          int64_t B, int64_t S, int64_t C, int k, int stride, int dtype,
                          cst_stream stream);

int cst_conv0_ln_gelu_fwd(const float* wav, const void* w, const void* bias, const void* gamma, const void* beta, void* y,
                          float* mean, float* rstd, const int32_t* frame_limit, int64_t B, int64_t S, int64_t C, int k,
                          int stride, float eps, int dtype, cst_stream stream);
int64_t cst_conv0_ln_bwd_workspace(int64_t B, int64_t S, int64_t C, int k, int stride);
int cst_conv0_ln_gelu_bwd(const void* dy, const float* wav, const void* w, const void* bias, const void* gamma, const void* beta,
                          const float* mean, const float* rstd, float* dw, float* dbias, float* dgamma, float* dbeta,
                          float* workspace, const int32_t* frame_limit, int64_t B, int64_t S, int64_t C, int k, int stride,
                          int dtype, cst_stream stream);
int cst_ln_gelu_fwd(const void* u, const void* gamma, const void* beta, void* y, float* mean, float* rstd,
                    const int32_t* row_limit, int64_t B, int64_t L, int64_t C, float eps, int dtype, cst_stream stream);
int64_t cst_ln_gelu_bwd_workspace(int64_t rows, int64_t C);
int cst_ln_gelu_bwd(const void* dy, const void* u, const void* gamma, const void* beta, const float* mean, const float* rstd,
                    void* du, int64_t du_batch_stride, float* dgamma, float* dbeta, float* dcolsum, float* workspace,
                    const int32_t* row_limit, int64_t B, int64_t L, int64_t C, int dtype, cst_stream stream);

int cst_glu_fwd(const void* z, void* y, int64_t rows, int64_t C, int dtype, cst_stream stream);
int cst_glu_bwd(const void* dy, const void* z, void* dz, int64_t rows, int64_t C, int dtype, cst_stream stream);
int cst_act_bwd(const void* dy, const void* z, void* dx, int64_t n, int act, int dtype, cst_stream stream);
int cst_act_fwd(const void* x, void* y, int64_t n, int act, int dtype, cst_stream stream);
int cst_colsum(const void* x, int64_t ldx, float* out, int64_t rows, int64_t cols, int dtype, cst_stream stream);
int cst_dropout_colsum(const void* x, void* xd, void* out, void* workspace, int64_t rows, int64_t cols, int dtype, int out_dtype,
                       float p, uint32_t key, const uint32_t* row_live, uint32_t epoch, cst_stream stream);
int64_t cst_colsum_workspace(int64_t rows, int64_t cols);
int cst_colsum_typed(const void* x, int64_t ldx, void* out, void* workspace, int64_t rows, int64_t cols, int dtype, int out_dtype,
                     cst_stream stream);
int cst_colsum_typed_live(const void* x, int64_t ldx, void* out, void* workspace, int64_t rows, int64_t cols, int dtype,
                          int out_dtype, const uint32_t* row_live, uint32_t epoch, cst_stream stream);
int cst_col2im1d(const void* dcol, const void* z, void* dx, int64_t B, int64_t Lin, int64_t Lout,
                 int64_t C, int k, int stride, int pad, int dact, int dtype, cst_stream stream);
int64_t cst_weight_norm_workspace(int64_t R, int64_t C);
int cst_weight_norm_fwd(const void* v, const void* g, void* w, float* norm, void* workspace, int64_t R, int64_t C, int dtype, cst_stream stream);
int cst_weight_norm_bwd(const void* v, const void* g, const void* dw, const float* norm, void* dv, void* dg, void* workspace, int64_t R,
                        int64_t C, int dtype, cst_stream stream);
int cst_transpose2d(const void* src, void* dst, int64_t R, int64_t C, int dtype, cst_stream stream);
typedef struct cst_transpose_item {
  const void* src; void* dst;
  int64_t R, C;
  int64_t tile0;
} cst_transpose_item;
int cst_transpose2d_multi(const cst_transpose_item* items_dev, int n, int64_t total_tiles, int dtype, cst_stream stream);
#define CST_REDUCE_MAX_ITEMS 64
typedef struct cst_reduce_item {
  const float* src; void* dst;
  int64_t stride, L;
  int32_t P, dst_dtype, block0, order;
} cst_reduce_item;
int cst_reduce_multi(const cst_reduce_item* items, int n, cst_stream stream);
int cst_mask_rows(const void* x, const uint8_t* mask, void* y, int64_t rows, int64_t cols, int dtype, cst_stream stream);

int cst_rows_pack(const void* src, const int32_t* seq_off, void* dst, int64_t B, int64_t T, int64_t C, int tail_sum, int dtype,
                  cst_stream stream);
int cst_rows_unpack(const void* src, const int32_t* seq_off, void* dst, int64_t B, int64_t T, int64_t C, int tail_broadcast, int dtype,
                    cst_stream stream);

int cst_dropout(const void* x, void* y, int64_t n, float p, uint32_t key, int dtype, cst_stream stream);
int cst_dropout_scale(const void* x, void* y, int64_t n, float alpha, float p, uint32_t key, int dtype, cst_stream stream);

int cst_embed_pos_fwd(const int64_t* tokens, const uint8_t* pad_mask, const void* embed, const void* x, const float* pos_table,
                      float scale, int64_t pad_idx, void* out, int64_t B, int64_t T, int64_t C, int64_t V, int64_t pos_rows,
                      float drop_p, uint32_t drop_key, int dtype, cst_stream stream);
int cst_embed_bwd(const void* dy, const int64_t* tokens, void* dE, float scale, int64_t pad_idx, int64_t n, int64_t C, int64_t V,
                  float drop_p, uint32_t drop_key, int dtype, int grad_dtype, cst_stream stream);

int cst_ls_ce_fwd(const void* logits, const int64_t* target, float* out2, float* lse, float* row_ws,
                  int64_t rows, int64_t V, float eps, int64_t pad_idx, int dtype, cst_stream stream);
int cst_ls_ce_bwd(const void* logits, const int64_t* target, const float* lse, const float* gscale,
                  void* dlogits, int64_t rows, int64_t V, float eps, int64_t pad_idx, int dtype,
                  cst_stream stream);

int cst_score_tokens(const void* logits, const void* const* logits_n, int64_t members, int64_t ld, const int64_t* target, int64_t pad,
                     float* pos, float* score, int32_t* len, int64_t B, int64_t T, int64_t V, int dtype, cst_stream stream);

int cst_ctc_fwd(const void* logits, int64_t stride_t, int64_t stride_b, const int64_t* targets, int64_t Lmax, const int64_t* target_len,
                const int64_t* input_len, int64_t blank, int zero_infinity, float* nll, float* loss, float* lse, float* emit, float* alpha,
                float* beta, int64_t T, int64_t B, int64_t V, int dtype, cst_stream stream);
int cst_ctc_bwd(const void* logits, int64_t stride_t, int64_t stride_b, const int64_t* targets, int64_t Lmax, const int64_t* target_len,
                const int64_t* input_len, int64_t blank, int zero_infinity, const float* nll, const float* lse, const float* alpha,
                const float* beta, const float* gscale, void* dlogits, int64_t dstride_t, int64_t dstride_b, int64_t T, int64_t B,
                int64_t V, int dtype, cst_stream stream);
int cst_ctc_greedy(const void* logits, int64_t stride_t, int64_t stride_b, const int64_t* input_len, int64_t blank, int32_t* argmax_ws,
                   int32_t* ids, int32_t* counts, int64_t T, int64_t B, int64_t V, int dtype, cst_stream stream);

int cst_w2v_negatives(uint32_t key, int64_t B, int64_t M, int64_t K, int64_t Kx, int32_t* out, cst_stream stream);
int cst_infonce_fwd(const void* x, const void* y, const int32_t* idx, float inv_temp, float* nll, float* loss, int32_t* counters,
                    float* lse, float* nx, float* ny, int32_t* flags, float* logits_dbg, int64_t N, int64_t KP, int64_t D, int dtype,
                    cst_stream stream);
int cst_infonce_bwd_x(const void* x, const void* y, const int32_t* idx, float inv_temp, const float* lse, const float* nx,
                      const float* ny, const float* gscale, void* dx, float* pairs, int64_t N, int64_t KP, int64_t D, int dtype,
                      cst_stream stream);
int cst_infonce_bwd_y(const void* x, const void* y, const int64_t* perm, const int32_t* offs, const float* pairs, const float* nx,
                      const float* ny, void* dy, int64_t N, int64_t KP, int64_t D, int dtype, cst_stream stream);

int64_t cst_gumbel_vq_workspace(int64_t N, int64_t G, int64_t V);
int cst_gumbel_vq_fwd(const void* logits, const void* vars, const float* noise, uint32_t key, int training, void* q, int32_t* idx,
                      void* onehot, float* avg_probs, float* stats, float* exph, void* workspace, int64_t N, int64_t G, int64_t V, int64_t d,
                      int dtype, cst_stream stream);
int cst_gumbel_vq_bwd(const void* logits, const float* noise, uint32_t key, float inv_tau, const void* gy, const float* avg_probs,
                      const float* exph, const float* dppl, void* dl, int64_t N, int64_t G, int64_t V, int dtype, cst_stream stream);

int cst_contrastive_fwd(const void* a, const void* t, float* loss, float* loss_rows, float* sim, float* na, float* nt,
                        int64_t B, int64_t M, int64_t C, float temp, int dtype, cst_stream stream);
int cst_contrastive_bwd(const void* a, const void* t, const float* sim, const float* na, const float* nt,
                        const float* gscale, void* da, void* dt, int64_t B, int64_t M, int64_t C, float temp,
                        int dtype, cst_stream stream);

int64_t cst_sumsq_workspace(void);
int cst_sumsq(const void* x, int64_t n, float* out, float* workspace, int dtype, cst_stream stream);
int cst_adam_step(float* master, float* exp_avg, float* exp_avg_sq, const void* grad, void* model_param,
                  int64_t n, float lr, float beta1, float beta2, float eps, float weight_decay,
                  int64_t step, const float* grad_scale, int grad_dtype, int param_dtype,
// ... 111 lines not shown
```

Before: 518.2.

## Fuse FFN bias-gradient column sum into persistent 8-wave GEMM epilogue

Adds an optional per-tile column-sum output to the persistent 8-wave bf16 GEMM epilogue. Each tile accumulates the rounded bf16 outputs per column, combines them across row-lanes through LDS, and writes them into 128-row slot partials. A later reduction turns the partials into db1 for the FFN first layer, replacing a separate colsum pass that re-reads dz1. This adds extra LDS traffic, barriers and register pressure to the epilogue, and an extra route query plus workspace allocation on the host. A non-fused tree colsum fallback keeps the same reduction order.

Result: slower. 506.2 (-2.3%).

```diff
diff --git a/chimera-st_amd/csrc/colsum_tree.h b/chimera-st_amd/csrc/colsum_tree.h
--- /dev/null
+++ b/chimera-st_amd/csrc/colsum_tree.h
@@ -0,0 +1,11 @@
+#pragma once
+#include <cstdint>
+
+namespace cst_tree {
+constexpr int SLOT_ROWS = 128;
+constexpr int LANES = 16;
+constexpr int ROWS_PER_LANE = SLOT_ROWS / LANES;
+
+constexpr int64_t slots(int64_t rows) { return rows > 0 ? 2 * ((rows + 2 * SLOT_ROWS - 1) / (2 * SLOT_ROWS)) : 0; }
+constexpr int64_t workspace_bytes(int64_t rows, int64_t cols) { return rows > 0 && cols > 0 ? slots(rows) * cols * (int64_t)sizeof(float) : 0; }
+}
diff --git a/chimera-st_amd/csrc/elementwise.hip b/chimera-st_amd/csrc/elementwise.hip
--- a/chimera-st_amd/csrc/elementwise.hip
+++ b/chimera-st_amd/csrc/elementwise.hip
@@ -1,4 +1,5 @@
 #include "cst_common.h"
+#include "colsum_tree.h"
 
 namespace {
 
@@ -64,7 +65,7 @@
   }
 }
 
-template <typename T, bool PART = false, bool DROP = false>
+template <typename T, bool PART = false, bool DROP = false, bool TREE = false>
 __global__ __launch_bounds__(256) void colsum_kernel(const T* x, int64_t ldx, float* out, int64_t rows, int64_t cols, int64_t rows_per,
                                                      const uint32_t* row_live = nullptr, uint32_t epoch = 0, T* xd = nullptr,
                                                      uint32_t dkey = 0, uint32_t dthr = 0, float dscale = 1.0f) {
@@ -88,7 +89,7 @@
   float acc[8] = {0, 0, 0, 0, 0, 0, 0, 0};
   if (ok) {
     int64_t r = r0 + g;
-    for (; r + 48 < r1; r += 64) {
+    for (; !TREE && r + 48 < r1; r += 64) {
       if (row_live && row_live[(r - g) >> 6] != epoch) {
         if (DROP) {
           float z[8] = {0, 0, 0, 0, 0, 0, 0, 0};
@@ -388,6 +389,28 @@
   return cst_check_launch("cst_dropout_colsum");
 }
 
+extern "C" int64_t cst_colsum_tree_workspace(int64_t rows, int64_t cols) { return cst_tree::workspace_bytes(rows, cols); }
+
+extern "C" int cst_colsum_tree(const void* x, int64_t ldx, void* out, void* workspace, int64_t rows, int64_t cols, int dtype, int out_dtype,
+                               cst_stream stream) {
+  static_assert(cst_tree::LANES == 16 && cst_tree::SLOT_ROWS == 128, "colsum_kernel: 16 row-lanes, rows 16 apart");
+  CST_REQUIRE(x && workspace && rows > 0 && cols > 0 && cols % 8 == 0 && ldx % 8 == 0, "cst_colsum_tree: cols/ldx must be multiples of 8");
+  CST_REQUIRE((dtype == CST_F32 || dtype == CST_BF16) && (out_dtype == CST_F32 || out_dtype == CST_BF16), "cst_colsum_tree: bad dtype");
+  hipStream_t s = (hipStream_t)stream;
+  CstProfScope prof(CST_K_ELEMENTWISE, s, 0.0, (double)rows * cols * cst_dtype_size(dtype));
+  const int64_t nslots = cst_tree::slots(rows);
+  CST_REQUIRE(nslots < 65536, "cst_colsum_tree: too many rows");
+  dim3 grid((unsigned)cst_ceil_div(cols / 8, 16), (unsigned)nslots);
+  float* part = (float*)workspace;
+  if (dtype == CST_BF16) hipLaunchKernelGGL((colsum_kernel<bf16_t, true, false, true>), grid, dim3(256), 0, s, (const bf16_t*)x, ldx, part, rows, cols, (int64_t)cst_tree::SLOT_ROWS);
+  else hipLaunchKernelGGL((colsum_kernel<float, true, false, true>), grid, dim3(256), 0, s, (const float*)x, ldx, part, rows, cols, (int64_t)cst_tree::SLOT_ROWS);
+  if (!out) return cst_check_launch("cst_colsum_tree");
+  const dim3 rgrid((unsigned)cst_ceil_div(cols, 16));
+  if (out_dtype == CST_BF16) hipLaunchKernelGGL(colsum_reduce_kernel<bf16_t>, rgrid, dim3(1024), 0, s, (const float*)part, (bf16_t*)out, (int)nslots, cols);
+  else hipLaunchKernelGGL(colsum_reduce_kernel<float>, rgrid, dim3(1024), 0, s, (const float*)part, (float*)out, (int)nslots, cols);
+  return cst_check_launch("cst_colsum_tree");
+}
+
 extern "C" int cst_colsum_typed(const void* x, int64_t ldx, void* out, void* workspace, int64_t rows, int64_t cols, int dtype,
                                 int out_dtype, cst_stream stream) {
   return colsum_typed_impl(x, ldx, out, workspace, rows, cols, dtype, out_dtype, nullptr, 0, stream);
diff --git a/chimera-st_amd/csrc/gemm.hip b/chimera-st_amd/csrc/gemm.hip
--- a/chimera-st_amd/csrc/gemm.hip
+++ b/chimera-st_amd/csrc/gemm.hip
@@ -1,4 +1,5 @@
 #include "gemm_common.h"
+#include "colsum_tree.h"
 #include <vector>
 #include <stdlib.h>
 #include <string.h>
@@ -836,6 +837,7 @@
   int stages;
   int splits;
   Colsum colsum;
+  bool c_colsum;
 };
 
 struct TileDims { int bm, bn, nt; };
@@ -899,6 +901,7 @@
   const bool large = use_large(d, r.seg, r.splits);
   const int64_t nbatch = d->batch0 * d->batch1;
   r.colsum = !d->colsum ? Colsum::None : (mm && !d->a_seg && !d->b_seg && !large) ? Colsum::Fused : Colsum::Separate;
+  r.c_colsum = false;
   auto take = [&r](Family f, Tile t, int stages = 2) { r.family = f; r.tile = t; r.stages = stages; return r; };
 
   if (!sw.no_narrow && !r.seg && !large && kk && d->N <= 64 && d->M > 256) return take(Family::Dma, Tile::NarrowN);
@@ -912,6 +915,7 @@
       if (f.kk != kk || strcmp(f.name, sw.force_cfg) != 0) continue;
       if (f.family == Family::Persistent8 && !cst_gemm8p_supported(q, r.ak, r.bk, nbatch)) break;
       if (f.family == Family::FourWave && !cst_gemm4w_supported(q, r.ak, r.bk, nbatch)) break;
+      r.c_colsum = f.family == Family::Persistent8 && d->c_colsum && cst_gemm8p_colsum_supported(q, r.ak, r.bk, nbatch);
       return take(f.family, f.tile, f.stages);
     }
     return take(Family::Reg, Tile::Unknown);
@@ -924,8 +928,10 @@
   }
   if (r.bf16 && !r.seg && !d->colsum) {
     if (!sw.no_4w && cst_gemm4w_supported(q, r.ak, r.bk, nbatch)) return take(Family::FourWave, Tile::Big4N);
-    if (r.ak && (!d->dact || (!d->resid && !d->aux_out)) && (large || mid8p) && cst_gemm8p_supported(q, r.ak, r.bk, nbatch))
+    if (r.ak && (!d->dact || (!d->resid && !d->aux_out)) && (large || mid8p) && cst_gemm8p_supported(q, r.ak, r.bk, nbatch)) {
+      r.c_colsum = d->c_colsum && cst_gemm8p_colsum_supported(q, r.ak, r.bk, nbatch);
       return take(Family::Persistent8, Tile::Large);
+    }
   }
   const Tile t = large ? Tile::Large : Tile::Small;
   if (r.seg) return take(Family::Reg, Tile::Small);
@@ -942,7 +948,7 @@
                r.colsum == Colsum::Fused ? " colsum" : "", r.splits);
       break;
     case Family::Dma: snprintf(out, (size_t)n, "glds %s %c%c %dx%d nt%d ns%d split%d", dt, a, b, t.bm, t.bn, t.nt, r.stages, r.splits); break;
-    case Family::Persistent8: snprintf(out, (size_t)n, "8p %c%c", a, b); break;
+    case Family::Persistent8: snprintf(out, (size_t)n, "8p %c%c%s", a, b, r.c_colsum ? " ccolsum" : ""); break;
     case Family::FourWave: snprintf(out, (size_t)n, "4w"); break;
   }
 }
@@ -1024,6 +1030,7 @@
   p.ws = nullptr;
   p.colsum = nullptr;
   p.colsum_ws = nullptr;
+  p.c_colsum = nullptr;
   return p;
 }
 
@@ -1043,6 +1050,12 @@
   CST_REQUIRE(cst_ceil_div(d->M, 128) * cst_ceil_div(d->N, 128) < (1ll << 31) && nbatch * r.splits < 65536, "cst_gemm: grid too large");
   p.splits = r.splits;
   p.colsum = r.colsum == Colsum::Fused ? d->colsum : nullptr;
+  if (d->c_colsum && !r.c_colsum) {
+    cst_set_error("cst_gemm: c_colsum is a by-product of the persistent 8-wave kernel's bf16 image epilogue only (cst_gemm_route tells)");
+    return CST_ERR_UNSUPPORTED;
+  }
+  CST_REQUIRE(!d->c_colsum || ((uintptr_t)d->c_colsum % 16) == 0, "cst_gemm: c_colsum must be 16-byte aligned");
+  p.c_colsum = d->c_colsum;
 #ifdef CST_TRACE
   if (p.splits == 1 && d->workspace) p.ws = (float*)d->workspace;
 #endif
@@ -1214,6 +1227,8 @@
 
 extern "C" int64_t cst_gemm_workspace(const cst_gemm_desc* d) { return route_workspace(d, query_route(d)); }
 
+extern "C" int64_t cst_gemm_colsum_workspace(const cst_gemm_desc* d) { return d ? cst_tree::workspace_bytes(d->M, d->N) : 0; }
+
 extern "C" int cst_gemm_route(const cst_gemm_desc* d, char* out, int64_t out_bytes) {
   if (out && out_bytes > 0) out[0] = 0;
   int rc = validate(d);
diff --git a/chimera-st_amd/csrc/gemm8p.hip b/chimera-st_amd/csrc/gemm8p.hip
--- a/chimera-st_amd/csrc/gemm8p.hip
+++ b/chimera-st_amd/csrc/gemm8p.hip
@@ -1,4 +1,5 @@
 #include "gemm_common.h"
+#include "colsum_tree.h"
 #include <atomic>
 #include <cstdlib>
 #include <mutex>
@@ -44,11 +45,17 @@
   return v;
 }
 
+template <int K>
+__device__ __forceinline__ void lds_read_lanes(float (&v)[cst_tree::LANES], unsigned addr) {
+  asm volatile("ds_read_b32 %0, %1 offset:%2" : "=v"(v[K]) : "v"(addr), "n"(K * 1024) : "memory");
+  if constexpr (K + 1 < cst_tree::LANES) lds_read_lanes<K + 1>(v, addr);
+}
+
 __device__ __forceinline__ void dma16(__amdgpu_buffer_rsrc_t rsrc, char* lds_wave_base, unsigned voff) {
   __builtin_amdgcn_raw_ptr_buffer_load_lds(rsrc, (__attribute__((address_space(3))) void*)lds_wave_base, 16, (int)voff, 0, 0, 0);
 }
 
-template <bool AK, bool BKM, int MODE>
+template <bool AK, bool BKM, int MODE, bool CS = false>
 __global__ __launch_bounds__(NTHREADS) void gemm8p_kernel(GemmParams p) {
   extern __shared__ __attribute__((aligned(16))) char smem[];
   const int tid = threadIdx.x, lane = tid & 63;
@@ -284,6 +291,19 @@
 
   char* const ebase = smem + BUFB;
   const unsigned ebase_off = lds_off(ebase);
+  const unsigned cs_off = lds_off(smem + 2 * BUFB + 1024 + 64);
+  auto cs_combine = [&](float* part, int64_t slot, int64_t n0c, int64_t ncols) {
+    if (tid < 256) {
+      float v[cst_tree::LANES];
+      lds_read_lanes<0>(v, cs_off + 4u * (unsigned)tid);
+      wait_lgkm<0>();
+      __builtin_amdgcn_sched_barrier(0);
+      float a = 0.0f;
+#pragma unroll
+      for (int k = 0; k < cst_tree::LANES; ++k) a += v[k];
+      if (n0c + tid < ncols) part[slot * ncols + n0c + tid] = a;
+    }
+  };
 
   int v = blockIdx.x;
   if (v >= total) return;
@@ -386,6 +406,8 @@
     q.aux_out = kp->aux_out; q.ld_aux_out = kp->ld_aux_out; q.dact = kp->dact; q.aux_in = kp->aux_in; q.ld_aux_in = kp->ld_aux_in;
     q.resid = kp->resid; q.ld_resid = kp->ld_resid; q.alpha = kp->alpha; q.splits = kp->splits; q.ws = kp->ws;
     q.c_f32 = kp->c_f32; q.vec_epi = kp->vec_epi; q.drop_thr = kp->drop_thr; q.drop_key = kp->drop_key; q.drop_scale = kp->drop_scale; q.drop_row0 = kp->drop_row0;
+    q.c_colsum = CS ? kp->c_colsum : nullptr;
+    const int64_t cs_slot0 = e_m0 / cst_tree::SLOT_ROWS;
     if (fast_epi && e_nt == 0 && q.bias_mode == CST_BIAS_NONE && !q.resid) {
       if (has_next) claim_land();
       const u32x4 z4 = {0u, 0u, 0u, 0u};
@@ -402,6 +424,10 @@
           }
         }
       }
+      if (CS && tid < 256 && e_n0 + tid < q.N) {
+        q.c_colsum[cs_slot0 * q.N + e_n0 + tid] = 0.0f;
+        if (!e_hf) q.c_colsum[(cs_slot0 + 1) * q.N + e_n0 + tid] = 0.0f;
+      }
     } else if (fast_epi) {
       constexpr int ERS = 528;
       const T* exsrc = MODE == 1 ? nullptr : (q.dact ? (const T*)q.aux_in : (const T*)q.resid);
@@ -425,6 +451,25 @@
       for (int hm = 0; hm < 2; ++hm) {
         if (hm && e_hf) break;
         if (hm) __builtin_amdgcn_s_barrier();
+        if (CS && hm) cs_combine(q.c_colsum, cs_slot0, e_n0, q.N);
+        typedef float f32x2 __attribute__((ext_vector_type(2)));
+        f32x2 cs[4] = {{0.0f, 0.0f}, {0.0f, 0.0f}, {0.0f, 0.0f}, {0.0f, 0.0f}};
+        auto cs_add = [&](const u32x4& w, bool ok) {
+          if (ok) {
+#pragma unroll
+            for (int e = 0; e < 4; ++e) {
+              const f32x2 v = {__uint_as_float(w[e] << 16), __uint_as_float(w[e] & 0xffff0000u)};
+              cs[e] += v;
+            }
+          }
+        };
+        auto cs_put = [&]() {
+          const unsigned a = cs_off + (unsigned)(tid >> 5) * 1024u + (unsigned)(tid & 31) * 32u;
+          const f32x4 lo = {cs[0][0], cs[0][1], cs[1][0], cs[1][1]}, hi4 = {cs[2][0], cs[2][1], cs[3][0], cs[3][1]};
+          lds_write_b128(a, lo);
+          lds_write_b128(a + 16u, hi4);
+          wait_lgkm<0>();
+        };
 #pragma unroll
         for (int i = 0; i < 2; ++i)
 #pragma unroll
@@ -544,6 +589,7 @@
 #pragma unroll
               for (int e = 0; e < 8; ++e) ob[e] = static_cast<__bf16>(x[e]);
               zr[it] = __builtin_bit_cast(u32x4, ob);
+              if (CS) cs_add(zr[it], col_ok && row0 + 16 * it < q.M);
             }
             if (hm == 0 && !e_hf) {
 #pragma unroll
@@ -557,6 +603,7 @@
             for (int it = 0; it < 8; ++it)
               if (col_ok && row0 + 16 * it < q.M)
                 __builtin_nontemporal_store(zr[it], reinterpret_cast<u32x4*>(cbase + (int64_t)(16 * it) * q.ldc));
+            if (CS) cs_put();
             continue;
           }
 #pragma unroll
@@ -570,6 +617,7 @@
             if (want_aux) __builtin_nontemporal_store(zraw, reinterpret_cast<u32x4*>(xbase + (int64_t)(16 * it) * q.ld_aux_out));
             if (!post) {
               __builtin_nontemporal_store(zraw, reinterpret_cast<u32x4*>(cdst));
+              if (CS) cs_add(zraw, true);
               continue;
             }
             float x[8];
@@ -591,9 +639,15 @@
 #pragma unroll
               for (int e = 0; e < 8; ++e) ob[e] = static_cast<__bf16>(x[e]);
               __builtin_nontemporal_store(__builtin_bit_cast(u32x4, ob), reinterpret_cast<u32x4*>(cdst));
+              if (CS) cs_add(__builtin_bit_cast(u32x4, ob), true);
             }
           }
+          if (CS) cs_put();
         }
+      }
+      if (CS) {
+        __builtin_amdgcn_s_barrier();
+        cs_combine(q.c_colsum, cs_slot0 + (e_hf ? 0 : 1), e_n0, q.N);
       }
     } else {
       constexpr int LDC = BN + 4;
@@ -688,11 +742,11 @@
 
 std::atomic<int> g_reserved_cus{[] { const char* e = getenv("CST_GEMM_RESERVE_CUS"); return e ? atoi(e) : 0; }()};
 
-template <bool AK, bool BKM, int MODE>
+template <bool AK, bool BKM, int MODE, bool CS = false>
 int launch8p(GemmParams p, int64_t nbatch, hipStream_t s) {
   static bool attr_set = false;
   if (!attr_set) {
-    (void)hipFuncSetAttribute(reinterpret_cast<const void*>(&gemm8p_kernel<AK, BKM, MODE>), hipFuncAttributeMaxDynamicSharedMemorySize, 160 * 1024);
+    (void)hipFuncSetAttribute(reinterpret_cast<const void*>(&gemm8p_kernel<AK, BKM, MODE, CS>), hipFuncAttributeMaxDynamicSharedMemorySize, 160 * 1024);
     attr_set = true;
   }
   p.tiles_m = (int)cst_ceil_div(p.M, BM);
@@ -739,7 +793,9 @@
   hipStreamCaptureStatus cap = hipStreamCaptureStatusNone;
   const bool capturing = hipStreamIsCapturing(s, &cap) != hipSuccess || cap != hipStreamCaptureStatusNone;
   p.sched = (!static_walk && !capturing && nitems > avail && grid.x % 8 == 0) ? sched_slot() : nullptr;
-  hipLaunchKernelGGL((gemm8p_kernel<AK, BKM, MODE>), grid, dim3(NTHREADS), LDS_BYTES + 1024 + 64, s, p);
+  constexpr int CS_BYTES = CS ? cst_tree::LANES * BN * (int)sizeof(float) : 0;
+  static_assert(LDS_BYTES + 1024 + 64 + CS_BYTES <= 160 * 1024, "LDS");
+  hipLaunchKernelGGL((gemm8p_kernel<AK, BKM, MODE, CS>), grid, dim3(NTHREADS), LDS_BYTES + 1024 + 64 + CS_BYTES, s, p);
   return cst_check_launch("cst_gemm (8-phase)");
 }
 
@@ -749,6 +805,15 @@
   const int old = g_reserved_cus.load();
   if (n >= 0) g_reserved_cus.store(n > 248 ? 248 : n);
   return old;
+}
+
+static bool image_epilogue(const cstg::GemmParams& p) {
+  return !p.c_f32 && p.splits == 1 && p.vec_epi && (p.N % 8) == 0 && p.bias_mode != CST_BIAS_ROW && (p.bias_mode == CST_BIAS_NONE || p.alpha == 1.0f);
+}
+
+bool cst_gemm8p_colsum_supported(const cstg::GemmParams& p, bool ak, bool bk, int64_t nbatch) {
+  (void)bk;
+  return ak && nbatch == 1 && image_epilogue(p);
 }
 
 bool cst_gemm8p_supported(const cstg::GemmParams& p, bool ak, bool bk, int64_t nbatch) {
@@ -761,15 +826,23 @@
 }
 
 int cst_gemm8p_launch(cstg::GemmParams p, bool ak, bool bk, int64_t nbatch, hipStream_t s) {
-  const bool fast = !p.c_f32 && p.splits == 1 && p.vec_epi && (p.N % 8) == 0 && p.bias_mode != CST_BIAS_ROW &&
-                    (p.bias_mode == CST_BIAS_NONE || p.alpha == 1.0f);
+  const bool fast = image_epilogue(p);
   const bool exf = fast && !p.aux_out && ((p.dact != 0) != (p.resid != nullptr)) && (!p.dact || p.aux_in);
   const bool plainf = fast && !p.dact && !p.resid;
 #define CST_8P_MODE(MODE)                                                                                          \
   (ak ? (bk ? launch8p<true, true, MODE>(p, nbatch, s) : launch8p<true, false, MODE>(p, nbatch, s))              \
       : (bk ? launch8p<false, true, MODE>(p, nbatch, s) : launch8p<false, false, MODE>(p, nbatch, s)))
+#define CST_8P_CS(MODE) (bk ? launch8p<true, true, MODE, true>(p, nbatch, s) : launch8p<true, false, MODE, true>(p, nbatch, s))
+  if (p.c_colsum) {
+    if (!cst_gemm8p_colsum_supported(p, ak, bk, nbatch)) {
+      cst_set_error("cst_gemm (8-phase): c_colsum needs the bf16 image epilogue, a k-major A and an unbatched problem");
+      return CST_ERR_UNSUPPORTED;
+    }
+    return exf ? CST_8P_CS(2) : plainf ? CST_8P_CS(1) : CST_8P_CS(0);
+  }
   if (exf) return CST_8P_MODE(2);
   if (plainf) return CST_8P_MODE(1);
   return CST_8P_MODE(0);
+#undef CST_8P_CS
 #undef CST_8P_MODE
 }
diff --git a/chimera-st_amd/csrc/gemm_common.h b/chimera-st_amd/csrc/gemm_common.h
--- a/chimera-st_amd/csrc/gemm_common.h
+++ b/chimera-st_amd/csrc/gemm_common.h
@@ -42,6 +42,7 @@
   const uint32_t* k_live; uint32_t k_epoch;
   void* colsum;
   float* colsum_ws;
+  float* c_colsum;
 };
 
 __device__ __forceinline__ int64_t segaddr(int64_t c, int64_t seg, int64_t seg_stride) {
@@ -105,5 +106,6 @@
 
 int cst_gemm8p_launch(cstg::GemmParams p, bool a_kmajor, bool b_kmajor, int64_t nbatch, hipStream_t s);
 bool cst_gemm8p_supported(const cstg::GemmParams& p, bool a_kmajor, bool b_kmajor, int64_t nbatch);
+bool cst_gemm8p_colsum_supported(const cstg::GemmParams& p, bool a_kmajor, bool b_kmajor, int64_t nbatch);
 int cst_gemm4w_launch(cstg::GemmParams p, hipStream_t s);
 bool cst_gemm4w_supported(const cstg::GemmParams& p, bool a_kmajor, bool b_kmajor, int64_t nbatch);
diff --git a/chimera-st_amd/functional.py b/chimera-st_amd/functional.py
--- a/chimera-st_amd/functional.py
+++ b/chimera-st_amd/functional.py
@@ -127,6 +127,9 @@
 WEIGHT_TRANSPOSES = _WeightTransposes()
 
 
+_NO_EPI_COLSUM = bool(_os.environ.get("CST_NO_EPI_COLSUM"))
+
+
 def _may_defer(*params):
     if not K.DEFER.on:
         return False
@@ -182,12 +185,12 @@
         return _linear_backward(ctx, dy, None)
 
 
-def _dx_gemm(dz, w, M, *, use_wt, like, resid=None, dact=L.ACT_NONE, aux_in=None, drop=(0.0, 0), m_live=None):
+def _dx_gemm(dz, w, M, *, use_wt, like, resid=None, dact=L.ACT_NONE, aux_in=None, drop=(0.0, 0), m_live=None, c_colsum=None):
     n_out, n_in = w.shape
     dx = torch.empty(M, n_in, dtype=like.dtype, device=like.device)
     b, b_kmajor, ldb = (WEIGHT_TRANSPOSES.get(w), 1, n_out) if use_wt else (w, 0, n_in)
     K.gemm(dz, b, dx, M, n_in, n_out, a_kmajor=1, b_kmajor=b_kmajor, lda=n_out, ldb=ldb, ldc=n_in, dact=dact, aux_in=aux_in, ld_aux_in=n_in,
-           resid=resid, ld_resid=n_in, split_k=1, drop_p=drop[0], drop_key=drop[1], m_live=m_live)
+           resid=resid, ld_resid=n_in, split_k=1, drop_p=drop[0], drop_key=drop[1], m_live=m_live, c_colsum=c_colsum)
     return dx
 
 
@@ -313,7 +316,10 @@
             dy2, db2_fused = _drop_grad(dy2, (p_out, key_out), w2.dtype, live, defer=_may_defer(w2, b2),
                                         with_colsum=not db2_in_dw and has_b2 and ctx.needs_input_grad[4] and dout % 8 == 0)
         use_wt = _want_wt(M, w2) and _want_wt(M, w1)
-        dz1 = _dx_gemm(dy2, w2, M, use_wt=use_wt, like=dy2, dact=act, aux_in=z1, drop=(p_act, key_act), m_live=live)
+        epi1 = None
+        if has_b1 and ctx.needs_input_grad[2] and not db1_in_dw and F_ % 8 == 0:
+            epi1 = K.EpiColsum(w1.dtype, _may_defer(w1, b1), fused=not _NO_EPI_COLSUM)
+        dz1 = _dx_gemm(dy2, w2, M, use_wt=use_wt, like=dy2, dact=act, aux_in=z1, drop=(p_act, key_act), m_live=live, c_colsum=epi1)
         dx = dw1 = db1 = dw2 = db2 = None
         if ctx.needs_input_grad[3]:
             dw2, db2 = _dw_gemm(dy2, h, w2, b2, M, db_in_dw=db2_in_dw, live=live, dz_travels_on=dy2.data_ptr() == dy.data_ptr() and has_res)
@@ -324,7 +330,7 @@
         if ctx.needs_input_grad[1]:
             dw1, db1 = _dw_gemm(dz1, x2, w1, b1, M, db_in_dw=db1_in_dw, live=live, dz_travels_on=False)
         if has_b1 and ctx.needs_input_grad[2] and db1 is None:
-            db1 = K.colsum(dz1, w1.dtype, live, defer=_may_defer(w1, b1))
+            db1 = epi1.out if epi1 is not None and epi1.out is not None else K.colsum(dz1, w1.dtype, live, defer=_may_defer(w1, b1))
         dres = dy if has_res and ctx.needs_input_grad[5] and not (ctx.res_is_x and ctx.needs_input_grad[0]) else None
         return dx, dw1, db1, dw2, db2, dres, None, None, None, None, None
 
diff --git a/chimera-st_amd/kernels.py b/chimera-st_amd/kernels.py
--- a/chimera-st_amd/kernels.py
+++ b/chimera-st_amd/kernels.py
@@ -121,11 +121,17 @@
     return v.data_ptr()
 
 
+class EpiColsum:
+
+    def __init__(self, out_dtype, defer=False, fused=True):
+        self.out_dtype, self.defer, self.fused, self.out = out_dtype, defer, fused, None
+
+
 def gemm(A, B, C, M, N, K, *, a_kmajor, b_kmajor, lda, ldb, ldc, bias=None, bias_mode=L.BIAS_COL, act=L.ACT_NONE,
          aux_out=None, ld_aux_out=0, dact=L.ACT_NONE, aux_in=None, ld_aux_in=0, resid=None, ld_resid=0, alpha=1.0,
          batch0=1, batch1=1, sa=(0, 0), sb=(0, 0), sc=(0, 0), sbias=(0, 0), a_seg=0, a_seg_stride=0, b_seg=0,
          b_seg_stride=0, split_k=-1, a_off=0, b_off=0, c_off=0, drop_p=0.0, drop_key=0, k_live=None, m_live=None, k_len=None, m_len=None,
-         ws=None, colsum=None, defer=False, reduce_to=None):
+         ws=None, colsum=None, defer=False, reduce_to=None, c_colsum=None):
     lib = L.load()
     d = L.GemmDesc()
     d.dtype = L.dtype_code(A.dtype)
@@ -189,7 +195,30 @@
         d.workspace, d.workspace_bytes = ws.data_ptr(), ws.numel()
     else:
         d.workspace, d.workspace_bytes = None, 0
+    part = None
+    if c_colsum is not None:
+        part = torch.empty(lib.cst_gemm_colsum_workspace(ctypes.byref(d)), dtype=torch.uint8, device=A.device)
+        d.c_colsum = part.data_ptr()
+        rc = lib.cst_gemm_route(ctypes.byref(d), _ROUTE_BUF, len(_ROUTE_BUF))
+        if rc == -4:
+            d.c_colsum, part = None, None
+        else:
+            L.check(rc, "cst_gemm_route")
+            if not c_colsum.fused:
+                d.c_colsum = None
     L.check(lib.cst_gemm(ctypes.byref(d), L.stream_ptr()), "cst_gemm")
+    if part is not None:
+        if not c_colsum.fused:
+            assert c_off == 0
+            L.check(lib.cst_colsum_tree(L.ptr(C), ldc, None, L.ptr(part), M, N, L.dtype_code(C.dtype), L.dtype_code(C.dtype), L.stream_ptr()), "cst_colsum_tree")
+        out = torch.empty(N, dtype=c_colsum.out_dtype, device=A.device)
+        slots = part.numel() // (4 * N)
+        if c_colsum.defer and DEFER.on:
+            DEFER.push(part.data_ptr(), out, N, N, slots, part, order=1)
+        else:
+            reduce_multi([(part.data_ptr(), out.data_ptr(), N, N, slots, L.dtype_code(out.dtype), 1)])
+        c_colsum.out = out
+        STATS["gemm_c_colsum"] = STATS.get("gemm_c_colsum", 0) + 1
     if reduce_to is not None:
         assert C.dtype == torch.float32 and sc == (M * N, 0) and ldc == N and reduce_to.numel() == M * N and reduce_to.is_contiguous() and colsum is None
         item = ((ws.data_ptr(), reduce_to, M * N, M * N, nb * splits, ws) if deferred else (C.data_ptr(), reduce_to, M * N, M * N, nb, C))
@@ -204,6 +233,7 @@
     return C
 
 
+_ROUTE_BUF = ctypes.create_string_buffer(128)
 _DW_FUSED = {}
 
 
@@ -594,6 +624,17 @@
     return out
 
 
+def colsum_tree(x, out_dtype=torch.float32):
+    x = _2d(x)
+    rows, cols = x.shape
+    lib = L.load()
+    out = torch.empty(cols, dtype=out_dtype, device=x.device)
+    ws = workspace(lib.cst_colsum_tree_workspace(rows, cols), x.device)
+    L.check(lib.cst_colsum_tree(L.ptr(x), x.stride(0), L.ptr(out), L.ptr(ws), rows, cols, L.dtype_code(x.dtype), L.dtype_code(out_dtype),
+                                L.stream_ptr()), "cst_colsum_tree")
+    return out
+
+
 def dropout_colsum(x, p, key, out_dtype=torch.float32, live=None, defer=False):
     x = _2d(x)
     assert x.is_contiguous()
diff --git a/chimera-st_amd/lib.py b/chimera-st_amd/lib.py
--- a/chimera-st_amd/lib.py
+++ b/chimera-st_amd/lib.py
@@ -41,6 +41,7 @@
         ("m_len", c_p),
         ("colsum", c_p),
         ("defer_reduce", c_int),
+        ("c_colsum", c_p),
     ]
 
 
@@ -137,6 +138,7 @@
     ("cst_layernorm_bwd", c_int, [c_p, c_p, c_p, c_p, c_p, c_p, c_p, c_p, c_p, c_p, c_i64, c_i64, c_int, c_int, c_p]),
     ("cst_layernorm_bwd_tiles", c_int, [c_p, c_p, c_p, c_p, c_p, c_p, c_p, c_p, c_p, c_p, c_i64, c_i64, c_int, c_int, c_p, ctypes.c_uint32, c_p]),
     ("cst_gemm_workspace", c_i64, [ctypes.POINTER(GemmDesc)]),
+    ("cst_gemm_colsum_workspace", c_i64, [ctypes.POINTER(GemmDesc)]),
     ("cst_gemm_colsum_is_fused", c_int, [ctypes.POINTER(GemmDesc)]),
     ("cst_gemm_splits", c_int, [ctypes.POINTER(GemmDesc)]),
     ("cst_gemm_route", c_int, [ctypes.POINTER(GemmDesc), ctypes.c_char_p, c_i64]),
@@ -173,6 +175,8 @@
     ("cst_colsum_workspace", c_i64, [c_i64, c_i64]),
     ("cst_colsum_typed", c_int, [c_p, c_i64, c_p, c_p, c_i64, c_i64, c_int, c_int, c_p]),
     ("cst_colsum_typed_live", c_int, [c_p, c_i64, c_p, c_p, c_i64, c_i64, c_int, c_int, c_p, ctypes.c_uint32, c_p]),
+    ("cst_colsum_tree_workspace", c_i64, [c_i64, c_i64]),
+    ("cst_colsum_tree", c_int, [c_p, c_i64, c_p, c_p, c_i64, c_i64, c_int, c_int, c_p]),
     ("cst_col2im1d", c_int, [c_p, c_p, c_p, c_i64, c_i64, c_i64, c_i64, c_int, c_int, c_int, c_int, c_int, c_p]),
     ("cst_mask_rows", c_int, [c_p, c_p, c_p, c_i64, c_i64, c_int, c_p]),
     ("cst_dropout", c_int, [c_p, c_p, c_i64, c_f, ctypes.c_uint32, c_int, c_p]),
diff --git a/include/cst.h b/include/cst.h
--- a/include/cst.h
+++ b/include/cst.h
@@ -75,9 +75,11 @@
   const int32_t* m_len;
   void* colsum;
   int defer_reduce;
+  float* c_colsum;
 } cst_gemm_desc;
 
 int64_t cst_gemm_workspace(const cst_gemm_desc* d);
+int64_t cst_gemm_colsum_workspace(const cst_gemm_desc* d);
 int cst_gemm_colsum_is_fused(const cst_gemm_desc* d);
 int cst_gemm_splits(const cst_gemm_desc* d);
 int cst_gemm_route(const cst_gemm_desc* d, char* out, int64_t out_bytes);
@@ -159,6 +161,9 @@
                      cst_stream stream);
 int cst_colsum_typed_live(const void* x, int64_t ldx, void* out, void* workspace, int64_t rows, int64_t cols, int dtype,
                           int out_dtype, const uint32_t* row_live, uint32_t epoch, cst_stream stream);
+int64_t cst_colsum_tree_workspace(int64_t rows, int64_t cols);
+int cst_colsum_tree(const void* x, int64_t ldx, void* out, void* workspace, int64_t rows, int64_t cols, int dtype, int out_dtype,
+                    cst_stream stream);
 int cst_col2im1d(const void* dcol, const void* z, void* dx, int64_t B, int64_t Lin, int64_t Lout,
                  int64_t C, int k, int stride, int pad, int dact, int dtype, cst_stream stream);
 int64_t cst_weight_norm_workspace(int64_t R, int64_t C);
```
